# ithakis/Option-Replicating-Portfolio-with-Neural-Networks

Measured on AMD Instinct MI355X. Metric: MC paths/sec training 30-step hedge-MLP + terminal P&L std-dev, 1/2/4/8 MI355X, higher is better.
Workload: dtype fp32

## Files before the change

csrc/hedge_lm.hip:

```cpp
#include <utility>

#include "hedge_core.h"
#include "hedge_narrow.h"

namespace rph {

typedef float lm_f32x16 __attribute__((ext_vector_type(16)));

template <int P>
struct LmShape {
  static constexpr int NP = ((P + 31) / 32) * 32;
  static constexpr int NB = NP / 32;
  static constexpr int NBLK = NB * (NB + 1) / 2;
  static constexpr int JP = NP + 33;
  static_assert(NP <= LM_NPMAX && NBLK * 1024 <= LM_GBLK_MAX, "network too large for the LM solver");
};

template <class F, int... J>
RPH_INLINE void lm_static_for(F&& f, std::integer_sequence<int, J...>) {
  (f(std::integral_constant<int, J>{}), ...);
}
template <int N, class F>
RPH_INLINE void lm_static_for(F&& f) {
  lm_static_for(f, std::make_integer_sequence<int, N>{});
}

}
#include "lm_chol.h"
namespace rph {

template <int P>
struct LmTPack {
  using TG = TileGrid<P>;
  static constexpr int OFF = LmShape<P>::NBLK * 1024;
  static constexpr int LEN = TG::NTILE * 256;
  static constexpr bool ON = TG::NX > 0 && OFF + LEN <= LM_GBLK_MAX;
  static constexpr int COPY = ON ? LEN : 0;
};

RPH_INLINE void lm_blk(int b, int NB, int& mb, int& nb) {
  int m = 0;
  while (b >= NB - m) {
    b -= NB - m;
    ++m;
  }
  mb = m;
  nb = m + b;
}

RPH_INLINE constexpr int lm_row(int q, int h) { return (q & 3) + 8 * (q >> 2) + 4 * h; }

template <class B>
__global__ __launch_bounds__(256, B::WAVES_PER_SIMD) void k_lm_pass(const TrainDesc d, const LmDesc lm, const int pass,
                                                                   const double* __restrict__ red_new) {
  constexpr int P = B::P;
  constexpr int R = B::R;
  constexpr int NR = B::NR;
  using S = typename B::S;
  using LS = LmShape<P>;
  constexpr int NP = LS::NP, NB = LS::NB, NBLK = LS::NBLK, JP = LS::JP;
  constexpr int NIN = B::NIN_, H = B::H_, NO = B::NO_, HEAD = B::HEAD_, NHOLD = B::NHOLD;
  const uint32_t kat = prefetch_kernarg_begin<(sizeof(TrainDesc) + sizeof(LmDesc) + 16 < 640 ? sizeof(TrainDesc) + sizeof(LmDesc) + 16 : 640)>();
  __shared__ __attribute__((aligned(16))) float scratch[B::SCRATCH_FLOATS];
  __shared__ __attribute__((aligned(16))) float wl[P + 4];
  __shared__ __attribute__((aligned(16))) float jt[B::FINAL ? 4 : LM_TILE * JP];
  __shared__ __attribute__((aligned(16))) unsigned char og_img[B::OGM ? B::OG_LDS : 16];
  const int tid = threadIdx.x, lane = tid & 63, wid = tid >> 6;
  prefetch_kernarg_end(kat);
  const bool stamp_wg = blockIdx.x >= 2 && blockIdx.y == 0;
#define RPH_STAMPP(k)                 \
  do {                                \
    if (stamp_wg) RPH_STAMP(k);       \
  } while (0)
  RPH_STAMPP(0);
  const int inst = blockIdx.y;
  double* st = lm.state + (size_t)inst * LMS_FLOATS;
  red_new += (size_t)inst * LM_RED;
  float* const slab_b = lm.slab_b + (size_t)inst * lm.num_wgs * R;
  float* const slab_g = lm.slab_g + (size_t)inst * lm.gram_wgs * NBLK * 1024;
  double* sl = st + LMS_SLOTS + LM_SLOT * (pass & 1);
  const int trial = pass == 0 ? 0 : 1 - (int)sl[LSS_BEST];
  const Perm perm = make_perm(1u, 0u, 0u, false);
  const bool path_wg = (int)blockIdx.x < lm.num_wgs;
  typename B::Pre pre;
  const int gram_base = B::OGM ? 0 : lm.gram_base;
  const bool fin = B::FINAL || pass == lm.passes;
  const typename B::Sched sc =
      B::sched(d, lm.num_wgs, (gram_base > 0 || fin) ? 0 : lm.gram_wgs, lm.gram_skip, lm.leaf_blocks);
  if (path_wg) B::load(d, 0, perm, sc.b0 * 128, lane, pre);
  for (int i = tid; i < P; i += 256) {
    float w;
    if (pass == 0) {
      const float* w0p = lm.w0 != nullptr ? lm.w0 + inst * LM_NPMAX : d.wts->w[0];
      w = w0p[i];
      if (lm.renorm) {
        if (i >= S::OW1 && i < S::OW1 + NIN * H) {
          const int f = (i - S::OW1) / H;
          w = (float)((double)w * ((double)lm.ren_isd[f] / (double)d.fisd[f]));
        } else if (i >= S::OB1 && i < S::OB1 + H) {
          double acc = (double)w;
#pragma unroll
          for (int f = 0; f < NIN; ++f)
            acc += (double)w0p[S::OW1 + f * H + (i - S::OB1)] * (double)lm.ren_isd[f] *
                   ((double)d.fmu[f] - (double)lm.ren_mu[f]);
          w = (float)acc;
        }
      }
    } else {
      w = (float)st[LMS_W + trial * LM_NPMAX + i];
    }
    wl[i] = w;
    if (pass == 0 && blockIdx.x == 0) st[LMS_W + i] = (double)w;
  }
  if (pass > 0 && sl[LSS_COPY] != 0.0) {
    constexpr int NG = LmShape<P>::NBLK * 1024 + LmTPack<P>::COPY;
    constexpr int NGR = LM_RED_OUTG - LM_GBLK_MAX + (B::NU <= LM_OG_MAX ? B::NU * (B::NU + 1) / 2 : 1);
    double* best_red = st + LMS_RED;
    for (int e = blockIdx.x * 256 + tid; e < NG + NGR; e += (int)gridDim.x * 256) {
      const int o = e < NG ? e : LM_GBLK_MAX + e - NG;
      best_red[o] = red_new[o];
    }
  }
  if (pass > 0 && sl[LSS_STOP] != 0.0) return;
  if (lm.dp_fused && blockIdx.x == 0 && tid == 0)
    __hip_atomic_fetch_add(lm.dp.counter, 1u, __ATOMIC_RELAXED, __HIP_MEMORY_SCOPE_AGENT);
  if (pass == 0 && blockIdx.x == 0 && tid == 0) {
    sl[LSS_BEST] = 1.0;
    sl[LSS_LAM] = lm.lam_carry > 0.f ? fmax(st[LMS_LAM] * (double)lm.lam_carry, (double)lm.lam_min) : (double)lm.lam0;
    sl[LSS_NU] = 2.0;
    sl[LSS_PRED] = 0.0;
    sl[LSS_COPY] = 0.0;
    sl[LSS_SPEC_IDX] = (double)LM_SPEC;
    sl[LSS_LBEST] = INFINITY;
    sl[LSS_STOP] = 0.0;
    st[LMS_NACC] = 0.0;
    st[LMS_FAIL] = 0.0;
  }
  if (pass == 0 && blockIdx.x == 0 && inst == 0 && !lm.weights_only && !lm.explore) {
    for (int k = tid; k < MAXHIST; k += 256) d.fit->hist[k] = __builtin_nanf("");
  }
  __syncthreads();
  RPH_STAMPP(1);
  if (path_wg) {
    typename B::Frags fr;
    B::make_frags(wl + S::OW2, fr);
    float val[NR];
    B::partial(d, 0, perm, wl, fr, scratch, pre, val, sc, og_img,
               lm.slab_o + ((size_t)inst * lm.num_wgs + blockIdx.x) * 3 * 1024);
#pragma unroll
    for (int j = 0; j < NR; ++j)
      if (tid + 256 * j < R) slab_b[(size_t)blockIdx.x * R + tid + 256 * j] = val[j];
  }
  RPH_STAMPP(2);
  const int gtile = (int)blockIdx.x - gram_base;
  if (fin || gtile < 0 || gtile >= lm.gram_wgs) return;
  if constexpr (!B::FINAL) {
  if (wid == 0) {
    const long long slot = (long long)gtile * LM_TILE + lane;
    float x[NIN], pr[NHOLD];
    bool ok;
    if (lm.gram_side) {
      ok = true;
#pragma unroll
      for (int f = 0; f < NIN; ++f) x[f] = (lm.gfeat[f][slot] - d.fmu[f]) * d.fisd[f];
#pragma unroll
      for (int k = 0; k < NHOLD - 1; ++k) pr[k] = lm.gprice[k][slot];
    } else {
      const long long p = (slot / lm.gram_blk) * lm.gram_blk_stride + slot % lm.gram_blk;
      ok = p < d.n_local;
      const long long q = ok ? p : 0;
#pragma unroll
      for (int f = 0; f < NIN; ++f) x[f] = (d.feat[f][q] - d.fmu[f]) * d.fisd[f];
#pragma unroll
      for (int k = 0; k < NHOLD - 1; ++k) pr[k] = d.price[k][q];
    }
    pr[NHOLD - 1] = d.bond;
    float z1[H], a1[H], z2[H], a2[H], hold[NHOLD];
    net_forward<NIN, H, NO, HEAD>(wl, x, d.alpha, z1, a1, z2, a2, hold);
    float wq = 1.f;
    if (d.loss == LOSS_PINBALL) {
      const long long p = (slot / lm.gram_blk) * lm.gram_blk_stride + slot % lm.gram_blk;
      float V = 0.f;
#pragma unroll
      for (int k = 0; k < NHOLD; ++k) V = fmaf(hold[k], pr[k], V);
      const float y = lm.gram_side ? lm.gtarget[slot] : d.target[ok ? p : 0];
      const float ra = ok ? fabsf(V - y) : 0.f;
      float sa = ra, sc = ok ? 1.f : 0.f;
#pragma unroll
      for (int o = 32; o >= 1; o >>= 1) {
        sa += __shfl_xor(sa, o, 64);
        sc += __shfl_xor(sc, o, 64);
      }
      const float dl = fmaxf(lm.q_delta, lm.q_kappa * sa / fmaxf(sc, 1.f));
      wq = 0.5f * __builtin_amdgcn_rsqf(fmaxf(ra, dl));
    }
    float dout[NO];
    if (HEAD == HEAD_COMPLEMENT) {
      dout[0] = pr[0] - pr[1];
    } else {
#pragma unroll
      for (int k = 0; k < NO; ++k) dout[k] = pr[k];
// ... 509 lines not shown
          const int i = k + 1 + e / MK, j = k + 1 + e % MK;
          if (j <= i) A[i * LDA + j] = aij[t] - (aik[t] * ajk[t]) * inv;
        }
      }
      lmc_wave_sync();
    });
    const int li = lane < N ? lane : 0;
    double rw[N], cl[N];
#pragma unroll
    for (int k = 0; k < N; ++k) {
      rw[k] = A[li * LDA + k];
      cl[k] = A[k * LDA + li];
    }
    const double di = lane < N ? A[lane * LDA + lane] : 1.0;
    const double ri = lm_rcp(di);
    const double gi = lane < N ? pre.gi : 0.0;
    double b = -gi;
#pragma unroll
    for (int k = 0; k < N; ++k) {
      const double zk = lmc_readlane(b, k) * lmc_readlane(ri, k);
      if (lane > k && lane < N) b -= rw[k] * zk;
    }
    b *= ri;
#pragma unroll
    for (int k = N - 1; k >= 0; --k) {
      const double dk = lmc_readlane(b, k);
      if (lane < k) b -= (cl[k] * ri) * dk;
    }
    if (lane >= N) b = 0.0;
    if (lane < N) out[lane] = b;
    double gd = 0.0;
#pragma unroll
    for (int j = 0; j < N; ++j) {
      const double gj = lane < N ? (lane == j ? G2d[li] : (lane < j ? rw[j] : cl[j])) : 0.0;
      gd += (0.5 * gj) * lmc_readlane(b, j);
    }
    double t = b * (gi + gd), tl = b * gi;
#pragma unroll
    for (int o = 32; o >= 1; o >>= 1) {
      t += __shfl_xor(t, o, 64);
      tl += __shfl_xor(tl, o, 64);
    }
    if (lane == 0) {
      *dl = t;
      dl[1] = tl;
      s_ok = ok ? 1 : 0;
    }
  }
  __syncthreads();
  return s_ok != 0;
}

template <int P, int R, int NU>
__global__ __launch_bounds__(256) void k_lm_solve(const TrainDesc d, const LmDesc lm, const double* __restrict__ red_new,
                                                  const int pass) {
#pragma clang fp contract(off)
  using LS = LmShape<P>;
  constexpr int NB = LS::NB, NBLK = LS::NBLK;
  extern __shared__ __attribute__((aligned(16))) double lds[];
  __shared__ int s_fail;
  __shared__ double s_diag;
  const int tid = threadIdx.x, lane = tid & 63, wid = tid >> 6;
  const int m = blockIdx.x;
  unsigned long long ts[8] = {};
  const bool stamp_on = d.stamps != nullptr && m == 0 && blockIdx.y == 0 && tid == 0;
#define RPH_STAMPS(k)                                        \
  do {                                                       \
    if (stamp_on) ts[(k)] = rph_stamp_clock();                \
  } while (0)
  RPH_STAMPS(0);
#ifdef RPH_LDS_POISON
  for (int i = tid; i < TileGrid<P>::LDS_BYTES / 8; i += 256) lds[i] = __builtin_nan("");
  __syncthreads();
#endif
  const int inst = blockIdx.y;
  double* st = lm.state + (size_t)inst * LMS_FLOATS;
  red_new += (size_t)inst * LM_RED;
  double* best_red = st + LMS_RED;
  const double* sin = st + LMS_SLOTS + LM_SLOT * (pass & 1);
  double* sout = st + LMS_SLOTS + LM_SLOT * ((pass + 1) & 1);
  const double sv_best = sin[LSS_BEST], sv_lbest = sin[LSS_LBEST], sv_stop = sin[LSS_STOP];
  const double sv_lam = sin[LSS_LAM], sv_nu = sin[LSS_NU], sv_pred = sin[LSS_PRED], sv_sidx = sin[LSS_SPEC_IDX];
  const double t_loss = red_new[LM_GBLK_MAX + LM_NPMAX], cnt = red_new[LM_GBLK_MAX + LM_NPMAX + 3];
  double sp_lam[LM_SPEC], sp_ok[LM_SPEC], sp_pred[LM_SPEC];
#pragma unroll
  for (int k = 0; k < LM_SPEC; ++k) {
    sp_lam[k] = st[LMS_SPEC_LAM + k];
    sp_ok[k] = st[LMS_SPEC_OK + k];
    sp_pred[k] = st[LMS_SPEC_PRED + k];
  }
  constexpr int NDS = (P + 63) / 64;
  const int tc = tid < P ? tid : P - 1;
  const double w_slot0 = st[LMS_W + tc], w_slot1 = st[LMS_W + LM_NPMAX + tc];
  const double g_new = red_new[LM_GBLK_MAX + tc], g_old = best_red[LM_GBLK_MAX + tc];
  const double d_new = lmc_gram<TileGrid<P>::NBG>(red_new, tc, tc), d_old = lmc_gram<TileGrid<P>::NBG>(best_red, tc, tc);
  double ds_new[NDS], ds_old[NDS];
#pragma unroll
  for (int k = 0; k < NDS; ++k) {
    const int i = lane + 64 * k < P ? lane + 64 * k : P - 1;
    ds_new[k] = lmc_gram<TileGrid<P>::NBG>(red_new, i, i);
    ds_old[k] = lmc_gram<TileGrid<P>::NBG>(best_red, i, i);
  }
  const bool final_pass = pass == lm.passes;
  constexpr bool OG_PRE = NU * NU <= 512;
  LmOgPre og_pre[2];
  double ogm_new = -1.0, ogm_old = -1.0;
  if constexpr (OG_PRE) {
    if (final_pass && m == 0 && lm.out_gram && lm.out_n == NU) {
      ogm_new = red_new[LM_RED_OUTG];
      ogm_old = best_red[LM_RED_OUTG];
#pragma unroll
      for (int u = 0; u < 2; ++u) {
// ... 254 lines not shown
      break;
    default:
      LmcOwner<P, 2>::template run<STAGED>(src, lds + TG::OFF_DIAG, g, T, pub, fac, &s_fail, lds + TG::OFF_RDG,
                                             lds + TG::OFF_X, xdone);
      break;
  }
  __syncthreads();
  RPH_STAMPS(3);
#ifdef RPH_DUMP_T
  if (m == 0 && d.stamps != nullptr)
    for (int i = tid; i < TG::NTILE * 256 + 2 * TG::PT; i += 256) reinterpret_cast<double*>(d.stamps)[i] = lds[i];
#endif
  const bool failed = s_fail != 0;
  __shared__ double s_pred[4];
  if (!failed) {
    double pv = 0.0;
    if (tid < P) {
      const double dv = vec[tid];
      pv = 0.5 * (dmp * dv * dv - gi * dv);
    }
#pragma unroll
    for (int o = 32; o >= 1; o >>= 1) pv += __shfl_xor(pv, o, 64);
    if (lane == 0) s_pred[wid] = pv;
    __syncthreads();
  }
  const double pred = (s_pred[0] + s_pred[1]) + (s_pred[2] + s_pred[3]);
  if (m > 0) {
    if (tid < P) st[LMS_SPEC_W + m * LM_NPMAX + tid] = failed ? wbest : wbest + vec[tid];
    if (tid == 0) {
      st[LMS_SPEC_LAM + m] = lam_m;
      st[LMS_SPEC_PRED + m] = failed ? 0.0 : pred;
      st[LMS_SPEC_OK + m] = failed ? 0.0 : 1.0;
    }
    return;
  }
  RPH_STAMPS(4);
  if (failed) {
    if (tid < P) st[LMS_W + (1 - best) * LM_NPMAX + tid] = wbest;
    publish(fmin(lam * lm.lam_up * lm.lam_up, (double)lm.lam_max), pred_prev, (double)LM_SPEC);
    if (tid == 0) {
      st[LMS_FAIL] += 1.0;
      st[LMS_FAILTOT] += 1.0;
    }
    return;
  }
  RPH_STAMPS(5);
  if (tid < P) st[LMS_W + (1 - best) * LM_NPMAX + tid] = wbest + vec[tid];
  publish(lam, pred, 1.0);
  if (stamp_on)
    for (int k = 0; k < 8; ++k) d.stamps[k] = ts[k];
#undef RPH_STAMPS
}

template <int NIN, int H, int NO, int HEAD>
struct LmKernels {
  using Body = NarrowPairBody<NIN, H, NO, HEAD>;
  using BodyOG = NarrowPairBody<NIN, H, NO, HEAD, true>;
  using S = NetShape<NIN, H, NO, HEAD>;
  static constexpr int smem() { return TileGrid<S::P>::LDS_BYTES; }
  static_assert(smem() + 128 <= 160 * 1024, "LM solve exceeds the LDS of one workgroup");
};

static int lm_validate(const TrainDesc* d, const LmDesc* lm, int P, int R, int nblk, int nu) {
  if (int rc = validate_train(d, 3 , "rph_lm")) return rc;
  if (!lm->state || !lm->slab_b || !lm->slab_g) return rph_report("rph_lm", "null LM buffer");
  if (d->batch != d->n_local || d->steps_per_epoch != 1) return rph_report("rph_lm", "LM fits are full batch");
  if (lm->num_wgs < 1 || lm->num_wgs > LM_PASS_WGS_MAX || lm->passes < 0 || lm->passes >= MAXHIST)
    return rph_report("rph_lm", "bad num_wgs (1..512) / passes");
  if (lm->leaf_blocks < 0 || (lm->leaf_blocks > 0 && (long long)lm->leaf_blocks * 128 * 4 * lm->num_wgs < d->batch))
    return rph_report("rph_lm", "leaf_blocks: the waves' leaves must cover the shard");
  if (lm->gram_wgs < 1 || lm->gram_wgs > 65535) return rph_report("rph_lm", "bad Gram workgroup count");
  if (lm->gram_base != 0 && (lm->gram_base != lm->num_wgs || lm->inst != 1))
    return rph_report("rph_lm", "gram_base: 0 or the path grid (one instance)");
  if (lm->gram_side) {
    const int nhold = d->head == HEAD_COMPLEMENT ? 2 : d->nout;
    for (int f = 0; f < d->nin; ++f)
      if (!lm->gfeat[f]) return rph_report("rph_lm", "null Gram subsample feature");
    for (int k = 0; k < nhold - 1; ++k)
      if (!lm->gprice[k]) return rph_report("rph_lm", "null Gram subsample price");
  } else {
    if (lm->gram_blk < 1 || lm->gram_blk > lm->gram_blk_stride)
      return rph_report("rph_lm", "bad Gram subsample geometry");
    const long long ns = (long long)lm->gram_wgs * LM_TILE;
    const long long last = ((ns - 1) / lm->gram_blk) * lm->gram_blk_stride + (ns - 1) % lm->gram_blk;
    if (last >= d->n_local) return rph_report("rph_lm", "Gram subsample leaves the shard");
  }
  if (lm->red_wgs != nblk * 1024 / 64 + R / 4 + lm_og_wgs(nu)) return rph_report("rph_lm", "bad red_wgs");
  if (lm->out_gram && (!lm->slab_o || nu > LM_OG_MAX)) return rph_report("rph_lm", "output Gram needs slab_o (<= 64 output parameters)");
  if (d->loss != LOSS_MSE && d->loss != LOSS_PINBALL) return rph_report("rph_lm", "LM fits: MSE or pinball loss");
  if (d->loss == LOSS_PINBALL && ((lm->gram_side && !lm->gtarget) || lm->out_gram || lm->out_n > 0 ||
                                  lm->bias_index >= 0 || !(lm->q_delta > 0.f)))
    return rph_report("rph_lm", "pinball LM fits: subsample targets with a simulated subsample, no output / "
                                "bias step, q_delta > 0");
  if (R != 128 && R != 256) return rph_report("rph_lm", "packet width must be 128 or 256");
  if (lm->inst < 1 || lm->inst > LM_SEL_MAX) return rph_report("rph_lm", "bad instance count");
  if (lm->inst > 1 && !lm->explore) return rph_report("rph_lm", "several instances are exploration fits only");
  if (lm->dp_fused) {
    const int nflags = R / 4 + lm_og_wgs(nu);
    if (!lm->gram_side || lm->inst != 1 || lm->explore || lm->weights_only)
      return rph_report("rph_lm", "fused DP exchange: one main fit on the shared Gram subsample only");
    if (lm->dp.world < 2 || lm->dp.world > 8 || lm->dp.rank < 0 || lm->dp.rank >= lm->dp.world ||
        lm->dp.pitch < LM_DP_PITCH || !lm->dp.counter || !lm->dp.error || nflags > LM_DP_FLAGS)
      return rph_report("rph_lm", "fused DP exchange: bad mailbox descriptor");
    for (int q = 0; q < lm->dp.world; ++q)
      if (!lm->dp.mbox[q]) return rph_report("rph_lm", "fused DP exchange: null peer mailbox");
  }
  if (lm->explore && lm->weights_only) return rph_report("rph_lm", "exploration fits publish nothing");
  if (lm->out_gram && lm->bias_index != -1 && (lm->bias_index < P - nu || lm->bias_index >= P))
    return rph_report("rph_lm", "output Gram: bias_index must be -1 or an output-layer parameter");
  return 0;
}

template <int A, int B, int C, int E>
static int lm_pass_launch(const TrainDesc* d, const LmDesc* lm, int pass, const double* red_new, hipStream_t s) {
  using K = LmKernels<A, B, C, E>;
  const bool og = lm->out_gram && pass > lm->passes - LM_OUTG_TAIL;
  const int gend = pass == lm->passes ? 0 : (og && K::BodyOG::OGM ? 0 : lm->gram_base) + lm->gram_wgs;
  const unsigned grid = (unsigned)(gend > lm->num_wgs ? gend : lm->num_wgs);
  if constexpr (K::BodyOG::OGM) {
    if (og) {
      hipLaunchKernelGGL((k_lm_pass<typename K::BodyOG>), dim3(grid, lm->inst), dim3(256), 0, s, *d, *lm, pass,
                         red_new);
      return (int)hipGetLastError();
    }
  }
  hipLaunchKernelGGL((k_lm_pass<typename K::Body>), dim3(grid, lm->inst), dim3(256), 0, s, *d, *lm, pass, red_new);
  return (int)hipGetLastError();
}

__global__ __launch_bounds__(256) void k_lm_dp_exchange(const LmDpDesc x, double* __restrict__ red, const int ng,
                                                         const int p) {
  __shared__ unsigned s_seq;
  const int tid = threadIdx.x, wg = blockIdx.x, W = x.world, me = x.rank;
  if (tid == 0) s_seq = __hip_atomic_load(x.counter, __ATOMIC_RELAXED, __HIP_MEMORY_SCOPE_AGENT) + 1u;
  __syncthreads();
  const unsigned seq = s_seq;
  const int slot = (int)(seq % DP_SLOTS);
  (void)p;
  const int len = ng + (LM_RED - LM_GBLK_MAX), chunk = (len + LM_DP_WGS - 1) / LM_DP_WGS;
  const int e0 = wg * chunk, e1 = min(len, e0 + chunk);
  auto off = [&](int e) {
    return e < ng ? e : LM_GBLK_MAX + e - ng;
  };
  for (int e = e0 + tid; e < e1; e += 256) {
    const double v = red[off(e)];
    for (int q = 0; q < W; ++q)
      if (q != me)
        __hip_atomic_store(x.mbox[q] + ((size_t)slot * W + me) * x.pitch + e, v, __ATOMIC_RELAXED,
                           __HIP_MEMORY_SCOPE_SYSTEM);
  }
  asm volatile("s_waitcnt vmcnt(0)" ::: "memory");
  __syncthreads();
  if (tid < W && tid != me) {
    unsigned* fo = reinterpret_cast<unsigned*>(x.mbox[tid] + ((size_t)slot * W + me) * x.pitch + LM_RED + wg);
    __hip_atomic_store(fo, seq, __ATOMIC_RELEASE, __HIP_MEMORY_SCOPE_SYSTEM);
    const unsigned* fi =
        reinterpret_cast<const unsigned*>(x.mbox[me] + ((size_t)slot * W + tid) * x.pitch + LM_RED + wg);
    unsigned it = 0;
    const unsigned long long t0 = __builtin_amdgcn_s_memrealtime();
    while (__hip_atomic_load(fi, __ATOMIC_ACQUIRE, __HIP_MEMORY_SCOPE_SYSTEM) != seq) {
      __builtin_amdgcn_s_sleep(2);
      if ((++it & 255u) == 0u && (__builtin_amdgcn_s_memrealtime() - t0 > DP_SPIN_TICKS ||
                                  __hip_atomic_load(x.error, __ATOMIC_RELAXED, __HIP_MEMORY_SCOPE_SYSTEM) != 0u)) {
        __hip_atomic_store(x.error, 1u, __ATOMIC_RELAXED, __HIP_MEMORY_SCOPE_SYSTEM);
        break;
      }
    }
  }
  __syncthreads();
  for (int e = e0 + tid; e < e1; e += 256) {
    const int o = off(e);
    double s = 0.0;
    for (int q = 0; q < W; ++q)
      s += q == me ? red[o]
                   : __hip_atomic_load(x.mbox[me] + ((size_t)slot * W + q) * x.pitch + e, __ATOMIC_RELAXED,
                                       __HIP_MEMORY_SCOPE_SYSTEM);
    red[o] = s;
  }
  __syncthreads();
// ... 128 lines not shown
  hipLaunchKernelGGL(k_lm_select, dim3(1), dim3(256), 0, (hipStream_t)stream, *d, *lm, sel, main_state, world, rank,
                     P, phase);
  return (int)hipGetLastError();
}

extern "C" int rph_lm_dp_exchange(const LmDpDesc* x, double* red, int ng, int p, void* stream) {
  if (!x || !red || x->world < 2 || x->world > 8 || x->rank < 0 || x->rank >= x->world)
    return rph_report("rph_lm_dp_exchange", "bad world / rank");
  if (x->pitch < LM_RED + LM_DP_WGS || ng < 0 || ng > LM_GBLK_MAX || p < 1 || (ng > 0 && p > LM_NPMAX))
    return rph_report("rph_lm_dp_exchange", "bad mailbox pitch / block geometry");
  if ((x->pitch % 2) != 0) return rph_report("rph_lm_dp_exchange", "mailbox rows must be 16-byte aligned");
  for (int q = 0; q < x->world; ++q)
    if (!x->mbox[q]) return rph_report("rph_lm_dp_exchange", "null peer mailbox");
  if (ng == 0) {
    if (p > LM_GREG || (p & 1)) return rph_report("rph_lm_dp_exchange", "bad gradient-region length");
    hipLaunchKernelGGL(k_lm_dp_exchange_g, dim3(1), dim3(256), 0, (hipStream_t)stream, *x, red, p);
    return (int)hipGetLastError();
  }
  hipLaunchKernelGGL(k_lm_dp_exchange, dim3(LM_DP_WGS), dim3(256), 0, (hipStream_t)stream, *x, red, ng, p);
  return (int)hipGetLastError();
}

extern "C" int rph_lm_shape(int nin, int h, int nout, int head, int* p, int* r, int* nblk) {
  int rc = -1;
  match_shape(NarrowShapes{}, nin, h, nout, head, &rc, [&](auto t) {
    using S = typename decltype(t)::S;
    *p = S::P;
    *r = S::R;
    *nblk = LmShape<S::P>::NBLK;
    return 0;
  });
  return rc;
}

extern "C" int rph_lm_pass_wps(int nin, int h, int nout, int head) {
  int wps = 1;
  match_shape(NarrowShapes{}, nin, h, nout, head, &wps, [](auto t) {
    using T = decltype(t);
    return (int)LmKernels<T::NIN, T::H, T::NO, T::HEAD>::Body::WAVES_PER_SIMD;
  });
  return wps;
}

template <class K>
static LmDesc lm_pass_desc(const LmDesc& lm, const int pass) {
  LmDesc lp = lm;
  const bool og = lm.out_gram && pass > lm.passes - LM_OUTG_TAIL;
  if (og && K::BodyOG::WAVES_PER_SIMD == 1 && lm.leaf_blocks == 0 && lm.gram_base == 0 && lm.num_wgs > 256 &&
      pass == lm.passes)
    lp.num_wgs = 256;
  return lp;
}

extern "C" int rph_lm_eval(const TrainDesc* d, const LmDesc* lm, double* red_new, int pass, void* stream) {
  hipStream_t s = (hipStream_t)stream;
  int rc = 0;
  if (match_shape(NarrowShapes{}, d->nin, d->h, d->nout, d->head, &rc, [&](auto t) {
        using T = decltype(t);
        using K = LmKernels<T::NIN, T::H, T::NO, T::HEAD>;
        constexpr int P = K::S::P, R = K::S::R, NU = K::Body::NU, NBLK = LmShape<P>::NBLK;
        if (int rc = lm_validate(d, lm, P, R, NBLK, NU)) return rc;
        const LmDesc lp = lm_pass_desc<K>(*lm, pass);
        if (int rc = lm_pass_launch<T::NIN, T::H, T::NO, T::HEAD>(d, &lp, pass, red_new, s)) return rc;
        const int ngw = lm_gram_red_wgs(NBLK * 1024, lp.gram_wgs);
        const int wg0 = pass == lp.passes ? ngw : 0;
        const int rg = ngw + lm_pk_red_wgs(R, lp.num_wgs, lp.dp_fused) + lm_og_wgs(NU) - wg0;
        hipLaunchKernelGGL((k_lm_reduce<P, R, NU>), dim3(rg, lp.inst), dim3(1024), 0, s, lp, red_new, pass, wg0);
        return (int)hipGetLastError();
      }))
    return rc;
  return rph_report("rph_lm_eval", "no LM solver for this network shape (8-unit nets only)");
}

extern "C" int rph_lm_solve(const TrainDesc* d, const LmDesc* lm, const double* red_new, int pass, void* stream) {
  hipStream_t s = (hipStream_t)stream;
  int rc = 0;
  if (match_shape(NarrowShapes{}, d->nin, d->h, d->nout, d->head, &rc, [&](auto t) {
        using T = decltype(t);
        using K = LmKernels<T::NIN, T::H, T::NO, T::HEAD>;
        constexpr auto kernel = k_lm_solve<K::S::P, K::S::R, K::Body::NU>;
        const int bytes = K::smem();
        static bool attr = false;
        if (!attr) {
          hipError_t e = hipFuncSetAttribute((const void*)kernel, hipFuncAttributeMaxDynamicSharedMemorySize, bytes);
          if (e != hipSuccess) {
            (void)hipGetLastError();
            return rph_report("rph_lm_solve", "dynamic LDS request refused");
          }
          attr = true;
        }
        hipLaunchKernelGGL(kernel, dim3(LM_SPEC, lm->inst), dim3(256), bytes, s, *d, *lm, red_new, pass);
        return (int)hipGetLastError();
      }))
    return rc;
  return rph_report("rph_lm_solve", "no LM solver for this network shape");
}

extern "C" int rph_lm_fit(const TrainDesc* d, const LmDesc* lm, double* red_new, void* stream) {
  for (int k = 0; k <= lm->passes; ++k) {
    if (int rc = rph_lm_eval(d, lm, red_new, k, stream)) return rc;
    if (int rc = rph_lm_solve(d, lm, red_new, k, stream)) return rc;
  }
  return 0;
}
```

csrc/hedge_mlp.hip:

```cpp
#include "hedge_core.h"
#include "hedge_fit.h"
#include "hedge_lag.h"
#include "hedge_narrow.h"

#include <type_traits>

namespace rph {

template <int NIN, int H, int NO, int HEAD>
__global__ __launch_bounds__(256) void k_hedge_train_step(const TrainDesc d, const int step, const int epoch,
                                                          const Perm perm) {
  using B = NarrowBody<NIN, H, NO, HEAD>;
  constexpr int R = B::R;
  constexpr int P = B::P;
  prefetch_kernarg<sizeof(TrainDesc) + 2 * sizeof(int) + sizeof(Perm)>();
  __shared__ __attribute__((aligned(16))) float lds[B::SCRATCH_FLOATS];
  __shared__ __attribute__((aligned(16))) float wl[P + 4];
  __shared__ int s_last;

  RPH_DASSERT(d.batch > 0 && d.n_local >= d.batch && d.num_wgs == (int)gridDim.x);
  RPH_STAMP(0);
  const float stopped = d.fit->stopped;
  const float wv = threadIdx.x < P ? d.wts->w[0][threadIdx.x] : 0.f;
  UpdPre<P> up;
  if (d.fused_update) prefetch_update<P>(up, d.wts, d.opt, d.fit, d.lr_sched, epoch, step);
  const int lane = threadIdx.x & 63, wid = threadIdx.x >> 6;
  typename B::Pre pre;
  pre.valid = false;
  if (B::first(wid) < d.batch) B::load(d, step, perm, B::first(wid), lane, pre);

  if (stopped != 0.f) return;
  if (threadIdx.x < P) wl[threadIdx.x] = wv;
  if (d.fused_update) {
    asm volatile("" ::"v"(up.m[0]), "v"(up.v[0]), "v"(up.w[0]), "v"(up.wbest[0]), "s"(up.t), "s"(up.lr), "s"(up.loss_sum),
                 "s"(up.wait), "s"(up.best_loss), "s"(up.lr_sched_e));
  }
  __syncthreads();
  RPH_STAMP(1);
  float vv[1];
  B::partial(d, step, perm, wl, typename B::Frags{}, lds, pre, vv);
  float val = vv[0];
  float* red = lds;
  RPH_STAMP(3);

  if (gridDim.x > 1) {
    const int G = gridDim.x;
    if (threadIdx.x < R) {
      if (d.deterministic) st_agent(d.slab + (size_t)blockIdx.x * R + threadIdx.x, val);
      else __hip_atomic_fetch_add(d.acc + (blockIdx.x % ACC_REPLICAS) * R + threadIdx.x, val, __ATOMIC_RELAXED,
                                  __HIP_MEMORY_SCOPE_AGENT);
    }
    asm volatile("s_waitcnt vmcnt(0)" ::: "memory");
    __syncthreads();
// ... 29 lines not shown
              "global_load_dword %0, %8, off sc1\n\t"
              "global_load_dword %1, %8, off offset:512 sc1\n\t"
              "global_load_dword %2, %8, off offset:1024 sc1\n\t"
              "global_load_dword %3, %8, off offset:1536 sc1\n\t"
              "global_load_dword %4, %8, off offset:2048 sc1\n\t"
              "global_load_dword %5, %8, off offset:2560 sc1\n\t"
              "global_load_dword %6, %8, off offset:3072 sc1\n\t"
              "global_load_dword %7, %8, off offset:3584 sc1\n\t"
              "s_waitcnt vmcnt(0)"
              : "=&v"(r0), "=&v"(r1), "=&v"(r2), "=&v"(r3), "=&v"(r4), "=&v"(r5), "=&v"(r6), "=&v"(r7)
              : "v"(a)
              : "memory");
        } else {
          float* b = a + 4 * R;
          asm volatile(
              "global_load_dword %0, %8, off sc1\n\t"
              "global_load_dword %1, %8, off offset:1024 sc1\n\t"
              "global_load_dword %2, %8, off offset:2048 sc1\n\t"
              "global_load_dword %3, %8, off offset:3072 sc1\n\t"
              "global_load_dword %4, %9, off sc1\n\t"
              "global_load_dword %5, %9, off offset:1024 sc1\n\t"
              "global_load_dword %6, %9, off offset:2048 sc1\n\t"
              "global_load_dword %7, %9, off offset:3072 sc1\n\t"
              "s_waitcnt vmcnt(0)"
              : "=&v"(r0), "=&v"(r1), "=&v"(r2), "=&v"(r3), "=&v"(r4), "=&v"(r5), "=&v"(r6), "=&v"(r7)
              : "v"(a), "v"(b)
              : "memory");
        }
        val = ((r0 + r1) + (r2 + r3)) + ((r4 + r5) + (r6 + r7));
#pragma unroll
        for (int rp = 0; rp < ACC_REPLICAS; ++rp) st_agent(a + rp * R, 0.f);
      }
    }
    if (threadIdx.x == 0) __hip_atomic_store(d.counter, 0u, __ATOMIC_RELAXED, __HIP_MEMORY_SCOPE_AGENT);
  }
  if (threadIdx.x < R) red[threadIdx.x] = val;
  __syncthreads();
  RPH_STAMP(6);

  if (d.dp_world > 1) {
    dp_allreduce<R>(d, red);
    RPH_STAMP(7);
  }
  if (d.fused_update) {
    apply_update<P>(red, up, d.wts, d.opt, d.fit, epoch, step, d.steps_per_epoch);
  } else if (threadIdx.x < R) {
    d.grad_out[threadIdx.x] = red[threadIdx.x];
  }
  if (d.dp_world <= 1) RPH_STAMP(7);
}

template <int NIN, int H, int NO, int HEAD, bool PA, bool EX = false>
__global__ __launch_bounds__(256) void k_hedge_eval(const EvalDesc d) {
  using S = NetShape<NIN, H, NO, HEAD>;
  constexpr int NHOLD = S::NHOLD;
  static_assert(!PA || NIN >= NHOLD - 1, "price alias needs a feature per traded asset");
  prefetch_kernarg<sizeof(EvalDesc)>();
  RPH_DASSERT(d.n_local > 0 && d.num_wgs == (int)gridDim.x && d.wa != nullptr && d.stats != nullptr);
  __shared__ double sst[4][EVAL_NSTAT];
  constexpr int WBOFF = (S::P + 3) / 4 * 4;
  __shared__ __attribute__((aligned(16))) float wl[WBOFF + S::P + 4];
  const bool has_b = d.wb != nullptr;
  for (int i = threadIdx.x; i < S::P; i += 256) {
    wl[i] = d.wa->w[0][i];
    if (has_b) wl[WBOFF + i] = d.wb->w[0][i];
  }
  __syncthreads();
  if (blockIdx.x == 0) {
    for (int i = threadIdx.x; i < S::P; i += 256) {
      if (d.snap_a) d.snap_a->w[0][i] = wl[i];
      if (d.snap_b) d.snap_b->w[0][i] = has_b ? wl[WBOFF + i] : wl[i];
    }
  }
  const float* __restrict__ WA = wl;
  const float* __restrict__ WB = has_b ? wl + WBOFF : wl;
  const int lane = threadIdx.x & 63, wid = threadIdx.x >> 6;

  constexpr int NS = 64;
  float st[NS];
#pragma unroll
  for (int i = 0; i < NS; ++i) st[i] = 0.f;
  float rmin = INFINITY, rmax = -INFINITY;

  struct In {
    float x[NIN], pt[NHOLD], pt1[NHOLD], tgt, gb;
    int p;
    bool valid;
  };
  constexpr int EPF = 4;
  const int stride = (int)gridDim.x * 256;
  const bool has1 = d.price_t1[0] != nullptr;
  const bool pnl_on = !EX && d.pnl_acc != nullptr;
  const bool pnl_read = pnl_on && !d.pnl_first;
  auto load_in = [&](int p, In& in) {
    in.p = p;
    in.valid = p < d.n_local;
    const int pp = in.valid ? p : 0;
#pragma unroll
    for (int f = 0; f < NIN; ++f) in.x[f] = d.feat[f][pp];
#pragma unroll
    for (int k = 0; k < NHOLD - 1; ++k) {
      if constexpr (PA) in.pt[k] = in.x[PA ? k : 0];
      else in.pt[k] = d.price_t[k][pp];
      in.pt1[k] = has1 ? d.price_t1[k][pp] : 0.f;
    }
    in.tgt = (has1 && d.target) ? d.target[pp] : 0.f;
    in.gb = d.g_base ? d.g_base[pp] : 0.f;
  };
  In q[EPF];
  const int p_first = blockIdx.x * 256 + threadIdx.x;
#pragma unroll
  for (int i = 0; i < EPF; ++i) load_in(p_first + i * stride, q[i]);

  for (int p0 = blockIdx.x * 256; p0 < d.n_local; p0 += stride) {
    const In cur = q[0];
#pragma unroll
    for (int i = 0; i + 1 < EPF; ++i) q[i] = q[i + 1];
    if (p0 + EPF * stride < d.n_local) load_in(cur.p + EPF * stride, q[EPF - 1]);
    const int p = cur.p;
    const bool valid = cur.valid;
    const float racc = pnl_read ? d.pnl_acc[valid ? p : 0] : 0.f;
    uint32_t zo = 0;
    asm volatile("" : "+v"(zo));
    const float* __restrict__ WAi = (const float*)__builtin_assume_aligned(WA + (zo & ~3u), 16);
    const float* __restrict__ WBi = (const float*)__builtin_assume_aligned(WB + (zo & ~3u), 16);
    float z1[H], a1[H], z2[H], a2[H], hold[NHOLD], holdv[NHOLD], xn[NIN];
#pragma unroll
    for (int f = 0; f < NIN; ++f) xn[f] = (cur.x[f] - d.fmu[f]) * d.fisd[f];
    net_forward<NIN, H, NO, HEAD>(WAi, xn, d.alpha, z1, a1, z2, a2, hold);
#pragma unroll
    for (int k = 0; k < NHOLD; ++k) holdv[k] = hold[k];
    if (has_b) {
      net_forward<NIN, H, NO, HEAD>(WBi, xn, d.alpha, z1, a1, z2, a2, holdv);
#pragma unroll
      for (int k = 0; k < NHOLD; ++k) hold[k] = hold[k] + d.hold_c * (holdv[k] - hold[k]);
    }
    float V = 0.f;
#pragma unroll
    for (int k = 0; k < NHOLD - 1; ++k) V = fmaf(holdv[k], cur.pt[k], V);
    V = fmaf(holdv[NHOLD - 1], d.bond_t, V);
    if (d.g_base) V = cur.gb + d.blend_c * (V - cur.gb);
    [[maybe_unused]] float cont = V, xval = 0.f;
    [[maybe_unused]] bool exer = false;
    if constexpr (EX) {
      xval = d.ex_kind == EX_PUT ? fmaxf(d.ex_strike - cur.pt[0], 0.f) : fmaxf(cur.pt[0] - d.ex_strike, 0.f);
      exer = xval > 0.f && xval >= cont;
      V = exer ? xval : cont;
    }
    float res = 0.f, pred1 = 0.f;
    const float tgt = cur.tgt;
    if (has1) {
#pragma unroll
      for (int k = 0; k < NHOLD - 1; ++k) pred1 = fmaf(hold[k], cur.pt1[k], pred1);
      pred1 = fmaf(hold[NHOLD - 1], d.bond_t1, pred1);
      if (d.target) res = tgt - pred1;
    }
    if (valid) {
      if (d.v_out) d.v_out[p] = V;
#pragma unroll
      for (int k = 0; k < NHOLD; ++k)
        if (d.hold_out[k]) d.hold_out[k][p] = hold[k];
      if (d.resid_out) d.resid_out[p] = res;
      if (d.pred1_out) d.pred1_out[p] = pred1;
      if constexpr (!EX) {
        if (pnl_on) {
          float gain = 0.f;
#pragma unroll
          for (int k = 0; k < NHOLD - 1; ++k) gain = fmaf(hold[k], cur.pt1[k] - cur.pt[k] * d.pnl_grow, gain);
          d.pnl_acc[p] = fmaf(d.pnl_carry, gain, racc);
        }
      }
      st[ES_V] += V;
      st[ES_V2] += V * V;
      st[ES_RES] += res;
      st[ES_RES2] += res * res;
      st[ES_ABSRES] += fabsf(res);
      st[ES_APE] += d.target ? fabsf(res) * __frcp_rn(fmaxf(fabsf(tgt), 1e-7f)) : 0.f;
      st[ES_PRED1] += pred1;
      st[ES_COUNT] += 1.f;
      if constexpr (EX) {
        st[ES_EXER] += exer ? 1.f : 0.f;
        st[ES_EXVAL] += exer ? xval : 0.f;
        st[ES_CONT] += cont;
      }
#pragma unroll
      for (int k = 0; k < NHOLD; ++k) {
        st[ES_HOLD + k] += hold[k];
        st[ES_HOLD2 + k] += hold[k] * hold[k];
      }
      rmin = fminf(rmin, res);
      rmax = fmaxf(rmax, res);
    }
  }
  wave_reduce_scatter<NS>(st, lane);
#pragma unroll
  for (int o = 1; o < 64; o <<= 1) {
    rmin = fminf(rmin, __shfl_xor(rmin, o, 64));
    rmax = fmaxf(rmax, __shfl_xor(rmax, o, 64));
  }
  if (lane < EVAL_NSTAT) sst[wid][lane] = (double)st[0];
  if (lane == 0) {
    sst[wid][ES_RESMIN] = rmin;
    sst[wid][ES_RESMAX] = rmax;
  }
  __syncthreads();
  if (threadIdx.x < EVAL_NSTAT) {
    const int i = threadIdx.x;
    double v;
    if (i == ES_RESMIN) v = fmin(fmin(sst[0][i], sst[1][i]), fmin(sst[2][i], sst[3][i]));
    else if (i == ES_RESMAX) v = fmax(fmax(sst[0][i], sst[1][i]), fmax(sst[2][i], sst[3][i]));
    else v = sst[0][i] + sst[1][i] + sst[2][i] + sst[3][i];
    d.stats[(size_t)blockIdx.x * EVAL_NSTAT + i] = v;
  }
}


template <int NIN, int H, int NO, int HEAD, bool EX = false>
__global__ __launch_bounds__(256) void k_hedge_pnl(const PnlDesc d) {
  using S = NetShape<NIN, H, NO, HEAD>;
  constexpr int NHOLD = S::NHOLD;
  constexpr int NA = NHOLD - 1;
  constexpr int WBOFF = (S::P + 3) / 4 * 4;
  prefetch_kernarg<sizeof(PnlDesc)>();
  RPH_DASSERT(d.n_local > 0 && d.num_wgs == (int)gridDim.x && d.snap != nullptr && d.stats != nullptr);
  __shared__ __attribute__((aligned(16))) float wl[WBOFF + S::P + 4];
  __shared__ double sred[4][EX ? 12 : 8];
  const int tid = threadIdx.x, lane = tid & 63, wid = tid >> 6;
  const long long base = (long long)blockIdx.x * 256 * PNL_PPT + tid;
  const bool has_b = d.has_b != 0;
  float wealth[PNL_PPT], s_cur[PNL_PPT][NA > 0 ? NA : 1];
  long long pidx[PNL_PPT];
#pragma unroll
  for (int j = 0; j < PNL_PPT; ++j) {
    const long long p = base + (long long)j * 256;
    const bool ok = p < d.n_local;
    pidx[j] = ok ? p : 0;
    wealth[j] = ok ? (d.w0 ? d.w0[p] : d.wealth0) : 0.f;
#pragma unroll
    for (int a = 0; a < NA; ++a) s_cur[j][a] = d.price[a][pidx[j]];
  }
  float xr[PNL_PPT][NIN], s_nxt[PNL_PPT][NA > 0 ? NA : 1];
  auto load_date = [&](int t) {
#pragma unroll
    for (int j = 0; j < PNL_PPT; ++j) {
#pragma unroll
      for (int f = 0; f < NIN; ++f) xr[j][f] = d.feat[f][(long long)t * d.feat_ts[f] + pidx[j]];
#pragma unroll
      for (int a = 0; a < NA; ++a) s_nxt[j][a] = d.price[a][(long long)(t + 1) * d.price_ts[a] + pidx[j]];
    }
  };
  [[maybe_unused]] int tau[PNL_PPT];
  [[maybe_unused]] float pnl_ex[PNL_PPT];
  [[maybe_unused]] double paid[PNL_PPT];
  if constexpr (EX) {
#pragma unroll
    for (int j = 0; j < PNL_PPT; ++j) {
      tau[j] = d.n_dates;
      pnl_ex[j] = 0.f;
      paid[j] = 0.0;
    }
  }
  if (d.n_dates > 0) load_date(0);
  for (int t = 0; t < d.n_dates; ++t) {
    float xc[PNL_PPT][NIN], sc_nxt[PNL_PPT][NA > 0 ? NA : 1];
#pragma unroll
    for (int j = 0; j < PNL_PPT; ++j) {
// ... 393 lines not shown
```

csrc/hedge_narrow.h:

```cpp
#pragma once
#include "hedge_core.h"

namespace rph {

template <int NIN, int H, int NO, int HEAD, int WPE = 1, int PFD = 1, bool LDSW = (WPE > 1), bool HYB = false>
struct NarrowBody {
  static constexpr int WAVES_PER_SIMD = WPE;
  static constexpr int NIN_ = NIN, H_ = H, NO_ = NO, HEAD_ = HEAD;
  static constexpr bool LDS_WEIGHTS = LDSW;
  static constexpr int PF = PFD;
  using S = NetShape<NIN, H, NO, HEAD>;
  static constexpr int P = S::P;
  static constexpr int R = S::R;
  static constexpr int NR = (R + 255) / 256;
  static constexpr int NREP = NARROW_NREP;
  static constexpr bool ACC_PLAIN = true;
  static constexpr int NHOLD = S::NHOLD;
  static constexpr int SCRATCH_FLOATS = (4 * R > 1024 ? 4 * R : 1024) + 8;
  struct Frags {};
  struct Pre {
    float x[NIN], pr[NHOLD], y;
    bool valid;
  };

  RPH_INLINE static void make_frags(const float*, Frags&) {}

  RPH_INLINE static long long first(int wid) { return (long long)(blockIdx.x * 4 + wid) * 64; }

  RPH_INLINE static void load(const TrainDesc& d, int step, const Perm& perm, long long j0, int lane, Pre& p) {
    const long long jl = j0 + lane;
    const long long j = (long long)step * d.batch + jl;
    p.valid = (jl < d.batch) && (j < d.n_local);
    const uint32_t q = p.valid ? perm_path(perm, (uint32_t)j, d.chunk_log2, d.n_local) : 0u;
#pragma unroll
    for (int f = 0; f < NIN; ++f) p.x[f] = d.feat[f][q];
#pragma unroll
    for (int k = 0; k < NHOLD - 1; ++k) p.pr[k] = d.price[k][q];
    p.pr[NHOLD - 1] = d.bond;
    p.y = d.target[q];
  }

  RPH_INLINE static void partial(const TrainDesc& d, int step, const Perm& perm, const float* __restrict__ W,
                                 const Frags&, float* lds, Pre& pre, float (&val)[NR]) {
    const int lane = threadIdx.x & 63, wid = threadIdx.x >> 6;
    const long long stride = (long long)gridDim.x * 4 * 64;
    float g[R];
#pragma unroll
    for (int i = 0; i < R; ++i) g[i] = 0.f;
    const float alpha = d.alpha;
    Pre q[PF];
    q[0] = pre;
#pragma unroll
    for (int i = 1; i < PF; ++i) {
// ... 67 lines not shown
#pragma unroll
        for (int f = 0; f < NIN; ++f) g[S::OW1 + f * H + i] = fmaf(x[f], dz1, g[S::OW1 + f * H + i]);
      }
    }
    RPH_STAMP(5);
    wave_reduce_scatter<R>(g, lane);
    constexpr int PER = R / 64;
#pragma unroll
    for (int i = 0; i < PER; ++i) lds[wid * R + lane * PER + i] = g[i];
    __syncthreads();
    const int t = threadIdx.x;
    val[0] = (t < R) ? (lds[t] + lds[R + t]) + (lds[2 * R + t] + lds[3 * R + t]) : 0.f;
    __syncthreads();
  }
};

typedef float nb_f2 __attribute__((ext_vector_type(2)));

RPH_INLINE nb_f2 nb_s(float w) { return nb_f2{w, w}; }
RPH_INLINE nb_f2 nb_fma(nb_f2 a, nb_f2 b, nb_f2 c) { return __builtin_elementwise_fma(a, b, c); }
RPH_INLINE nb_f2 nb_lrelu(nb_f2 z, float alpha) { return __builtin_elementwise_max(z, z * alpha); }
RPH_INLINE nb_f2 nb_lrelu_bwd(nb_f2 a, nb_f2 da, float alpha) {
  const nb_f2 t = da * alpha;
  return nb_f2{a.x > 0.f ? da.x : t.x, a.y > 0.f ? da.y : t.y};
}
RPH_INLINE float nb_acc(float g, nb_f2 a, nb_f2 b) { return fmaf(a.x, b.x, fmaf(a.y, b.y, g)); }

typedef __bf16 nb_bf16x8 __attribute__((ext_vector_type(8)));
typedef __bf16 nb_bf16x4 __attribute__((ext_vector_type(4)));
typedef float nb_f32x16 __attribute__((ext_vector_type(16)));
typedef short nb_s16x4 __attribute__((ext_vector_type(4)));
typedef short nb_s16x8 __attribute__((ext_vector_type(8)));
typedef __attribute__((address_space(3))) nb_s16x4 nb_lds_s16x4;

template <int PITCH, int NU>
RPH_INLINE void nb_img_put(unsigned char* img, int row, int c0, float u0, float u1, float u2, float u3) {
  const __bf16 h0 = (__bf16)u0, h1 = (__bf16)u1, h2 = (__bf16)u2, h3 = (__bf16)u3;
  const nb_bf16x4 h = {h0, h1, h2, h3};
  const nb_bf16x4 l = {(__bf16)(u0 - (float)h0), (__bf16)(u1 - (float)h1), (__bf16)(u2 - (float)h2),
                       (__bf16)(u3 - (float)h3)};
  *(nb_bf16x4*)(img + row * PITCH + 2 * c0) = h;
  *(nb_bf16x4*)(img + row * PITCH + 2 * (NU + c0)) = l;
}
template <int PITCH>
RPH_INLINE nb_bf16x8 nb_img_frag(const unsigned char* img, int s, int ub, int lane) {
  const int grp = lane >> 4, i = lane & 15, q = i >> 2, p = i & 3;
  const int c0 = 32 * ub + 16 * (grp & 1), hh = grp >> 1;
  const int off = (16 * s + 8 * hh + q) * PITCH + (c0 + 4 * p) * 2;
  const nb_s16x4 r0 = __builtin_amdgcn_ds_read_tr16_b64_v4i16((nb_lds_s16x4*)(img + off));
  const nb_s16x4 r1 = __builtin_amdgcn_ds_read_tr16_b64_v4i16((nb_lds_s16x4*)(img + off + 4 * PITCH));
  return __builtin_bit_cast(nb_bf16x8, __builtin_shufflevector(r0, r1, 0, 1, 2, 3, 4, 5, 6, 7));
}

template <int NIN, int H, int NO, int HEAD, bool OG = false>
struct NarrowPairBody {
  static constexpr int WAVES_PER_SIMD = (!OG && NIN <= 2 && HEAD == HEAD_FREE && NO <= 2) ? 2 : 1;
  static constexpr int NIN_ = NIN, H_ = H, NO_ = NO, HEAD_ = HEAD;
  using S = NetShape<NIN, H, NO, HEAD>;
  static constexpr int P = S::P;
  static constexpr int R = S::R;
  static constexpr int NR = (R + 255) / 256;
  static constexpr int NHOLD = S::NHOLD;
  static constexpr int SCRATCH_FLOATS = (4 * R > 1024 ? 4 * R : 1024) + 8;
  static_assert(R <= 256, "one packet entry per thread");
  static constexpr int NU = HEAD == HEAD_FREE ? H * NO + NO : H + 1;
  static constexpr int NUP = NU <= 32 ? 32 : 64;
  static constexpr int NBO = NUP == 32 ? 1 : 3;
  static constexpr int OG_PITCH = 4 * NUP + 8;
  static constexpr int OG_ROWS = 64;
  static constexpr int OG_LDS = 4 * OG_ROWS * OG_PITCH;
  static constexpr bool OGM = OG && NU <= 64;
  static_assert(!OG || NU <= 64, "output-layer Gram: at most 64 output parameters");
  static constexpr bool FINAL = OG;
  static_assert(!OG || LM_OUTG_TAIL == 1, "the output-Gram body is the final-evaluation body (gradient of the output block only)");
  static_assert(P - NU == S::OW3, "the output block is [OW3, P)");
  static_assert(4 * NBO * 1024 * 4 <= OG_LDS, "the waves' output-Gram tiles reuse the image LDS");
  struct Frags {};
  struct Pre {
    nb_f2 x[NIN], pr[NHOLD], y;
    nb_f2 m;
  };

  RPH_INLINE static void make_frags(const float*, Frags&) {}
  RPH_INLINE static long long first(int wid) { return (long long)(blockIdx.x * 4 + wid) * 128; }

  struct Sched {
    long long b0, bstep, bend;
  };
  RPH_INLINE static Sched sched(const TrainDesc& d, int num_wgs, int gram_wgs, int gram_skip, int leaf_blocks = 0) {
    const long long nblk = (d.batch + 127) / 128;
    const int TW = num_wgs * 4, w = (int)blockIdx.x * 4 + (int)(threadIdx.x >> 6);
    if (leaf_blocks > 0) {
      const long long b0 = (long long)w * leaf_blocks, b1 = b0 + leaf_blocks;
      return {b0, 1, b1 < nblk ? b1 : nblk};
    }
    const int GW = (gram_wgs < num_wgs ? gram_wgs : num_wgs) * 4;
    const long long per = nblk / TW;
    if (gram_skip <= 0 || GW >= TW || per <= 0) return {w, TW, nblk};
    const long long gb = per > gram_skip ? per - gram_skip : 0;
    if (w < GW) return {w, GW, GW * gb};
    return {GW * gb + (w - GW), TW - GW, nblk};
  }

  RPH_INLINE static void load(const TrainDesc& d, int, const Perm&, long long j0, int lane, Pre& p) {
    const long long ja = j0 + lane, jb = ja + 64;
    const bool va = ja < d.batch, vb = jb < d.batch;
    const long long qa = va ? ja : 0, qb = vb ? jb : 0;
#pragma unroll
    for (int f = 0; f < NIN; ++f) p.x[f] = nb_f2{d.feat[f][qa], d.feat[f][qb]};
#pragma unroll
    for (int k = 0; k < NHOLD - 1; ++k) p.pr[k] = nb_f2{d.price[k][qa], d.price[k][qb]};
    p.pr[NHOLD - 1] = nb_s(d.bond);
    p.y = nb_f2{d.target[qa], d.target[qb]};
    p.m = nb_f2{va ? 1.f : 0.f, vb ? 1.f : 0.f};
  }

  RPH_INLINE static void og_wave_sync() {
    __builtin_amdgcn_fence(__ATOMIC_RELEASE, "wavefront");
    __builtin_amdgcn_wave_barrier();
    __builtin_amdgcn_fence(__ATOMIC_ACQUIRE, "wavefront");
  }
  RPH_INLINE static void og_put(unsigned char* img, int row, int c0, float u0, float u1, float u2, float u3) {
    nb_img_put<OG_PITCH, NUP>(img, row, c0, u0, u1, u2, u3);
  }
  RPH_INLINE static nb_bf16x8 og_frag(const unsigned char* img, int s, int ub, int lane) {
    return nb_img_frag<OG_PITCH>(img, s, ub, lane);
  }

  RPH_INLINE static void og_accum(unsigned char* img, nb_f32x16 (&oacc)[NBO], const nb_f2 (&a2)[H],
                                  const nb_f2 (&pr)[NHOLD], const nb_f2 m, const int lane) {
    nb_f2 c[NO];
    if (HEAD == HEAD_COMPLEMENT) {
      c[0] = (pr[0] - pr[1]) * m;
    } else {
#pragma unroll
      for (int k = 0; k < NO; ++k) c[k] = pr[k] * m;
    }
    float ua[(NU + 3) / 4 * 4], ub[(NU + 3) / 4 * 4];
#pragma unroll
    for (int j = 0; j < H; ++j)
#pragma unroll
      for (int k = 0; k < NO; ++k) {
        const nb_f2 v = a2[j] * c[k];
        ua[j * NO + k] = v.x;
        ub[j * NO + k] = v.y;
      }
#pragma unroll
    for (int k = 0; k < NO; ++k) {
      ua[H * NO + k] = c[k].x;
      ub[H * NO + k] = c[k].y;
    }
#pragma unroll
    for (int e = NU; e < (NU + 3) / 4 * 4; ++e) ua[e] = ub[e] = 0.f;
    constexpr int LO = NUP / 32;
#pragma unroll
    for (int h2 = 0; h2 < 2; ++h2) {
      og_wave_sync();
#pragma unroll
      for (int c0 = 0; c0 < NU; c0 += 4) {
        if (h2) og_put(img, lane, c0, ub[c0], ub[c0 + 1], ub[c0 + 2], ub[c0 + 3]);
        else og_put(img, lane, c0, ua[c0], ua[c0 + 1], ua[c0 + 2], ua[c0 + 3]);
      }
      og_wave_sync();
#pragma unroll
      for (int s2 = 0; s2 < OG_ROWS / 16; ++s2) {
        const nb_bf16x8 h0 = og_frag(img, s2, 0, lane), l0 = og_frag(img, s2, LO, lane);
        oacc[0] = __builtin_amdgcn_mfma_f32_32x32x16_bf16(h0, h0, oacc[0], 0, 0, 0);
        oacc[0] = __builtin_amdgcn_mfma_f32_32x32x16_bf16(h0, l0, oacc[0], 0, 0, 0);
        oacc[0] = __builtin_amdgcn_mfma_f32_32x32x16_bf16(l0, h0, oacc[0], 0, 0, 0);
        if constexpr (NBO == 3) {
          const nb_bf16x8 h1 = og_frag(img, s2, 1, lane), l1 = og_frag(img, s2, LO + 1, lane);
          oacc[1] = __builtin_amdgcn_mfma_f32_32x32x16_bf16(h0, h1, oacc[1], 0, 0, 0);
          oacc[1] = __builtin_amdgcn_mfma_f32_32x32x16_bf16(h0, l1, oacc[1], 0, 0, 0);
          oacc[1] = __builtin_amdgcn_mfma_f32_32x32x16_bf16(l0, h1, oacc[1], 0, 0, 0);
          oacc[2] = __builtin_amdgcn_mfma_f32_32x32x16_bf16(h1, h1, oacc[2], 0, 0, 0);
          oacc[2] = __builtin_amdgcn_mfma_f32_32x32x16_bf16(h1, l1, oacc[2], 0, 0, 0);
          oacc[2] = __builtin_amdgcn_mfma_f32_32x32x16_bf16(l1, h1, oacc[2], 0, 0, 0);
        }
      }
    }
  }

  RPH_INLINE static void partial(const TrainDesc& d, int step, const Perm& perm, const float* __restrict__ W,
                                 const Frags&, float* lds, Pre& pre, float (&val)[NR], const Sched& sc,
                                 unsigned char* og_lds = nullptr, float* __restrict__ og_out = nullptr) {
    const int lane = threadIdx.x & 63, wid = threadIdx.x >> 6;
    const long long stride = sc.bstep * 128;
    const long long jend = sc.bend * 128 < d.batch ? sc.bend * 128 : d.batch;
    constexpr bool PKG = HEAD == HEAD_FREE && NO % 2 == 0 && P % 2 == 0;
    float g[R];
    nb_f2 gv[PKG ? R / 2 : 1];
#pragma unroll
    for (int i = 0; i < R; ++i) g[i] = 0.f;
#pragma unroll
    for (int i = 0; i < (PKG ? R / 2 : 1); ++i) gv[i] = nb_s(0.f);
    const float alpha = d.alpha;
    const float two_inv = 2.f * d.inv_batch;
    const bool pinball = d.loss == LOSS_PINBALL;
    const float q = d.quantile;
    Pre cur = pre;
    if constexpr (FINAL) asm volatile("" ::: "v255", "a3");
    nb_f32x16 oacc[NBO];
    unsigned char* const img = og_lds + wid * OG_ROWS * OG_PITCH;
    if constexpr (OGM) {
#pragma unroll
      for (int b = 0; b < NBO; ++b) oacc[b] = nb_f32x16{};
      constexpr int NU4 = (NU + 3) / 4 * 4;
#pragma unroll
      for (int c0 = NU4; c0 < NUP; c0 += 4) og_put(img, lane, c0, 0.f, 0.f, 0.f, 0.f);
    }
    for (long long j0 = sc.b0 * 128; j0 < jend; j0 += stride) {
      uint32_t z = 0;
      asm volatile("" : "+v"(z));
      const float* __restrict__ Wi = (const float*)__builtin_assume_aligned(W + (z & ~3u), 16);
      nb_f2 x[NIN], pr[NHOLD];
#pragma unroll
      for (int f = 0; f < NIN; ++f) x[f] = (cur.x[f] - d.fmu[f]) * d.fisd[f];
#pragma unroll
      for (int k = 0; k < NHOLD; ++k) pr[k] = cur.pr[k];
      const nb_f2 y = cur.y, m = cur.m;
      if (j0 + stride < jend) load(d, step, perm, j0 + stride, lane, cur);

      nb_f2 a1[H], a2[H], o[NO];
#pragma unroll
      for (int j = 0; j < H; ++j) {
        nb_f2 acc = nb_s(Wi[S::OB1 + j]);
#pragma unroll
        for (int f = 0; f < NIN; ++f) acc = nb_fma(x[f], nb_s(Wi[S::OW1 + f * H + j]), acc);
        a1[j] = nb_lrelu(acc, alpha);
      }
#pragma unroll
      for (int j = 0; j < H; ++j) a2[j] = nb_s(Wi[S::OB2 + j]);
#pragma unroll
      for (int i = 0; i < H; ++i)
#pragma unroll
        for (int j = 0; j < H; ++j) a2[j] = nb_fma(a1[i], nb_s(Wi[S::OW2 + i * H + j]), a2[j]);
#pragma unroll
      for (int j = 0; j < H; ++j) a2[j] = nb_lrelu(a2[j], alpha);
#pragma unroll
      for (int k = 0; k < NO; ++k) {
        nb_f2 acc0 = nb_s(Wi[S::OB3 + k]), acc1 = nb_s(0.f);
#pragma unroll
        for (int j = 0; j < H; j += 2) {
          acc0 = nb_fma(a2[j], nb_s(Wi[S::OW3 + j * NO + k]), acc0);
          acc1 = nb_fma(a2[j + 1], nb_s(Wi[S::OW3 + (j + 1) * NO + k]), acc1);
        }
        o[k] = acc0 + acc1;
      }
      nb_f2 V;
      if (HEAD == HEAD_COMPLEMENT) {
        V = nb_fma(o[0], pr[0] - pr[1], pr[1]);
      } else {
        V = o[0] * pr[0];
#pragma unroll
        for (int k = 1; k < NO; ++k) V = nb_fma(o[k], pr[k], V);
      }
      const nb_f2 e = V - y;
      nb_f2 le, dV;
      if (pinball) {
        float lx, ly, gx, gy;
        path_loss(LOSS_PINBALL, q, V.x, y.x, lx, gx);
        path_loss(LOSS_PINBALL, q, V.y, y.y, ly, gy);
        le = nb_f2{lx, ly} * m;
        dV = nb_f2{gx, gy} * m * d.inv_batch;
      } else {
        le = e * e * m;
        dV = e * m * two_inv;
      }
      const nb_f2 ae = nb_f2{fabsf(e.x), fabsf(e.y)} * m;
      const nb_f2 ape = ae * nb_f2{__builtin_amdgcn_rcpf(fmaxf(fabsf(y.x), 1e-7f)),
                                   __builtin_amdgcn_rcpf(fmaxf(fabsf(y.y), 1e-7f))};
      if constexpr (PKG) {
        gv[P / 2].x += le.x + le.y;
        gv[P / 2].y += ae.x + ae.y;
// ... 139 lines not shown
```

csrc/rph_layout.h:

```cpp
#pragma once
#include <stddef.h>

#include "rph_types.h"

namespace rph {

#define RPH_FIELDS_TrainDesc(X, T)                                                                                  \
  X(T, feat) X(T, price) X(T, target) X(T, wts) X(T, opt) X(T, fit) X(T, lr_sched) X(T, slab) X(T, counter)          \
  X(T, grad_out) X(T, bond) X(T, alpha) X(T, quantile) X(T, inv_batch) X(T, loss) X(T, n_local) X(T, batch)         \
  X(T, steps_per_epoch) X(T, chunk_log2) X(T, shuffle) X(T, seed) X(T, fused_update) X(T, num_wgs) X(T, nin)        \
  X(T, h) X(T, nout) X(T, head) X(T, pad_acc) X(T, acc) X(T, deterministic) X(T, pad_stamps) X(T, stamps)           \
  X(T, dp_world) X(T, dp_rank) X(T, dp_mbox) X(T, dp_flags) X(T, dp_counter) X(T, dp_error) X(T, mfma_fp32)         \
  X(T, pad_lag) X(T, lag) X(T, variant) X(T, pad_fit_init) X(T, fit_init) X(T, fmu) X(T, fisd)
#define RPH_FIELDS_EvalDesc(X, T)                                                                                   \
  X(T, feat) X(T, price_t) X(T, price_t1) X(T, target) X(T, wa) X(T, wb) X(T, g_base) X(T, v_out) X(T, hold_out)    \
  X(T, resid_out) X(T, pred1_out) X(T, stats) X(T, bond_t) X(T, bond_t1) X(T, alpha) X(T, blend_c) X(T, hold_c)     \
  X(T, n_local) X(T, num_wgs) X(T, nin) X(T, h) X(T, nout) X(T, head) X(T, fmu) X(T, fisd) X(T, pad_snap)           \
  X(T, snap_a) X(T, snap_b) X(T, ex_kind) X(T, ex_strike) X(T, pnl_acc) X(T, pnl_grow) X(T, pnl_carry)              \
  X(T, pnl_first) X(T, pad_pnl)
#define RPH_FIELDS_PnlFinishDesc(X, T)                                                                              \
  X(T, acc) X(T, w0) X(T, payoff) X(T, pnl_out) X(T, stats) X(T, carry) X(T, n_local) X(T, num_wgs) X(T, nin)       \
  X(T, h) X(T, nout) X(T, head) X(T, pad0)
#define RPH_FIELDS_PnlDesc(X, T)                                                                                    \
  X(T, feat) X(T, feat_ts) X(T, price) X(T, price_ts) X(T, snap) X(T, fmu) X(T, fisd) X(T, bond) X(T, w0)           \
  X(T, payoff) X(T, pnl_out) X(T, stats) X(T, alpha) X(T, hold_c) X(T, wealth0) X(T, has_b) X(T, n_local)           \
  X(T, n_dates) X(T, num_wgs) X(T, nin) X(T, h) X(T, nout) X(T, head) X(T, ex_kind) X(T, ex_every) X(T, ex_strike)  \
  X(T, tau_out)
#define RPH_FIELDS_LmDpDesc(X, T) \
  X(T, mbox) X(T, counter) X(T, error) X(T, world) X(T, rank) X(T, pitch) X(T, fault)
#define RPH_FIELDS_LmDesc(X, T)                                                                                     \
  X(T, state) X(T, slab_b) X(T, slab_g) X(T, num_wgs) X(T, gram_wgs) X(T, red_wgs) X(T, passes) X(T, gram_blk)      \
  X(T, gram_blk_stride) X(T, inv_ns) X(T, inv_n) X(T, lam0) X(T, lam_up) X(T, lam_down) X(T, lam_min) X(T, lam_max) \
  X(T, ridge) X(T, bias_index) X(T, weights_only) X(T, damping) X(T, stop_min) X(T, stop_tol) X(T, gram_skip)       \
  X(T, inst) X(T, explore) X(T, lam_carry) X(T, diag_floor) X(T, w0) X(T, renorm) X(T, pad1) X(T, ren_mu)           \
  X(T, ren_isd) X(T, out_n) X(T, out_mu) X(T, out_gram) X(T, out_tr) X(T, slab_o) X(T, gfeat) X(T, gprice)          \
  X(T, gram_side) X(T, q_delta) X(T, q_kappa) X(T, pad_dp) X(T, dp) X(T, dp_fused) X(T, leaf_blocks) X(T, gtarget)  \
  X(T, gram_base) X(T, pad4)
#define RPH_FIELDS_SimDesc(X, T)                                                                                    \
  X(T, model) X(T, n_local) X(T, path_offset) X(T, n_fine) X(T, reduction) X(T, n_coarse) X(T, na) X(T, fp64)       \
  X(T, parity) X(T, sv1) X(T, shift1) X(T, dims1) X(T, pad_sv2) X(T, sv2) X(T, shift2) X(T, dims2) X(T, pad_s0)     \
  X(T, s0) X(T, mu) X(T, sigma) X(T, chol) X(T, dt) X(T, inv_norm) X(T, v0) X(T, a) X(T, b) X(T, c) X(T, kappa)     \
  X(T, theta) X(T, xi) X(T, rho) X(T, l0) X(T, lc) X(T, eta) X(T, n0) X(T, seed) X(T, out) X(T, out2) X(T, out3)    \
  X(T, final_out) X(T, final2_out) X(T, sv_tscale) X(T, scheme) X(T, path_stat) X(T, map_blk) X(T, map_stride)

#define RPH_FIELDS_OosDesc(X, T)                                                                                    \
  X(T, sim) X(T, snap) X(T, fmu) X(T, fisd) X(T, bond) X(T, pnl_out) X(T, payoff_out) X(T, stats) X(T, alpha)       \
  X(T, hold_c) X(T, wealth0) X(T, strike) X(T, has_b) X(T, payoff_kind) X(T, n_dates) X(T, num_wgs) X(T, nin)       \
  X(T, h) X(T, nout) X(T, head)

#define RPH_DESCRIPTORS(X) \
  X(TrainDesc) X(EvalDesc) X(PnlFinishDesc) X(PnlDesc) X(LmDpDesc) X(LmDesc) X(SimDesc)
#define RPH_DESCRIPTORS_EXT(X) X(OosDesc)

struct FieldRow {
  const char* strct;
  const char* field;
  unsigned offset, size;
};

#define RPH_FIELD_ROW(T, f) {#T, #f, (unsigned)offsetof(T, f), (unsigned)sizeof(T::f)},
#define RPH_STRUCT_ROWS(T) RPH_FIELDS_##T(RPH_FIELD_ROW, T)
constexpr FieldRow kFieldRows[] = {RPH_DESCRIPTORS(RPH_STRUCT_ROWS)};
constexpr FieldRow kFieldRowsExt[] = {RPH_DESCRIPTORS_EXT(RPH_STRUCT_ROWS)};

constexpr bool layout_same(const char* a, const char* b) {
  for (; *a && *a == *b; ++a, ++b) {}
  return *a == *b;
}
template <size_t N>
constexpr bool layout_covers(const FieldRow (&rows)[N], const char* strct, size_t size) {
  size_t end = 0;
  for (const FieldRow& r : rows)
    if (layout_same(r.strct, strct)) {
      if (r.offset != end) return false;
      end += r.size;
    }
  return end == size;
}
#define RPH_STRUCT_COVERED_IN(rows, T)                                                         \
  static_assert(layout_covers(rows, #T, sizeof(T)), "RPH_FIELDS_" #T " does not cover " #T     \
                                                    ": a field is missing or out of order, or " \
                                                    "the struct has implicit padding");
#define RPH_STRUCT_COVERED(T) RPH_STRUCT_COVERED_IN(kFieldRows, T)
#define RPH_STRUCT_COVERED_EXT(T) RPH_STRUCT_COVERED_IN(kFieldRowsExt, T)
RPH_DESCRIPTORS(RPH_STRUCT_COVERED)
RPH_DESCRIPTORS_EXT(RPH_STRUCT_COVERED_EXT)

struct ConstRow {
  const char* name;
  long long value;
};

#define RPH_CONST(n) {#n, (long long)(n)},
#define RPH_FLOAT_INDEX(n, T, f) {#n, (long long)(offsetof(T, f) / 4)},
constexpr ConstRow kConstRows[] = {
    RPH_CONST(PMAX) RPH_CONST(MAXIN) RPH_CONST(MAXHOLD) RPH_CONST(MAXHIST) RPH_CONST(EVAL_NSTAT) RPH_CONST(LAG_SLOTS)
    RPH_CONST(LAG_FLOATS) RPH_CONST(PNL_PPT) RPH_CONST(OOS_WGS_PER_CU) RPH_CONST(NETW_FLOATS) RPH_CONST(OPT_FLOATS) RPH_CONST(FIT_FLOATS)
    RPH_CONST(DP_SLOTS) RPH_CONST(LM_NPMAX) RPH_CONST(LM_TILE) RPH_CONST(LM_GBLK_MAX) RPH_CONST(LM_OUTG)
    RPH_CONST(LM_OUTG_TAIL) RPH_CONST(LM_RED_OUTG) RPH_CONST(LM_RED) RPH_CONST(LM_PASS_WGS_MAX) RPH_CONST(LM_OG_MAX)
    RPH_CONST(LM_SPEC) RPH_CONST(LM_SLOT) RPH_CONST(LM_DP_WGS) RPH_CONST(LM_DP_FLAGS) RPH_CONST(LM_DP_PITCH)
    RPH_CONST(LM_SEL_W) RPH_CONST(LM_SEL_MAX)
    RPH_CONST(HEAD_FREE) RPH_CONST(HEAD_COMPLEMENT) RPH_CONST(LOSS_MSE) RPH_CONST(LOSS_PINBALL)
    RPH_CONST(EX_NONE) RPH_CONST(EX_PUT) RPH_CONST(EX_CALL) RPH_CONST(HESTON_EULER) RPH_CONST(HESTON_QE)
    RPH_CONST(STAT_NONE) RPH_CONST(STAT_MEAN) RPH_CONST(STAT_GEOMEAN) RPH_CONST(STAT_MAX) RPH_CONST(STAT_MIN)
    RPH_CONST(SIM_GBM_ARITH) RPH_CONST(SIM_GBM_LOG) RPH_CONST(SIM_SV_REF) RPH_CONST(SIM_HESTON) RPH_CONST(SIM_BASKET)
    RPH_CONST(SIM_MORTALITY)
    RPH_CONST(ES_V) RPH_CONST(ES_V2) RPH_CONST(ES_RES) RPH_CONST(ES_RES2) RPH_CONST(ES_ABSRES) RPH_CONST(ES_APE)
    RPH_CONST(ES_PRED1) RPH_CONST(ES_COUNT) RPH_CONST(ES_HOLD) RPH_CONST(ES_HOLD2) RPH_CONST(ES_RESMIN)
    RPH_CONST(ES_RESMAX) RPH_CONST(ES_EXER) RPH_CONST(ES_EXVAL) RPH_CONST(ES_CONT) RPH_CONST(ES_TAU)
    RPH_CONST(LMS_W) RPH_CONST(LMS_RED) RPH_CONST(LMS_BEST) RPH_CONST(LMS_LAM) RPH_CONST(LMS_NACC) RPH_CONST(LMS_FAIL)
    RPH_CONST(LMS_LFIN) RPH_CONST(LMS_FAILTOT) RPH_CONST(LMS_SPEC_LAM) RPH_CONST(LMS_SPEC_PRED) RPH_CONST(LMS_SPEC_OK)
    RPH_CONST(LMS_SPEC_W) RPH_CONST(LMS_SLOTS) RPH_CONST(LMS_FLOATS)
    RPH_CONST(LSS_BEST) RPH_CONST(LSS_LAM) RPH_CONST(LSS_NU) RPH_CONST(LSS_PRED) RPH_CONST(LSS_COPY)
    RPH_CONST(LSS_SPEC_IDX) RPH_CONST(LSS_LBEST) RPH_CONST(LSS_STOP)
    RPH_FLOAT_INDEX(W_CUR, NetWeights, cur)
    RPH_FLOAT_INDEX(O_M, OptState, m) RPH_FLOAT_INDEX(O_V, OptState, v) RPH_FLOAT_INDEX(O_T, OptState, t)
    RPH_FLOAT_INDEX(O_LR, OptState, lr) RPH_FLOAT_INDEX(O_B1, OptState, beta1) RPH_FLOAT_INDEX(O_B2, OptState, beta2)
    RPH_FLOAT_INDEX(O_EPS, OptState, eps) RPH_FLOAT_INDEX(O_NAN, OptState, nan_steps)
    RPH_FLOAT_INDEX(F_WBEST, FitState, w_best) RPH_FLOAT_INDEX(F_BEST, FitState, best_loss)
    RPH_FLOAT_INDEX(F_WAIT, FitState, wait) RPH_FLOAT_INDEX(F_STOPPED, FitState, stopped)
    RPH_FLOAT_INDEX(F_EPOCH, FitState, epoch) RPH_FLOAT_INDEX(F_PATIENCE, FitState, patience)
    RPH_FLOAT_INDEX(F_MAXEP, FitState, max_epochs) RPH_FLOAT_INDEX(F_RESTORE, FitState, restore_best)
    RPH_FLOAT_INDEX(F_HASBEST, FitState, has_best) RPH_FLOAT_INDEX(F_LOSS_SUM, FitState, loss_sum)
    RPH_FLOAT_INDEX(F_LOSS_CNT, FitState, loss_cnt) RPH_FLOAT_INDEX(F_ABS_SUM, FitState, abs_sum)
    RPH_FLOAT_INDEX(F_APE_SUM, FitState, ape_sum) RPH_FLOAT_INDEX(F_LAST_LOSS, FitState, last_loss)
    RPH_FLOAT_INDEX(F_LAST_MAE, FitState, last_mae) RPH_FLOAT_INDEX(F_LAST_MAPE, FitState, last_mape)
    RPH_FLOAT_INDEX(F_RESTORE_END, FitState, restore_at_end) RPH_FLOAT_INDEX(F_HIST, FitState, hist)
};

}
```

csrc/rph_types.h:

```cpp
#pragma once
#include <stdint.h>

namespace rph {

constexpr int PMAX = 2048;
constexpr int MAXIN = 8;
constexpr int MAXHOLD = 8;
constexpr int MAXHIST = 1024;
constexpr int EVAL_NSTAT = 32;
constexpr int LAG_SLOTS = 16;
constexpr int LAG_FLOATS = 3 * PMAX + 16;
constexpr int PNL_PPT = 4;
constexpr int OOS_WGS_PER_CU = 8;

enum Head : int { HEAD_FREE = 0, HEAD_COMPLEMENT = 1 };
enum Loss : int { LOSS_MSE = 0, LOSS_PINBALL = 1 };

struct NetWeights {
  float w[2][PMAX];
  float cur;
  float pad[3];
};

struct OptState {
// ... 190 lines not shown
  unsigned* error;
  int world, rank;
  int pitch;
  int fault;
};

struct LmDesc {
  double* state;
  float* slab_b;
  float* slab_g;
  int num_wgs;
  int gram_wgs;
  int red_wgs;
  int passes;
  int gram_blk;
  int gram_blk_stride;
  float inv_ns;
  float inv_n;
  float lam0, lam_up, lam_down, lam_min, lam_max, ridge;
  int bias_index;
  int weights_only;
  int damping;
  int stop_min;
  float stop_tol;
  int gram_skip;
  int inst;
  int explore;
  float lam_carry;
  float diag_floor;
  const float* w0;
  int renorm;
  int pad1;
  float ren_mu[MAXIN];
  float ren_isd[MAXIN];
  int out_n;
  float out_mu;
  int out_gram;
  float out_tr;
  float* slab_o;
  const float* gfeat[MAXIN];
  const float* gprice[MAXIN];
  int gram_side;
  float q_delta;
  float q_kappa;
  int pad_dp;
  LmDpDesc dp;
  int dp_fused;
  int leaf_blocks;
  const float* gtarget;
  int gram_base;
  int pad4;
};

constexpr int LM_SEL_W = LM_NPMAX + 2;
constexpr int LM_SEL_MAX = 64;


enum EvalStat : int {
  ES_V = 0, ES_V2 = 1, ES_RES = 2, ES_RES2 = 3, ES_ABSRES = 4, ES_APE = 5, ES_PRED1 = 6,
  ES_COUNT = 7, ES_HOLD = 8 , ES_HOLD2 = 16 , ES_RESMIN = 24,
  ES_RESMAX = 25,
  ES_EXER = 26, ES_EXVAL = 27, ES_CONT = 28, ES_TAU = 29
};

enum ExKind : int { EX_NONE = 0, EX_PUT = 1, EX_CALL = 2 };

struct SimDesc {
  int model;
  int n_local;
  long long path_offset;
  int n_fine;
  int reduction;
  int n_coarse;
  int na;
  int fp64;
  int parity;
  const uint32_t* sv1; const uint32_t* shift1; int dims1;
  int pad_sv2;
  const uint32_t* sv2; const uint32_t* shift2; int dims2;
  int pad_s0;
  double s0[MAXIN], mu[MAXIN], sigma[MAXIN];
  double chol[MAXIN * MAXIN];
  double dt;
  double inv_norm[MAXIN];
  double v0, a, b, c, kappa, theta, xi, rho;
  double l0, lc, eta; int n0; uint32_t seed;
  float* out;
  float* out2;
  float* out3;
  float* final_out;
  float* final2_out;
  double sv_tscale;
  int scheme;
  int path_stat;
  long long map_blk;
  long long map_stride;
};

struct OosDesc {
  SimDesc sim;
  const NetWeights* snap;
  const float* fmu;
  const float* fisd;
  const double* bond;
  float* pnl_out;
  float* payoff_out;
// ... 27 lines not shown
```

csrc/runtime.cpp:

```cpp
#include <hip/hip_runtime.h>
#include <rccl/rccl.h>
#include <stddef.h>
#include <stdio.h>
#include <string.h>

#include "rph_layout.h"

using namespace rph;

static thread_local char g_err[512];

static int set_err(const char* what, int code, const char* msg) {
  snprintf(g_err, sizeof(g_err), "%s failed (%d): %s", what, code, msg ? msg : "");
  return code == 0 ? -1 : code;
}

#define HIP_TRY(expr)                                                              \
  do {                                                                             \
    hipError_t _e = (expr);                                                        \
    if (_e != hipSuccess) return set_err(#expr, (int)_e, hipGetErrorString(_e));   \
  } while (0)

#define NCCL_TRY(expr)                                                             \
  do {                                                                             \
    ncclResult_t _r = (expr);                                                      \
    if (_r != ncclSuccess) return set_err(#expr, (int)_r, ncclGetErrorString(_r)); \
  } while (0)

extern "C" const char* rph_last_error() { return g_err; }

namespace rph {
int rph_report(const char* what, const char* msg) { return set_err(what, -22, msg); }
int rph_report_shape(const char* what, int nin, int h, int nout, int head) {
  char msg[128];
  snprintf(msg, sizeof(msg), "unsupported network shape (nin %d, h %d, nout %d, head %d)", nin, h, nout, head);
  return rph_report(what, msg);
}
}

extern "C" int rph_layout_fields(const FieldRow** rows) {
  *rows = kFieldRows;
  return (int)(sizeof(kFieldRows) / sizeof(kFieldRows[0]));
}

extern "C" int rph_layout_fields_ext(const FieldRow** rows) {
  *rows = kFieldRowsExt;
  return (int)(sizeof(kFieldRowsExt) / sizeof(kFieldRowsExt[0]));
}

extern "C" int rph_layout_consts(const ConstRow** rows) {
  *rows = kConstRows;
  return (int)(sizeof(kConstRows) / sizeof(kConstRows[0]));
}

extern "C" int rph_device_info(int dev, int* cus, int* lds_per_cu, long long* hbm_bytes, char* name, int name_cap) {
  hipDeviceProp_t p;
  HIP_TRY(hipGetDeviceProperties(&p, dev));
  *cus = p.multiProcessorCount;
  *lds_per_cu = (int)p.maxSharedMemoryPerMultiProcessor;
  *hbm_bytes = (long long)p.totalGlobalMem;
  snprintf(name, name_cap, "%s", p.gcnArchName);
  return 0;
}

extern "C" int rph_memset_async(void* ptr, int value, long long bytes, void* stream) {
  HIP_TRY(hipMemsetAsync(ptr, value, (size_t)bytes, (hipStream_t)stream));
  return 0;
}

extern "C" int rph_stream_sync(void* stream) {
  HIP_TRY(hipStreamSynchronize((hipStream_t)stream));
  return 0;
}

extern "C" int rph_graph_begin(void* stream) {
  HIP_TRY(hipStreamBeginCapture((hipStream_t)stream, hipStreamCaptureModeThreadLocal));
  return 0;
}

extern "C" int rph_graph_end(void* stream, void** exec_out, long long* num_nodes) {
  hipGraph_t g = nullptr;
  HIP_TRY(hipStreamEndCapture((hipStream_t)stream, &g));
  size_t nn = 0;
  HIP_TRY(hipGraphGetNodes(g, nullptr, &nn));
  *num_nodes = (long long)nn;
  hipGraphExec_t ex = nullptr;
  HIP_TRY(hipGraphInstantiate(&ex, g, nullptr, nullptr, 0));
  HIP_TRY(hipGraphDestroy(g));
  *exec_out = (void*)ex;
  return 0;
}

extern "C" int rph_graph_launch(void* exec, void* stream) {
  HIP_TRY(hipGraphLaunch((hipGraphExec_t)exec, (hipStream_t)stream));
  return 0;
}

extern "C" int rph_graph_destroy(void* exec) {
  HIP_TRY(hipGraphExecDestroy((hipGraphExec_t)exec));
  return 0;
// ... 91 lines not shown
```

rphedge/api.py:

```python
from __future__ import annotations

import math
import time
from dataclasses import dataclass, field

import numpy as np
import torch

from . import risk
from .config import RunConfig, parse_params
from .driver import BackwardInduction, InductionConfig, InductionResult, error_history, expected_value_trajectory
from .engine import Exercise, TrainConfig, gram_subsample, make_backend, set_weights
from .models import hedge_mlp as hm
from .ops import layout as L
from .ops import paths as P
from .parallel import dist as D
from .utils.logging import get_logger
from .utils.profiling import PhaseTimer


@dataclass
class RunResult:
    phi: float
    psi: float
# ... 272 lines not shown
        if p.nfrac_final is not None:
            en = float(p.nfrac_final.double().sum())
            out["E_N_T"] = (D.all_reduce_scalar(en, device=self.device) if w > 1 else en) / n * c.N
        out["mean_Y_T"] = (D.all_reduce_scalar(float(yT.double().sum()), device=self.device) if w > 1
                           else float(yT.double().sum())) / n * (c.Y if self.kind != "pension" else 1.0)
        return out

    def init_align(self) -> tuple | None:
        c = self.cfg
        if str(getattr(c.train, "init", "reference")) != "aligned" or self.kind != "basket":
            return None
        return tuple(c.basket_weights or [1.0 / c.n_assets] * c.n_assets)

    def feature_centers(self) -> tuple | None:
        c = self.cfg
        if self.kind == "pension" or c.payoff not in ("call", "put", "basket_call"):
            return None
        k = float(c.K) / float(c.Y)
        nin = self.spec.nin
        return tuple([k] * nin) if self.kind == "basket" else (k,) + (None,) * (nin - 1)

    def init_weights(self, stats: dict) -> np.ndarray:
        c, spec = self.cfg, self.spec
        if self.kind == "pension":
            bias = [1.0 - stats["p_oom"], stats["p_oom"]]
        elif spec.head == L.HEAD_COMPLEMENT:
            bias = [stats["E_payoff"]]
        else:
            p_itm = 1.0 - stats["p_oom"]
            bias = [p_itm, stats["E_payoff"] - p_itm] + [0.0] * (spec.nout - 2)
            if self.kind == "basket":
                bias = [p_itm / c.n_assets] * c.n_assets + [stats["E_payoff"] - p_itm]
        return hm.init_weights(spec, bias[: spec.nout], seed=c.train.seed,
                               spread=str(getattr(c.train, "init", "reference")) in ("spread", "aligned"),
                               align=self.init_align(),
                               shared_stream=bool(c.parity.shared_initializer))

    def build(self, w0: np.ndarray | None = None):
        c = self.cfg
        if self.paths is None:
            self.simulate()
        self.stats0 = self.summary_stats()
        self.w0 = self.init_weights(self.stats0) if w0 is None else w0
        tr = c.train
        tcfg = TrainConfig(batch_size=tr.batch_size, shuffle=tr.shuffle, chunk_log2=tr.chunk_log2, seed=tr.seed,
                           lr=tr.lr, deterministic=tr.deterministic, max_wgs=tr.max_wgs,
                           mfma_fp32=str(tr.mfma_precision).lower() == "fp32", step_mode=tr.step_mode,
                           lm_gram_paths=int(tr.lm_gram_paths), lm_damping=str(tr.lm_damping),
                           lm_leaf_paths=int(getattr(tr, "lm_leaf_paths", -1)),
                           lm_lam0=float(tr.lm_lam0), lm_lam_up=float(tr.lm_lam_up),
                           lm_lam_down=float(tr.lm_lam_down), lm_out_fix=bool(tr.lm_out_fix),
                           lm_out_mu=float(tr.lm_out_mu), lm_out_tr=float(getattr(tr, "lm_out_tr", 0.0)),
                           lm_ridge=float(getattr(tr, "lm_ridge", 1e-10)),
                           lm_diag_floor=float(tr.lm_diag_floor))
        if int(tr.variant) >= 0:
            tcfg.variant = int(tr.variant)
        kw = {}
        if self.backend_kind == "hip" and self.di.world > 1:
            if self.di.probe is None and self.di.dp_mode == "xgmi":
                D.select_transport(self.di)
            self.mailbox = D.make_mailbox(self.di, self.spec.red_width)
            kw["mailbox"] = self.mailbox
            self.lm_mailbox = D.make_mailbox(self.di, L.LM_DP_PITCH, tag="rph_lmbox",
                                             mode=self.di.lm_dp_mode)
            kw["lm_mailbox"] = self.lm_mailbox
            kw["lm_comm"] = self.di.lm_comm
        self.backend = make_backend(self.backend_kind, self.spec, self.n_local, tcfg, device=self.device,
                                    comm=self.di.comm, world=self.di.world, rank=self.di.rank, stream=self.stream,
                                    **kw)
        pf = c.parity
        icfg = InductionConfig(epochs_first=tr.epochs_first, epochs_rest=tr.epochs_rest,
                               patience_first=tr.patience_first, patience_rest=tr.patience_rest,
                               early_stopping=tr.early_stopping,
                               lr_schedule_first=tr.lr_schedule_first and pf.lr_schedule_first_only,
                               lr=tr.lr, lr_rest=tr.lr_rest, lr_decay=tr.lr_decay,
                               q99=tr.q99, quantile=tr.quantile, cost_of_capital=tr.cost_of_capital,
                               shared_q99_model=pf.shared_q99_model,
                               holdings_blend_sign_rp=pf.holdings_blend_sign_rp, warm_start=pf.warm_start, carry_optimizer=pf.carry_optimizer,
                               restore_best_at_end=pf.restore_best_at_end, keep_paths=c.keep_paths,
                               poll_every=tr.poll_every, seed=tr.seed,
                               feature_norm="none" if pf.raw_features else tr.feature_norm,
                               feature_centers=self.feature_centers(),
                               feature_norm_floor=float(getattr(tr, "feature_norm_floor", 0.0)),
                               optimizer=str(tr.optimizer).lower(), lm_passes_first=int(tr.lm_passes_first),
                               q99_optimizer=str(getattr(tr, "q99_optimizer", "adam")).lower(),
                               lm_q_passes_first=int(getattr(tr, "lm_q_passes_first", 40)),
                               lm_q_passes_rest=int(getattr(tr, "lm_q_passes_rest", 4)),
                               lm_q_delta=float(getattr(tr, "lm_q_delta", 1e-4)),
                               lm_q_kappa=float(getattr(tr, "lm_q_kappa", 3.0)),
                               lm_q_start=str(getattr(tr, "lm_q_start", "mse")),
                               lm_passes_rest=int(tr.lm_passes_rest), lm_stop_tol=float(tr.lm_stop_tol),
                               lm_stop_min=int(tr.lm_stop_min), lm_lam0_rest=float(tr.lm_lam0_rest),
                               lm_lam0_first=float(tr.lm_lam0_first),
                               lm_lam_carry=float(tr.lm_lam_carry), lm_starts=int(tr.lm_starts),
                               lm_renorm=bool(tr.lm_renorm),
                               lm_explore_passes=int(tr.lm_explore_passes), lm_explore_log2=int(tr.lm_explore_log2),
                               lm_explore_one=bool(getattr(tr, "lm_explore_one", False)),
                               init_spread=str(getattr(tr, "init", "reference")) in ("spread", "aligned"),
                               init_align=self.init_align(),
                               init_shared_stream=bool(pf.shared_initializer),
                               mean_refit=bool(tr.mean_refit) and not pf.keras_fit_only,
                               exercise=self.exercise)
        backend_q = None
        if (self.backend_kind == "hip" and self.di.world == 1 and icfg.q99 and not icfg.shared_q99_model
                and not icfg.poll_every and tr.concurrent_q99):
            backend_q = make_backend(self.backend_kind, self.spec, self.n_local, tcfg, device=self.device,
                                     world=1, rank=0, stream=None)
# ... 311 lines not shown
```

rphedge/config.py:

```python
from __future__ import annotations

import math
from dataclasses import asdict, dataclass, field, fields

GBM_KEYS = ("Y", "K", "T", "mu", "r", "sigma", "rebalancing", "N", "P", "x", "l0", "c", "ita", "dt", "n_paths")
SV_KEYS = ("Y", "K", "T", "mu", "r", "s0", "a", "b", "c", "rebalancing", "N", "P", "x", "l0", "ita", "dt",
           "n_paths")


@dataclass
class ParityFlags:

    shared_q99_model: bool = False
    holdings_blend_sign_rp: bool = False
    lambda_fine_index: bool = False
    sv_c_overwrite: bool = False
    sv_reference_dynamics: bool = False
    sv_sqrt_nan: bool = False
    fine_terminal_payoff: bool = True
    lr_schedule_first_only: bool = True
    warm_start: bool = True
    carry_optimizer: bool = True
    restore_best_at_end: bool = False
    numpy_binomial: bool = False
# ... 24 lines not shown
    patience_first: int = 50
    patience_rest: int = 7
    lr: float = 1e-3
    lr_schedule_first: bool = True
    lr_rest: float = 0.0
    lr_decay: float = 1.0
    early_stopping: bool = True
    cost_of_capital: float = 0.1
    quantile: float = 0.99
    q99: bool = True
    shuffle: bool = True
    chunk_log2: int = 0
    seed: int = 1234
    leaky_alpha: float = 0.3
    poll_every: int = 0
    deterministic: bool = False
    max_wgs: int = 0
    hidden: int = 8
    mfma_precision: str = "bf16"
    step_mode: str = "auto"
    variant: int = -1
    concurrent_q99: bool = True
    optimizer: str = "adam"
    q99_optimizer: str = "adam"
    lm_q_passes_first: int = 40
    lm_q_passes_rest: int = 4
    lm_q_delta: float = 1e-4
    lm_q_kappa: float = 3.0
    lm_q_start: str = "mse"
    lm_passes_first: int = 80
    lm_passes_rest: int = 3
    lm_stop_tol: float = 0.0
    lm_stop_min: int = 2
    init: str = "reference"
    lm_lam0_rest: float = 0.0
    lm_lam_carry: float = 0.0
    lm_out_fix: bool = False
    lm_out_mu: float = 1e-5
    lm_out_tr: float = 0.0
    lm_ridge: float = 1e-10
    lm_renorm: bool = False
    lm_starts: int = 1
    lm_explore_passes: int = 45
    lm_explore_log2: int = 16
    lm_explore_one: bool = False
    lm_gram_paths: int = 4096
    lm_leaf_paths: int = -1
    lm_damping: str = "simple"
    lm_lam0: float = 1e-3
    lm_lam_up: float = 4.0
    lm_lam_down: float = 1.0 / 3.0
    lm_lam0_first: float = 0.0
    lm_diag_floor: float = 0.0
    mean_refit: bool = True
    feature_norm: str = "date"
    feature_norm_floor: float = 0.0


@dataclass
class RunConfig:

    Y: float = 1.0
    K: float = 1.0
    T: float = 10.0
    mu: float = 0.08
    r: float = 0.03
    sigma: float = 0.15
    rebalancing: float = 0.25
    N: int = 10_000
    P: float = 100.0
    x: float = 55.0
    l0: float = 0.01
    c: float = 0.075
    ita: float = 0.000597
    dt: float = 1 / 100
    n_paths: int = 12
    s0: float = 0.15965
    a: float = 0.0033566
    b: float = 0.15431
    sv_c: float = 0.015833
    kappa: float = 2.0
    theta: float = 0.0256
    xi: float = 0.3
    rho: float = -0.7
    v0: float = 0.0256
    heston_scheme: str = "qe"
    sv_days_per_year: float = 252.0
    model: str = "gbm"
    payoff: str = "guarantee"
    path_feature: bool = True
    option_type: str = "CALL"
    exercise: str = "european"
    exercise_every: int = 1
    oos_paths_log2: int = 0
    oos_seed: int | None = None
    oos_stress: object = None
    mortality: bool = True
    n_assets: int = 1
    basket_weights: tuple = ()
    basket_corr: float = 0.5
    device: str | None = None
    backend: str | None = None
    world_size: int | None = None
    dtype: str = "fp32"
    verbose: bool = True
    save_dir: str | None = None
# ... 71 lines not shown
```

rphedge/driver.py:

```python
from __future__ import annotations

import math
from dataclasses import dataclass, field

import numpy as np
import torch

from .engine import (MAXIN, DateData, Exercise, FitConfig, PnlData, TrainConfig, fit_seed, fit_summary,
                     geometric_lr_schedule, keras_lr_schedule, pnl_fold_factors, reduce_stats)
from .models.hedge_mlp import NetSpec
from .ops import layout as L
from .ops.paths import Paths


@dataclass
class InductionConfig:
    epochs_first: int = 500
    epochs_rest: int = 100
    patience_first: int = 50
    patience_rest: int = 7
    early_stopping: bool = True
    lr_schedule_first: bool = True
    lr: float = 1e-3
    lr_rest: float = 0.0
# ... 239 lines not shown
    def explore_data(self, t: int) -> DateData | None:
        if self.explore_paths is None:
            return None
        if t != self.paths.n_coarse - 2:
            raise ValueError(f"explore_data(t={t}): the exploration prefix holds the terminal payoff, the target of "
                             f"the first fitted date t = {self.paths.n_coarse - 2} only")
        xp, xv = self.explore_paths
        mu, isd = self.norms[t] if self.norms else ((), ())
        return DateData(feats=xp.features(t), prices_next=xp.prices(t + 1), bond_next=float(xp.bond[t + 1]),
                        target=xv, prices_now=xp.prices(t), bond_now=float(xp.bond[t]), fmu=mu, fisd=isd)

    def date_data(self, t: int) -> DateData:
        p = self.paths
        mu, isd = self.norms[t] if self.norms else ((), ())
        gp = self.gram_paths
        return DateData(feats=p.features(t), prices_next=p.prices(t + 1), bond_next=float(p.bond[t + 1]),
                        target=self.values[t + 1], prices_now=p.prices(t), bond_now=float(p.bond[t]),
                        fmu=mu, fisd=isd, gram_feats=gp.features(t) if gp is not None else None,
                        gram_prices_next=gp.prices(t + 1) if gp is not None else None,
                        gram_target=self.gvalues[t + 1] if self.gvalues is not None else None)

    def gram_date_data(self, t: int) -> DateData:
        gp = self.gram_paths
        mu, isd = self.norms[t] if self.norms else ((), ())
        return DateData(feats=gp.features(t), prices_next=gp.prices(t + 1), bond_next=float(gp.bond[t + 1]),
                        target=self.gvalues[t + 1], prices_now=gp.prices(t), bond_now=float(gp.bond[t]),
                        fmu=mu, fisd=isd)

    def eval_gram_values(self, t: int, with_target: bool = True):
        c, be = self.cfg, self.backend
        gd = self.gram_date_data(t)
        if not with_target:
            gd.target = None
        ns = self.ggbuf.numel()
        be.eval(self.w_mse, gd, self.gstats[0], v_out=self.ggbuf, n_local=ns)
        be.eval(self.w_mse, gd, self.gstats[1], wts_b=self.w_q, g_base=self.ggbuf,
                blend_c=c.cost_of_capital, hold_c=self.hold_c, v_out=self.gvalues[t], n_local=ns)

    def restore_gram_values(self, date: int):
        if self.gvalues is None:
            return
        if date >= self.paths.n_coarse - 1:
            self.gvalues[date].copy_(self.g_terminal)
        else:
            self.eval_gram_values(date, with_target=False)

    def enqueue(self, start: int | None = None):
        c, be = self.cfg, self.backend
        nc = self.paths.n_coarse
        start = nc - 2 if start is None else int(start)
        self.ran = list(range(start, -1, -1))
        self.pnl_done = start == nc - 2
        fold = self.pnl_fold and self.pnl_done
        for t in self.ran:
            first = t == nc - 2
            pnl_kw = dict(pnl_acc=self.pnl_acc, pnl_grow=float(self.pnl_grow[t]), pnl_carry=float(self.pnl_carry[t]),
                          pnl_first=first) if fold else {}
            data = self.date_data(t)
            if not c.carry_optimizer and c.warm_start and not first:
                self.opt_mse.copy_(self.opt_init)
                if c.q99:
                    self.opt_q.copy_(self.opt_init)
            if not c.warm_start and not first:
                self.w_mse.copy_(self.w_init)
                self.opt_mse.copy_(self.opt_init)
                if c.q99:
                    if not c.shared_q99_model:
                        self.w_q.copy_(self.w_init)
                    self.opt_q.copy_(self.opt_init)
            f_m, f_q = self.fits[t]
            s_m, s_q = self.stats[t]
            join = None
            q_from_mse = self.q_lm and str(c.lm_q_start).lower() == "mse"
            if self.backend_q is not None and not q_from_mse:
                main = torch.cuda.current_stream(self.values.device)
                if self._side is None:
                    self._side = torch.cuda.Stream(self.values.device)
                fork = torch.cuda.Event()
                fork.record(main)
                self._side.wait_event(fork)
                with torch.cuda.stream(self._side):
                    self.backend_q.fit(self.w_q, self.opt_q, f_q, data, self._fcfg(first, L.LOSS_PINBALL),
                                       seed=fit_seed(c.seed, t, 1), poll_every=0)
                    join = torch.cuda.Event()
                    join.record(self._side)
            be.fit(self.w_mse, self.opt_mse, f_m, data, self._fcfg(first, L.LOSS_MSE, t),
                   seed=fit_seed(c.seed, t, 0), poll_every=c.poll_every)
            if c.mean_refit and c.optimizer != "lm":
                be.bias_refit(self.w_mse, self.opt_mse, f_m, data, self._fcfg(first, L.LOSS_MSE))
            hold_out = [self.holdings[t, k] for k in range(self.spec.nhold)] if self.holdings is not None else None
            resid_out = self.residuals[t] if self.residuals is not None else None
            if c.q99:
                be.eval(self.w_mse, data, s_m, v_out=self.gbuf)
                if join is not None:
                    torch.cuda.current_stream(self.values.device).wait_event(join)
                else:
                    if q_from_mse:
                        self.w_q.copy_(self.w_mse)
                    be.fit(self.w_q, self.opt_q, f_q, data, self._fcfg(first, L.LOSS_PINBALL),
                           seed=fit_seed(c.seed, t, 1), poll_every=c.poll_every)
                be.eval(self.w_mse, data, s_q, wts_b=self.w_q, g_base=self.gbuf, blend_c=c.cost_of_capital,
                        hold_c=self.hold_c, v_out=self.values[t], hold_out=hold_out, resid_out=resid_out,
                        snap_a=self.snap[t, 0], snap_b=self.snap[t, 1], **pnl_kw)
                if self.gvalues is not None:
                    self.eval_gram_values(t)
            else:
                be.eval(self.w_mse, data, s_q, v_out=self.values[t], hold_out=hold_out, resid_out=resid_out,
                        snap_a=self.snap[t, 0], exercise=self.exercise_at(t), **pnl_kw)
        if fold:
            be.pnl_finish(self.pnl_acc, self.values[0], self.values[nc - 1], float(self.pnl_carry_all),
                          self.pnl_stats, pnl_out=self.pnl_paths)
        elif self.pnl_done:
            be.pnl(self.snap, self.pnl_data, self.pnl_stats, has_b=c.q99, hold_c=self.hold_c,
                   pnl_out=self.pnl_paths, exercise=c.exercise, tau_out=self.tau)

    def collect(self) -> InductionResult:
        c = self.cfg
        nc = self.paths.n_coarse
        dtc = self.paths.grid.dt_coarse
        res = InductionResult(values=self.values, holdings=self.holdings, residuals=self.residuals,
                              weights_snapshots=self.snap)
        for t in getattr(self, "ran", range(nc - 2, -1, -1)):
            f_m, f_q = self.fits[t]
            s_m, s_q = self.stats[t]
            d = DateResult(index=t, time=t * dtc, fit_mse=fit_summary(f_m),
                           fit_q99=fit_summary(f_q) if c.q99 else None,
                           stats=reduce_stats(s_q, self.world),
                           stats_mse=reduce_stats(s_m, self.world) if c.q99 else None)
            res.dates.append(d)
        d0 = res.dates[-1]
        res.terminal = res.dates[0]
        res.v0 = d0.mean_value
        res.holdings0 = d0.mean_holdings(self.spec.nhold)
        if self.pnl_done:
            res.pnl = DateResult(index=-1, time=float(self.paths.grid.times()[-1]),
                                 stats=reduce_stats(self.pnl_stats, self.world))
            res.pnl_paths = self.pnl_paths
            res.tau = self.tau
        return res


def price_features(paths: Paths) -> list:
    nin = len(paths.features(0))
    return list(range(nin)) if paths.kind not in ("pension", "heston", "sv", "gbm_stat") else [0]


def feature_norms(paths: Paths, mode: str, world: int = 1, centers=None, floor: float = 0.0) -> list:
    mode = (mode or "none").lower()
    if mode == "none":
        return []
    if mode not in ("global", "date", "horizon"):
        raise ValueError(f"feature_norm must be none | global | date | horizon, got {mode!r}")
    nd = paths.n_coarse - 1
    nin = len(paths.features(0))
    s1, s2 = [], []
    for t in range(nd):
        for x in paths.features(t):
            s1.append(x.sum(dtype=torch.float64))
# ... 71 lines not shown
```

rphedge/engine/config.py:

```python
from __future__ import annotations

from dataclasses import dataclass, field

import numpy as np
import torch

from ..ops import layout as L


def keras_lr_schedule(epochs: int) -> list:
    return [1e-2 if e < 100 else 1e-3 if e < 200 else 5e-4 if e < 400 else float("nan") for e in range(epochs)]


def geometric_lr_schedule(lr0: float, epochs: int, decay: float = 1.0) -> tuple:
    n = max(int(epochs), 1)
    if n == 1 or decay == 1.0:
        return tuple([float(lr0)] * n)
    return tuple(float(lr0) * decay ** (e / (n - 1)) for e in range(n))


@dataclass
class FitConfig:
    epochs: int = 100
    patience: int = 7
# ... 4 lines not shown
    restore_at_end: bool = False
    early_stopping: bool = True
    optimizer: str = "adam"
    lm_stop_tol: float = 0.0
    lm_stop_min: int = 2
    lm_lam0: float | None = None
    lm_lam_carry: float = 0.0
    lm_renorm: tuple | None = None
    lm_starts: int = 1
    lm_explore_passes: int = 0
    lm_explore_paths: int = 0
    lm_w0s: object = None
    lm_explore_data: object = None
    lm_q_delta: float = 0.0
    lm_q_kappa: float = 3.0

    def key(self):
        return (self.epochs, self.patience if self.early_stopping else 1 << 30, self.restore_best,
                self.restore_at_end, tuple(self.lr_schedule) if self.lr_schedule is not None else None)


@dataclass
class TrainConfig:
    batch_size: int = 512
    shuffle: bool = True
    chunk_log2: int = 0
    seed: int = 1234
    lr: float = 1e-3
    beta1: float = 0.9
    beta2: float = 0.999
    eps: float = 1e-7
    max_wgs: int = 0
    paths_per_thread: int = 1
    deterministic: bool = False
    split_update: bool = False
    mfma_fp32: bool = False
    lm_gram_paths: int = 4096
    lm_lam0: float = 1e-3
    lm_lam_up: float = 4.0
    lm_lam_down: float = 1.0 / 3.0
    lm_lam_min: float = 1e-9
    lm_lam_max: float = 1e10
    lm_ridge: float = 1e-10
    lm_diag_floor: float = 0.0
    lm_damping: str = "simple"
    lm_bias_fix: bool = True
    lm_gram_skip: int = 3
    lm_leaf_paths: int = -1
    lm_gram_overlap: bool | None = None
    lm_out_fix: bool = False
    lm_out_mu: float = 1e-5
    lm_out_tr: float = 0.0
    lm_split: bool = False
    expose_packet: bool = False
    step_mode: str = "auto"
    variant: int = -1


@dataclass
class DateData:

    feats: list
    prices_next: list
    bond_next: float
    target: torch.Tensor
    prices_now: list = field(default_factory=list)
    bond_now: float = 1.0
    fmu: tuple = ()
    fisd: tuple = ()
    gram_feats: list | None = None
    gram_prices_next: list | None = None
    gram_target: torch.Tensor | None = None


@dataclass
class PnlData:

    n_dates: int
    features: object
    prices: object
    bond: torch.Tensor
    fmu: torch.Tensor
    fisd: torch.Tensor
    w0: torch.Tensor | None
    payoff: torch.Tensor
    wealth0: float = 0.0


def pnl_fold_factors(bond) -> tuple:
    b = np.asarray(bond, np.float64)
    g = (b[1:] / b[:-1]).astype(np.float32)
    tail = np.concatenate([np.cumprod(g[::-1].astype(np.float64))[::-1], [1.0]])
    return g, tail[1:].astype(np.float32), np.float32(tail[0])


@dataclass(frozen=True)
class Exercise:

    kind: str
    strike: float
    every: int = 1

    def __post_init__(self):
        if self.kind not in ("put", "call"):
            raise ValueError(f"exercise kind must be 'put' or 'call', got {self.kind!r}")
        if int(self.every) < 1:
# ... 10 lines not shown
```

rphedge/engine/hip.py:

```python
from __future__ import annotations

import os
from dataclasses import replace

import numpy as np
import torch

from ..models.hedge_mlp import NetSpec
from ..ops import layout as L
from .config import DateData, Exercise, FitConfig, PnlData, TrainConfig
from .lm_geometry import (_lm_bias_index, _lm_out_n, gram_subsample, lm_explore_nsub, lm_gram_geometry, lm_og_wgs,
                          lm_out_nu, lm_pass_schedule, lm_shard_gram_wgs, lm_tpack_len)
from .state import StateBlocks, _Cache, _check_eval_data, _set_norm, _steps, fit_template

PNL_PPT = L.PNL_PPT
PERSISTENT_MAX_WGS = 64


def _env(name: str, default) -> int:
    return int(os.environ.get("RPH_" + name, default))


_clone = lambda desc: type(desc).from_buffer_copy(desc)


class HipBackend(StateBlocks):
    name = "hip"

    def __init__(self, spec: NetSpec, n_local: int, tcfg: TrainConfig, device=None, comm=None,
                 world: int = 1, rank: int = 0, stream=None, mailbox=None, lm_mailbox=None, lm_comm=None):
        from ..ops import native

        self.mailbox = mailbox
        self.lm_mailbox = lm_mailbox
        self._lm_nccl = lm_comm
        self.native = native
        native.load(required=True)
        self.spec, self.n_local, self.tcfg = spec, int(n_local), tcfg
        self.device = torch.device(device) if device is not None else torch.device("cuda", torch.cuda.current_device())
        self.comm, self.world, self.rank, self.stream = comm, world, rank, stream
        self.shape = (spec.nin, spec.hidden, spec.nout, spec.head)
        self.P, self.R = native.net_nparams(*self.shape)
        self._lm_shape, self._lm_wps = native.lm_shape(*self.shape), native.lm_pass_wps(*self.shape)
        assert self.P == spec.nparams
        self.batch_local, self.steps_per_epoch = _steps(self.n_local, tcfg, world)
        hyb512 = spec.hidden == 8 and spec.nin <= 3 and self.R <= 128 and world == 1
        auto_v = 5 if (hyb512 or (spec.hidden == 8 and self.R > 128)) else 0
        self.variant = int(tcfg.variant) if int(tcfg.variant) >= 0 else auto_v
        work = max(1, self.batch_local // (256 * max(1, tcfg.paths_per_thread)))
        mw = int(tcfg.max_wgs)
        if mw <= 0:
            mw = 512 if (spec.hidden == 32 and not tcfg.mfma_fp32 and spec.nin == 1) else 256
            if (self.variant == 5 and hyb512 and tcfg.step_mode in ("auto", "lag") and not tcfg.deterministic
                    and not tcfg.split_update):
                mw = 512
        self.num_wgs = int(max(1, min(mw, work)))
        dev = self.device
        self.slab = torch.zeros(self.num_wgs, self.R, dtype=torch.float32, device=dev)
        self.counter = torch.zeros(4, dtype=torch.int32, device=dev)
        self.grad = torch.zeros(self.R, dtype=torch.float32, device=dev)
        self.acc = torch.zeros(8, self.R, dtype=torch.float32, device=dev)
        self.acc_fit = torch.zeros(3, L.LAG_SLOTS, self.R, dtype=torch.float32, device=dev)
        self.fit_ctl = torch.zeros(4, dtype=torch.int32, device=dev)
        self.lag = torch.zeros(2, L.LAG_FLOATS, dtype=torch.float32, device=dev)
        self._acc_clean = False
        self.stamps = None
        self.eval_wgs = int(max(1, min(_env("EVAL_WGS", 2048), (self.n_local + 255) // 256)))
        self._cache = _Cache()
        self.lm_last_fused = False
        self._lm_same_gram = True

    def _template(self, fcfg: FitConfig):
        return self._cache.get(("fit", fcfg.key()), lambda: fit_template(fcfg, self.device))

    def _lr(self, fcfg: FitConfig):
        if fcfg.lr_schedule is None:
            return None
        return self._cache.get(("lr", tuple(fcfg.lr_schedule)),
                               lambda: torch.tensor(list(fcfg.lr_schedule), dtype=torch.float32, device=self.device))

    def _train_desc(self, wts, opt, fit, data: DateData, fcfg: FitConfig, seed: int, lr_t):
        n = self.native
        d = n.TrainDesc()
        n.fill_ptrs(d.feat, data.feats)
        n.fill_ptrs(d.price, data.prices_next)
        d.target = data.target.data_ptr()
        d.wts, d.opt, d.fit = wts.data_ptr(), opt.data_ptr(), fit.data_ptr()
        d.lr_sched = n.ptr(lr_t)
        d.slab, d.counter, d.grad_out = self.slab.data_ptr(), self.counter.data_ptr(), self.grad.data_ptr()
        d.bond, d.alpha, d.quantile = float(data.bond_next), float(self.spec.alpha), float(fcfg.quantile)
        d.inv_batch, d.loss = 1.0 / float(self.batch_local * self.world), int(fcfg.loss)
        d.n_local, d.batch, d.steps_per_epoch = self.n_local, self.batch_local, self.steps_per_epoch
        d.chunk_log2, d.shuffle = int(self.tcfg.chunk_log2), 1 if self.tcfg.shuffle else 0
        d.seed = int(seed) & 0xFFFFFFFF
        fused_dp = self.mailbox is not None and self.world > 1
        d.fused_update = 1 if ((self.world == 1 or fused_dp) and not self.tcfg.split_update) else 0
        if self.world > 1 and self.comm is None and not fused_dp:
            raise RuntimeError("HipBackend with world_size > 1 needs an RCCL communicator or an IPC mailbox")
        if fused_dp:
            self.mailbox.fill(d)
        else:
            d.dp_world, d.dp_rank = 1, 0
        d.acc, d.stamps = self.acc.data_ptr(), n.ptr(self.stamps)
        d.deterministic, d.mfma_fp32 = 1 if self.tcfg.deterministic else 0, 1 if self.tcfg.mfma_fp32 else 0
        d.variant, d.num_wgs = self.variant, self.num_wgs
        d.nin, d.h, d.nout, d.head = self.shape
        _set_norm(d, data)
        return d

    def _full_batch_desc(self, wts, opt, fit, data: DateData, fcfg: FitConfig, loss: int):
        d = self._train_desc(wts, opt, fit, data, fcfg, 0, None)
        d.batch, d.steps_per_epoch, d.shuffle = self.n_local, 1, 0
        d.inv_batch = 1.0 / float(self.n_local * max(self.world, 1))
        d.loss = int(loss)
        return d

    def fit(self, wts, opt, fit, data: DateData, fcfg: FitConfig, seed: int, poll_every: int = 0):
        assert len(data.feats) == self.spec.nin and len(data.prices_next) == self.spec.nhold - 1
        if fcfg.optimizer == "lm":
            return self._lm_fit(wts, opt, fit, data, fcfg)
        d = self._train_desc(wts, opt, fit, data, fcfg, seed, self._lr(fcfg))
        n, S = self.native, self.steps_per_epoch
        mode = self.step_mode(poll_every)
        if mode == "lag" and not self.tcfg.expose_packet:
            d.grad_out = None
        if mode == "lag" and fcfg.epochs > 0:
            d.fit_init = self._template(fcfg).data_ptr()
            if not self._acc_clean:
                n.memset_async(self.acc_fit, 0, self.stream)
        else:
            fit.copy_(self._template(fcfg), non_blocking=True)
        self._acc_clean = False
        if mode == "persistent":
            n.memset_async(self.acc_fit, 0, self.stream)
            n.memset_async(self.fit_ctl, 0, self.stream)
            d.acc, d.counter = self.acc_fit.data_ptr(), self.fit_ctl.data_ptr()
            n.train_fit(d, fcfg.epochs, self.stream)
            return
        if mode == "lag":
            d.acc, d.lag = self.acc_fit.data_ptr(), self.lag.data_ptr()
            if not poll_every:
                n.train_lag_fit(d, fcfg.epochs, self.stream)
                self._acc_clean = fcfg.epochs > 0
                return
            k = 0
            for e in range(fcfg.epochs):
                for s in range(S):
                    n.train_lag_step(d, k, e, self.stream)
                    k += 1
                if poll_every and (e + 1) % poll_every == 0 and e + 1 < fcfg.epochs:
                    if float(fit[L.F_STOPPED].item()) != 0.0:
                        break
            n.train_lag_finalize(d, k, self.stream)
            self._acc_clean = True
            return
        per_step_host = (self.world > 1 and d.fused_update == 0) or self.tcfg.split_update
        if not poll_every and not per_step_host:
            n.train_ticket_fit(d, fcfg.epochs, self.stream)
            return
        for e in range(fcfg.epochs):
            for s in range(S):
                n.train_step(d, s, e, self.stream)
                if (self.world > 1 and d.fused_update == 0) or self.tcfg.split_update:
                    if self.comm is not None:
                        self.comm.allreduce_(self.grad, self.stream)
                    n.train_update(d, s, e, self.stream)
            if poll_every and (e + 1) % poll_every == 0 and e + 1 < fcfg.epochs:
                if float(fit[L.F_STOPPED].item()) != 0.0:
                    break

    def lm_supported(self) -> bool:
        return self._lm_shape is not None

# ... 41 lines not shown
        gw, blk, stride, inv = g["side" if (side or self.world <= 1) else "local"]
        if side:
            if data.gram_feats[0].numel() != gw * L.LM_TILE:
                raise ValueError(f"Gram subsample data has {data.gram_feats[0].numel()} paths, expected {gw * L.LM_TILE}")
            self.native.fill_ptrs(lm.gfeat, data.gram_feats)
            self.native.fill_ptrs(lm.gprice, data.gram_prices_next)
        lm.gram_side = 1 if side else 0
        lm.gram_wgs, lm.gram_blk, lm.gram_blk_stride, lm.inv_ns = gw, blk, stride, inv
        auto = int(lm.leaf_blocks) > 0 if self.tcfg.lm_gram_overlap is None else bool(self.tcfg.lm_gram_overlap)
        lm.gram_base = lm.num_wgs if (_env("LM_GRAM_OVERLAP", auto) and int(lm.inst) == 1) else 0
        return side or self.world <= 1

    def lm_exchange_bytes(self) -> int:
        if self.world <= 1:
            return 0
        P, _, nblk = self._lm_shape
        return 8 * self._lm_greg(False) if self._lm_same_gram else 8 * (nblk * 1024 + lm_tpack_len(P, nblk) + L.LM_RED - L.LM_GBLK_MAX)

    def _lm_greg(self, og: bool) -> int:
        n = L.LM_RED_OUTG - L.LM_GBLK_MAX
        if og:
            nu = lm_out_nu(self.spec)
            n += nu * (nu + 1) // 2
        return n + (n & 1)

    def lm_exchange_bytes_run(self, passes_first: int, passes_rest: int, dates: int) -> int:
        if self.world <= 1:
            return 0
        if not self._lm_same_gram:
            return self.lm_exchange_bytes() * (passes_first + 1 + (dates - 1) * (passes_rest + 1))
        og = bool(_lm_out_n(self.spec, self.tcfg))
        tot = 0
        for n in [passes_first] + [passes_rest] * (dates - 1):
            k_og = min(L.LM_OUTG_TAIL, n + 1) if og else 0
            tot += 8 * ((n + 1 - k_og) * self._lm_greg(False) + k_og * self._lm_greg(True))
        return tot

    def _lm_set_fit(self, lm, fcfg: FitConfig, data: DateData, fused: bool):
        lm.passes = int(fcfg.epochs)
        lm.stop_tol, lm.stop_min = float(fcfg.lm_stop_tol), max(1, int(fcfg.lm_stop_min))
        lm.lam0 = float(self.tcfg.lm_lam0 if fcfg.lm_lam0 is None else fcfg.lm_lam0)
        lm.lam_carry, lm.q_kappa = float(fcfg.lm_lam_carry), float(fcfg.lm_q_kappa)
        lm.q_delta = float(fcfg.lm_q_delta) if float(fcfg.lm_q_delta) > 0.0 else 1e-6
        lm.renorm = 0
        if fcfg.lm_renorm is not None and data.fmu:
            mu, isd = fcfg.lm_renorm
            for i in range(len(mu)):
                lm.ren_mu[i], lm.ren_isd[i] = float(mu[i]), float(isd[i])
            lm.renorm = 1
        lm.dp_fused = 1 if fused else 0
        if fused:
            lm.dp = self._cache.get(("lm_dp",), self.lm_mailbox.lm_desc)

    def _lm_prepare(self, wts, opt, fit, data: DateData, fcfg: FitConfig):
        pin = int(fcfg.loss) == L.LOSS_PINBALL
        if int(fcfg.loss) not in (L.LOSS_MSE, L.LOSS_PINBALL):
            raise ValueError(f"no Levenberg-Marquardt fit for loss {fcfg.loss}")
        explore = int(fcfg.lm_starts) >= 1 and int(fcfg.lm_explore_passes) > 0
        if pin and explore:
            raise ValueError("pinball LM fits have no multi-start exploration")
        lm = self._lm_buffers(fcfg.loss)["desc"]
        self._lm_same_gram = self._lm_gram_mode(lm, data, allow_side=(not pin or data.gram_target is not None))
        fused = self.world > 1 and self.lm_mailbox is not None and self._lm_same_gram and not self.tcfg.lm_split
        self._lm_set_fit(lm, fcfg, data, fused)
        if explore:
            lm.lam_carry = 1.0
        self.lm_last_fused = fused
        return self._full_batch_desc(wts, opt, fit, data, fcfg, fcfg.loss), lm

    def _lm_fit(self, wts, opt, fit, data: DateData, fcfg: FitConfig):
        d, lm = self._lm_prepare(wts, opt, fit, data, fcfg)
        if int(fcfg.lm_starts) >= 1 and int(fcfg.lm_explore_passes) > 0:
            self._lm_explore(d, fcfg)
        self._lm_launch(d, lm, self._lm_buffers(fcfg.loss)["red"],
                        (self.world <= 1 or lm.dp_fused) and not self.tcfg.lm_split, not self._lm_same_gram)

    def _lm_launch(self, d, lm, red, one_launch: bool, gram: bool):
        n = self.native
        if one_launch:
            n.lm_fit(d, lm, red, self.stream)
            return
        for k in range(lm.passes + 1):
            n.lm_eval(d, lm, red, k, self.stream)
            og = bool(lm.out_gram) and k > lm.passes - L.LM_OUTG_TAIL
            self._lm_allreduce(red, gram=gram, og=og)
            n.lm_solve(d, lm, red, k, self.stream)

    def lm_explore_paths(self, fcfg: FitConfig) -> int:
        return lm_explore_nsub(fcfg, self.n_local)

    def _lm_explore_buffers(self, K: int, nsub: int) -> dict:
        _, R, nblk = self._lm_shape
        t, dev = self.tcfg, self.device
        wps = _env("LM_EXPLORE_WPS", self._lm_wps)
        nw, leaf = lm_pass_schedule(nsub, 0 if int(t.lm_leaf_paths) >= 0 else -1, wps)
        nw1 = lm_pass_schedule(nsub, 0 if int(t.lm_leaf_paths) >= 0 else -1)[0]
        if K > 1:
            nw = max(1, min(nw, 256 * wps // K))
            nw1 = max(1, min(nw1, 256 // K))
            if leaf > 0:
                leaf = -(-((nsub + 127) // 128) // (4 * nw))
        gw = lm_shard_gram_wgs(nsub, t.lm_gram_paths, 1, nw1)
        bufs = dict(state=torch.zeros(K, L.LMS_FLOATS, dtype=torch.float64, device=dev),
                    red=torch.zeros(K, L.LM_RED, dtype=torch.float64, device=dev),
                    slab_b=torch.zeros(K, nw, R, dtype=torch.float32, device=dev),
                    slab_g=torch.zeros(K, gw, nblk * 1024, dtype=torch.float32, device=dev),
                    w0=torch.zeros(K, L.LM_NPMAX, dtype=torch.float32, device=dev), w0_rows=None,
                    sel=torch.zeros(L.LM_RED, dtype=torch.float64, device=dev))
        lm = _clone(self._lm_buffers()["base"])
        lm.state, lm.slab_b, lm.slab_g, lm.w0 = (bufs[k].data_ptr() for k in ("state", "slab_b", "slab_g", "w0"))
        lm.inst, lm.explore, lm.out_n, lm.out_gram = K, 1, 0, 0
        lm.num_wgs, lm.gram_wgs, lm.leaf_blocks = nw, gw, leaf
        lm.gram_blk, lm.gram_blk_stride = lm_gram_geometry(nsub, gw * L.LM_TILE, 1)
        lm.inv_ns, lm.inv_n = 1.0 / float(gw * L.LM_TILE), 1.0 / float(nsub)
        bufs["desc"] = lm
        return bufs

    def _lm_explore_prepare(self, d_main, fcfg: FitConfig):
        K, xd = int(fcfg.lm_starts), fcfg.lm_explore_data
        if self.world > 1 and xd is None:
            raise ValueError("data-parallel multi-start exploration needs lm_explore_data (the global prefix)")
        nsub = self.lm_explore_paths(fcfg)
        if K > L.LM_SEL_MAX:
            raise ValueError(f"{K} starts exceed the {L.LM_SEL_MAX} selection candidates")
        if fcfg.lm_w0s is None or len(fcfg.lm_w0s) < K:
            raise ValueError("multi-start exploration needs lm_w0s (one start point per instance)")
        x = self._cache.get(("lm_explore", K, nsub), lambda: self._lm_explore_buffers(K, nsub))
        self._lm_set_fit(x["desc"], replace(fcfg, epochs=int(fcfg.lm_explore_passes), lm_stop_tol=0.0, lm_lam_carry=0.0,
                                            lm_renorm=None), None, False)
        d = _clone(d_main)
        if xd is not None:
            self.native.fill_ptrs(d.feat, xd.feats)
            self.native.fill_ptrs(d.price, xd.prices_next)
            d.target = xd.target.data_ptr()
# ... 160 lines not shown
            d.ex_kind, d.ex_every, d.ex_strike = L.EX_KINDS[exercise.kind], int(exercise.every), float(exercise.strike)
        if tau_out is not None:
            assert tau_out.dtype == torch.int32 and tau_out.numel() == nl
            d.tau_out = tau_out.data_ptr()
        assert stats.shape[0] == d.num_wgs and snap.shape[0] >= data.n_dates
        n.pnl(d, self.stream)

    def oos_wgs(self, n_local: int) -> int:
        return int(max(1, min(self.native.oos_max_wgs(), (int(n_local) + 255) // 256)))

    def oos(self, sim, snap, data: PnlData, stats, payoff_kind: int, strike: float, has_b: bool = False,
            hold_c: float = 0.0, pnl_out=None, payoff_out=None):
        n = self.native
        d = n.OosDesc()
        d.sim = sim
        nl = int(sim.n_local)
        d.snap = snap.data_ptr()
        d.fmu, d.fisd, d.bond = data.fmu.data_ptr(), data.fisd.data_ptr(), data.bond.data_ptr()
        for name, t in (("pnl_out", pnl_out), ("payoff_out", payoff_out)):
            if t is not None and (t.dtype != torch.float32 or t.numel() != nl):
                raise ValueError(f"oos: {name} must be float32 [{nl}]")
        d.pnl_out, d.payoff_out = n.ptr(pnl_out), n.ptr(payoff_out)
        if stats.dtype != torch.float64 or stats.dim() != 2 or stats.shape[1] != L.EVAL_NSTAT:
            raise ValueError(f"oos: stats must be float64 [num_wgs, {L.EVAL_NSTAT}]")
        d.stats = stats.data_ptr()
        d.alpha, d.hold_c, d.wealth0, d.strike = float(self.spec.alpha), float(hold_c), float(data.wealth0), float(strike)
        d.has_b, d.payoff_kind, d.n_dates, d.num_wgs = 1 if has_b else 0, int(payoff_kind), int(data.n_dates), int(stats.shape[0])
        d.nin, d.h, d.nout, d.head = self.shape
        if snap.shape[0] < data.n_dates or data.fmu.shape[0] < data.n_dates or data.bond.numel() < data.n_dates + 1:
            raise ValueError("oos: snapshot / standardisation / bond tables shorter than n_dates")
        n.oos(d, self.stream)
        return d

    def pnl_finish(self, acc, w0, payoff, carry: float, stats, pnl_out=None):
        n = self.native
        d = n.PnlFinishDesc()
        for t in (acc, w0, payoff):
            assert t.dtype == torch.float32 and t.numel() == self.n_local
        d.acc, d.w0, d.payoff = acc.data_ptr(), w0.data_ptr(), payoff.data_ptr()
        if pnl_out is not None:
            assert pnl_out.dtype == torch.float32 and pnl_out.numel() == self.n_local
        d.pnl_out = n.ptr(pnl_out)
        d.stats = stats.data_ptr()
        d.carry = float(carry)
        d.n_local, d.num_wgs = self.n_local, self.pnl_wgs()
        d.nin, d.h, d.nout, d.head = self.shape
        assert stats.shape[0] == d.num_wgs
        n.pnl_finish(d, self.stream)

    def eval(self, wts, data: DateData, stats, wts_b=None, g_base=None, blend_c=0.0, hold_c=0.0,
             v_out=None, hold_out=None, resid_out=None, pred1_out=None, snap_a=None, snap_b=None,
             n_local: int | None = None, exercise: Exercise | None = None, pnl_acc=None, pnl_grow: float = 1.0,
             pnl_carry: float = 1.0, pnl_first: bool = False):
        _check_eval_data(self.spec, data)
        n = self.native
        d = n.EvalDesc()
        d.snap_a, d.snap_b = n.ptr(snap_a), n.ptr(snap_b)
        n.fill_ptrs(d.feat, data.feats)
        n.fill_ptrs(d.price_t, data.prices_now)
        n.fill_ptrs(d.price_t1, data.prices_next)
        d.target = n.ptr(data.target)
        d.wa, d.wb, d.g_base, d.v_out = wts.data_ptr(), n.ptr(wts_b), n.ptr(g_base), n.ptr(v_out)
        if hold_out is not None:
            n.fill_ptrs(d.hold_out, hold_out)
        d.resid_out, d.pred1_out = n.ptr(resid_out), n.ptr(pred1_out)
        d.stats = stats.data_ptr()
        d.bond_t, d.bond_t1 = float(data.bond_now), float(data.bond_next)
        d.alpha = float(self.spec.alpha)
        d.blend_c, d.hold_c = float(blend_c), float(hold_c)
        d.n_local = self.n_local if n_local is None else int(n_local)
        if d.n_local != int(data.feats[0].numel()):
            raise ValueError(f"eval over {data.feats[0].numel()} paths with n_local {d.n_local}")
        d.num_wgs = self.eval_wgs
        d.nin, d.h, d.nout, d.head = self.shape
        _set_norm(d, data)
        if exercise is not None:
            d.ex_kind, d.ex_strike = L.EX_KINDS[exercise.kind], float(exercise.strike)
        if pnl_acc is not None:
            if pnl_acc.dtype != torch.float32 or pnl_acc.numel() != d.n_local:
                raise ValueError(f"eval: pnl_acc must be float32 [{d.n_local}]")
            d.pnl_acc = pnl_acc.data_ptr()
            d.pnl_grow, d.pnl_carry, d.pnl_first = float(pnl_grow), float(pnl_carry), 1 if pnl_first else 0
        n.eval_(d, self.stream)
```

rphedge/ops/native.py:

```python
from __future__ import annotations

import ctypes as C
import os
from pathlib import Path

import torch

from . import layout as L
from .layout import DP_SLOTS, MAXHOLD, MAXIN

_LIB_ENV = os.environ.get("RPH_NATIVE_LIB", "")
_LIB_PATH = Path(_LIB_ENV).resolve() if _LIB_ENV.endswith(".so") else Path(__file__).resolve().parent.parent / "_lib" / (
    {"debug": "librphedge_debug.so", "asan": "librphedge_asan.so"}.get(_LIB_ENV, "librphedge.so"))
_lib = None
_load_error: str | None = None

VP = C.c_void_p



class TrainDesc(C.Structure):
    _fields_ = [
        ("feat", VP * MAXIN), ("price", VP * MAXHOLD), ("target", VP),
        ("wts", VP), ("opt", VP), ("fit", VP), ("lr_sched", VP),
# ... 34 lines not shown
        for f in range(MAXIN):
            self.fisd[f] = 1.0


class PnlFinishDesc(C.Structure):
    _fields_ = [
        ("acc", VP), ("w0", VP), ("payoff", VP), ("pnl_out", VP), ("stats", VP),
        ("carry", C.c_float), ("n_local", C.c_int), ("num_wgs", C.c_int),
        ("nin", C.c_int), ("h", C.c_int), ("nout", C.c_int), ("head", C.c_int), ("pad0", C.c_int),
    ]


class PnlDesc(C.Structure):
    _fields_ = [
        ("feat", VP * MAXIN), ("feat_ts", C.c_longlong * MAXIN), ("price", VP * MAXHOLD),
        ("price_ts", C.c_longlong * MAXHOLD), ("snap", VP), ("fmu", VP), ("fisd", VP), ("bond", VP),
        ("w0", VP), ("payoff", VP), ("pnl_out", VP), ("stats", VP),
        ("alpha", C.c_float), ("hold_c", C.c_float), ("wealth0", C.c_float), ("has_b", C.c_int),
        ("n_local", C.c_int), ("n_dates", C.c_int), ("num_wgs", C.c_int),
        ("nin", C.c_int), ("h", C.c_int), ("nout", C.c_int), ("head", C.c_int),
        ("ex_kind", C.c_int), ("ex_every", C.c_int), ("ex_strike", C.c_float), ("tau_out", VP),
    ]


class LmDpDesc(C.Structure):
    _fields_ = [
        ("mbox", VP * 8), ("counter", VP), ("error", VP),
        ("world", C.c_int), ("rank", C.c_int), ("pitch", C.c_int), ("fault", C.c_int),
    ]


class LmDesc(C.Structure):
    _fields_ = [
        ("state", VP), ("slab_b", VP), ("slab_g", VP),
        ("num_wgs", C.c_int), ("gram_wgs", C.c_int), ("red_wgs", C.c_int), ("passes", C.c_int),
        ("gram_blk", C.c_int), ("gram_blk_stride", C.c_int), ("inv_ns", C.c_float), ("inv_n", C.c_float),
        ("lam0", C.c_float), ("lam_up", C.c_float), ("lam_down", C.c_float), ("lam_min", C.c_float),
        ("lam_max", C.c_float), ("ridge", C.c_float), ("bias_index", C.c_int), ("weights_only", C.c_int),
        ("damping", C.c_int), ("stop_min", C.c_int), ("stop_tol", C.c_float), ("gram_skip", C.c_int),
        ("inst", C.c_int), ("explore", C.c_int), ("lam_carry", C.c_float), ("diag_floor", C.c_float), ("w0", VP),
        ("renorm", C.c_int), ("pad1", C.c_int), ("ren_mu", C.c_float * MAXIN), ("ren_isd", C.c_float * MAXIN),
        ("out_n", C.c_int), ("out_mu", C.c_float), ("out_gram", C.c_int), ("out_tr", C.c_float),
        ("slab_o", VP),
        ("gfeat", VP * MAXIN), ("gprice", VP * MAXIN), ("gram_side", C.c_int), ("q_delta", C.c_float), ("q_kappa", C.c_float),
        ("pad_dp", C.c_int), ("dp", LmDpDesc), ("dp_fused", C.c_int), ("leaf_blocks", C.c_int), ("gtarget", VP),
        ("gram_base", C.c_int), ("pad4", C.c_int),
    ]

    def __init__(self, *a, **kw):
        super().__init__(*a, **kw)
        self.inst = 1


class SimDesc(C.Structure):
    _fields_ = [
        ("model", C.c_int), ("n_local", C.c_int), ("path_offset", C.c_longlong),
        ("n_fine", C.c_int), ("reduction", C.c_int), ("n_coarse", C.c_int), ("na", C.c_int),
        ("fp64", C.c_int), ("parity", C.c_int),
        ("sv1", VP), ("shift1", VP), ("dims1", C.c_int), ("pad_sv2", C.c_int),
        ("sv2", VP), ("shift2", VP), ("dims2", C.c_int), ("pad_s0", C.c_int),
        ("s0", C.c_double * MAXIN), ("mu", C.c_double * MAXIN), ("sigma", C.c_double * MAXIN),
        ("chol", C.c_double * (MAXIN * MAXIN)), ("dt", C.c_double), ("inv_norm", C.c_double * MAXIN),
        ("v0", C.c_double), ("a", C.c_double), ("b", C.c_double), ("c", C.c_double),
        ("kappa", C.c_double), ("theta", C.c_double), ("xi", C.c_double), ("rho", C.c_double),
        ("l0", C.c_double), ("lc", C.c_double), ("eta", C.c_double), ("n0", C.c_int), ("seed", C.c_uint32),
        ("out", VP), ("out2", VP), ("out3", VP), ("final_out", VP), ("final2_out", VP),
        ("sv_tscale", C.c_double), ("scheme", C.c_int), ("path_stat", C.c_int),
        ("map_blk", C.c_longlong), ("map_stride", C.c_longlong),
    ]


class OosDesc(C.Structure):

    _fields_ = [
        ("sim", SimDesc), ("snap", VP), ("fmu", VP), ("fisd", VP), ("bond", VP), ("pnl_out", VP),
        ("payoff_out", VP), ("stats", VP),
        ("alpha", C.c_float), ("hold_c", C.c_float), ("wealth0", C.c_float), ("strike", C.c_float),
        ("has_b", C.c_int), ("payoff_kind", C.c_int), ("n_dates", C.c_int), ("num_wgs", C.c_int),
        ("nin", C.c_int), ("h", C.c_int), ("nout", C.c_int), ("head", C.c_int),
    ]


DESCRIPTORS = (TrainDesc, EvalDesc, PnlFinishDesc, PnlDesc, LmDpDesc, LmDesc, SimDesc)
DESCRIPTORS_EXT = (OosDesc,)

PYTHON_ONLY: tuple[str, ...] = ()


class _FieldRow(C.Structure):
    _fields_ = [("strct", C.c_char_p), ("field", C.c_char_p), ("offset", C.c_uint), ("size", C.c_uint)]


class _ConstRow(C.Structure):
    _fields_ = [("name", C.c_char_p), ("value", C.c_longlong)]


def native_layout(lib) -> tuple[list[tuple[str, str, int, int]], list[tuple[str, int]]]:
    fr, cr = C.POINTER(_FieldRow)(), C.POINTER(_ConstRow)()
    nf, nc = lib.rph_layout_fields(C.byref(fr)), lib.rph_layout_consts(C.byref(cr))
    return ([(r.strct.decode(), r.field.decode(), r.offset, r.size) for r in fr[:nf]],
            [(r.name.decode(), r.value) for r in cr[:nc]])


def native_layout_ext(lib) -> list[tuple[str, str, int, int]]:
    fr = C.POINTER(_FieldRow)()
    nf = lib.rph_layout_fields_ext(C.byref(fr))
    return [(r.strct.decode(), r.field.decode(), r.offset, r.size) for r in fr[:nf]]


def layout_mismatches(fields, consts, classes=DESCRIPTORS, layout=L) -> list[str]:
    bad = []
    for cls in classes:
        s = cls.__name__
        nat = {f: (o, z) for t, f, o, z in fields if t == s}
        py = {f[0]: (getattr(cls, f[0]).offset, getattr(cls, f[0]).size) for f in cls._fields_}
        say = lambda v, side: f"{side} offset {v[0]} size {v[1]}" if v else f"not in {side}"
        bad += [f"{s}.{f}: {say(nat.get(f), 'native')}, {say(py.get(f), 'ctypes')}"
                for f in dict(nat, **py) if nat.get(f) != py.get(f)]
        size = max((o + z for o, z in nat.values()), default=0)
        if size != C.sizeof(cls):
            bad.append(f"{s}: native size {size}, ctypes size {C.sizeof(cls)}")
    nat = dict(consts)
    py = {k: v for k, v in vars(layout).items() if k.isupper() and type(v) is int}
    bad += [f"layout.{k}: native {v}, python {py.get(k, 'has none')}" for k, v in nat.items() if py.get(k) != v]
    bad += [f"layout.{k}: python {v}, not in the native table" for k, v in py.items()
            if k not in nat and k not in PYTHON_ONLY]
    return bad


def _bind(lib):
    sig = {
        "rph_last_error": (C.c_char_p, []),
        "rph_layout_fields": (C.c_int, [C.POINTER(C.POINTER(_FieldRow))]),
        "rph_layout_consts": (C.c_int, [C.POINTER(C.POINTER(_ConstRow))]),
        "rph_layout_fields_ext": (C.c_int, [C.POINTER(C.POINTER(_FieldRow))]),
        "rph_oos": (C.c_int, [C.POINTER(OosDesc), VP]),
        "rph_oos_check": (C.c_int, [C.POINTER(OosDesc)]),
        "rph_oos_max_wgs": (C.c_int, [C.POINTER(C.c_int)]),
        "rph_device_info": (C.c_int, [C.c_int, C.POINTER(C.c_int), C.POINTER(C.c_int), C.POINTER(C.c_longlong),
                                      C.c_char_p, C.c_int]),
        "rph_memset_async": (C.c_int, [VP, C.c_int, C.c_longlong, VP]),
        "rph_stream_sync": (C.c_int, [VP]),
        "rph_graph_begin": (C.c_int, [VP]),
        "rph_graph_end": (C.c_int, [VP, C.POINTER(VP), C.POINTER(C.c_longlong)]),
        "rph_graph_launch": (C.c_int, [VP, VP]),
        "rph_graph_destroy": (C.c_int, [VP]),
        "rph_nccl_unique_id": (C.c_int, [C.c_char_p]),
        "rph_nccl_init": (C.c_int, [C.c_char_p, C.c_int, C.c_int, C.POINTER(VP)]),
        "rph_nccl_allreduce_f32": (C.c_int, [VP, VP, C.c_longlong, VP]),
        "rph_nccl_allreduce_f64": (C.c_int, [VP, VP, C.c_longlong, VP]),
        "rph_nccl_allreduce_u32": (C.c_int, [VP, VP, C.c_longlong, VP]),
        "rph_nccl_destroy": (C.c_int, [VP]),
        "rph_net_nparams": (C.c_int, [C.c_int] * 4 + [C.POINTER(C.c_int), C.POINTER(C.c_int)]),
        "rph_train_step": (C.c_int, [C.POINTER(TrainDesc), C.c_int, C.c_int, VP]),
        "rph_train_update": (C.c_int, [C.POINTER(TrainDesc), C.c_int, C.c_int, VP]),
        "rph_train_fit": (C.c_int, [C.POINTER(TrainDesc), C.c_int, VP]),
        "rph_train_lag_step": (C.c_int, [C.POINTER(TrainDesc), C.c_int, C.c_int, VP]),
        "rph_train_lag_finalize": (C.c_int, [C.POINTER(TrainDesc), C.c_int, VP]),
        "rph_train_lag_fit": (C.c_int, [C.POINTER(TrainDesc), C.c_int, VP]),
        "rph_train_ticket_fit": (C.c_int, [C.POINTER(TrainDesc), C.c_int, VP]),
        "rph_eval": (C.c_int, [C.POINTER(EvalDesc), VP]),
        "rph_pnl": (C.c_int, [C.POINTER(PnlDesc), VP]),
        "rph_pnl_finish": (C.c_int, [C.POINTER(PnlFinishDesc), VP]),
        "rph_lm_shape": (C.c_int, [C.c_int] * 4 + [C.POINTER(C.c_int)] * 3),
        "rph_lm_pass_wps": (C.c_int, [C.c_int] * 4),
        "rph_lm_eval": (C.c_int, [C.POINTER(TrainDesc), C.POINTER(LmDesc), VP, C.c_int, VP]),
        "rph_lm_solve": (C.c_int, [C.POINTER(TrainDesc), C.POINTER(LmDesc), VP, C.c_int, VP]),
        "rph_lm_fit": (C.c_int, [C.POINTER(TrainDesc), C.POINTER(LmDesc), VP, VP]),
        "rph_lm_dp_exchange": (C.c_int, [C.POINTER(LmDpDesc), VP, C.c_int, C.c_int, VP]),
        "rph_lm_select": (C.c_int, [C.POINTER(TrainDesc), C.POINTER(LmDesc), VP, VP, C.c_int, C.c_int, C.c_int,
                                    C.c_int, VP]),
        "rph_sobol_normal": (C.c_int, [VP, C.c_int, C.c_int, VP, VP, C.c_longlong, C.c_int, C.c_int, VP]),
        "rph_sobol_normal_check": (C.c_int, [C.c_int, C.c_longlong]),
        "rph_simulate": (C.c_int, [C.POINTER(SimDesc), VP]),
        "rph_simulate_check": (C.c_int, [C.POINTER(SimDesc)]),
        "rph_simulate_pair": (C.c_int, [C.POINTER(SimDesc), C.POINTER(SimDesc), C.POINTER(C.c_int), VP]),
        "rph_payoff": (C.c_int, [C.c_int, C.c_int, C.c_int, VP, VP, C.c_float, VP, VP, VP, VP]),
        "rph_radix_hist": (C.c_int, [VP, C.c_longlong, C.c_uint32, C.c_uint32, C.c_int, C.c_int, VP, VP]),
        "rph_ipc_alloc": (C.c_int, [C.c_longlong, C.POINTER(VP), C.c_char_p]),
        "rph_ipc_open": (C.c_int, [C.c_char_p, C.POINTER(VP)]),
        "rph_ipc_close": (C.c_int, [VP]),
        "rph_free": (C.c_int, [VP]),
        "rph_ipc_handle_size": (C.c_int, []),
        "rph_ipc_is_finegrained": (C.c_int, []),
    }
    for name, (res, args) in sig.items():
        fn = getattr(lib, name)
        fn.restype = res
        fn.argtypes = args


def load(required: bool | None = None):
    global _lib, _load_error
    if _lib is not None:
        return _lib
    if required is None:
        required = torch.cuda.is_available()
    try:
        if _LIB_ENV.endswith(".so") and not _LIB_PATH.exists():
            raise FileNotFoundError(f"RPH_NATIVE_LIB={_LIB_ENV} does not exist (it is never built implicitly)")
        if not _LIB_PATH.exists() or os.environ.get("RPH_REBUILD"):
            from .. import build as _build

            v = os.environ.get("RPH_NATIVE_LIB", "")
            _build.build(debug=v == "debug", asan=v == "asan")
        lib = C.CDLL(str(_LIB_PATH), mode=C.RTLD_GLOBAL)
        _bind(lib)
        fields, consts = native_layout(lib)
        bad = layout_mismatches(fields + native_layout_ext(lib), consts, classes=DESCRIPTORS + DESCRIPTORS_EXT)
        if bad:
            raise RuntimeError("native/Python layout mismatch:\n  " + "\n  ".join(bad))
        _lib = lib
        return lib
    except Exception as e:
        _load_error = f"{type(e).__name__}: {e}"
        if required:
            raise RuntimeError(f"rphedge native library unavailable on a GPU machine: {_load_error}") from e
        return None


def available() -> bool:
    return load(required=False) is not None


def _check(rc: int, what: str):
    if rc != 0:
        msg = _lib.rph_last_error().decode() if _lib is not None else ""
        raise RuntimeError(f"{what} failed with code {rc}: {msg}")


def ptr(t) -> int | None:
    if t is None:
        return None
    return t.data_ptr()


def fill_ptrs(arr, tensors):
    for i, t in enumerate(tensors):
        arr[i] = ptr(t)


def stream_handle(stream=None) -> int:
    if isinstance(stream, int):
        return stream
    s = stream if stream is not None else torch.cuda.current_stream()
    return s.cuda_stream


def net_nparams(nin: int, h: int, nout: int, head: int) -> tuple[int, int]:
    lib = load(required=True)
    p, r = C.c_int(), C.c_int()
    if lib.rph_net_nparams(nin, h, nout, head, C.byref(p), C.byref(r)) != 0:
        raise ValueError(f"unsupported hedge network shape nin={nin} h={h} nout={nout} head={head}")
    return p.value, r.value


def sobol_normal(out: torch.Tensor, table, offset: int = 0, raw: bool = False, stream=None):
    lib = load(required=True)
    sv, sh, dims = table
    n, d = out.shape
    assert d <= dims
    fp64 = 1 if out.dtype == torch.float64 else 0
# ... 19 lines not shown
def simulate_pair(a: SimDesc, b: SimDesc, stream=None) -> bool:
    lib = load(required=True)
    merged = C.c_int(0)
    _check(lib.rph_simulate_pair(C.byref(a), C.byref(b), C.byref(merged), stream_handle(stream)), "rph_simulate_pair")
    return bool(merged.value)


def train_step(desc: TrainDesc, step: int, epoch: int, stream=None):
    _check(_lib.rph_train_step(C.byref(desc), int(step), int(epoch), stream_handle(stream)), "rph_train_step")


def train_fit(desc: TrainDesc, epochs: int, stream=None):
    _check(_lib.rph_train_fit(C.byref(desc), int(epochs), stream_handle(stream)), "rph_train_fit")


def train_lag_step(desc: TrainDesc, k: int, epoch: int, stream=None):
    _check(_lib.rph_train_lag_step(C.byref(desc), int(k), int(epoch), stream_handle(stream)), "rph_train_lag_step")


def train_lag_fit(desc: TrainDesc, epochs: int, stream=None):
    load(required=True)
    _check(_lib.rph_train_lag_fit(C.byref(desc), int(epochs), stream_handle(stream)), "rph_train_lag_fit")


def train_ticket_fit(desc: TrainDesc, epochs: int, stream=None):
    load(required=True)
    _check(_lib.rph_train_ticket_fit(C.byref(desc), int(epochs), stream_handle(stream)), "rph_train_ticket_fit")


def train_lag_finalize(desc: TrainDesc, K: int, stream=None):
    _check(_lib.rph_train_lag_finalize(C.byref(desc), int(K), stream_handle(stream)), "rph_train_lag_finalize")


def train_update(desc: TrainDesc, step: int, epoch: int, stream=None):
    _check(_lib.rph_train_update(C.byref(desc), int(step), int(epoch), stream_handle(stream)), "rph_train_update")


def eval_(desc: EvalDesc, stream=None):
    _check(_lib.rph_eval(C.byref(desc), stream_handle(stream)), "rph_eval")


def lm_shape(nin: int, h: int, nout: int, head: int):
    lib = load(required=True)
    v = [C.c_int() for _ in range(3)]
    if lib.rph_lm_shape(nin, h, nout, head, *[C.byref(x) for x in v]) != 0:
        return None
    return tuple(int(x.value) for x in v)


def lm_pass_wps(nin: int, h: int, nout: int, head: int) -> int:
    return int(load(required=True).rph_lm_pass_wps(nin, h, nout, head))


def lm_eval(desc: TrainDesc, lm: LmDesc, red_new: torch.Tensor, pass_: int, stream=None):
    _check(_lib.rph_lm_eval(C.byref(desc), C.byref(lm), ptr(red_new), int(pass_), stream_handle(stream)),
           "rph_lm_eval")


def lm_solve(desc: TrainDesc, lm: LmDesc, red_new: torch.Tensor, pass_: int, stream=None):
    _check(_lib.rph_lm_solve(C.byref(desc), C.byref(lm), ptr(red_new), int(pass_), stream_handle(stream)),
           "rph_lm_solve")


def lm_fit(desc: TrainDesc, lm: LmDesc, red_new: torch.Tensor, stream=None):
    load(required=True)
    _check(_lib.rph_lm_fit(C.byref(desc), C.byref(lm), ptr(red_new), stream_handle(stream)), "rph_lm_fit")


def lm_select(desc: TrainDesc, lm: LmDesc, sel: torch.Tensor, main_state: torch.Tensor, world: int, rank: int,
              p: int, phase: int, stream=None):
    _check(_lib.rph_lm_select(C.byref(desc), C.byref(lm), ptr(sel), ptr(main_state), int(world), int(rank), int(p),
                              int(phase), stream_handle(stream)), "rph_lm_select")


def lm_dp_exchange(x: LmDpDesc, red: torch.Tensor, ng: int, p: int, stream=None):
    load(required=True)
    _check(_lib.rph_lm_dp_exchange(C.byref(x), ptr(red), int(ng), int(p), stream_handle(stream)),
           "rph_lm_dp_exchange")


def pnl(desc: PnlDesc, stream=None):
    load(required=True)
    _check(_lib.rph_pnl(C.byref(desc), stream_handle(stream)), "rph_pnl")


def oos(desc: OosDesc, stream=None):
    load(required=True)
    _check(_lib.rph_oos(C.byref(desc), stream_handle(stream)), "rph_oos")


def oos_check(desc: OosDesc):
    lib = load(required=True)
    _check(lib.rph_oos_check(C.byref(desc)), "rph_oos")


def oos_max_wgs() -> int:
    lib = load(required=True)
    v = C.c_int()
    _check(lib.rph_oos_max_wgs(C.byref(v)), "rph_oos_max_wgs")
    return int(v.value)


def pnl_finish(desc: PnlFinishDesc, stream=None):
    load(required=True)
    _check(_lib.rph_pnl_finish(C.byref(desc), stream_handle(stream)), "rph_pnl_finish")


def payoff(kind: int, s: torch.Tensor, out: torch.Tensor, strike: float, nfrac=None, wts=None, na: int = 1,
           stream=None, x=None):
    lib = load(required=True)
    n = out.numel()
    _check(lib.rph_payoff(kind, n, na, ptr(s), ptr(nfrac), float(strike), ptr(wts), ptr(x), ptr(out),
                          stream_handle(stream)), "rph_payoff")


def radix_hist(x: torch.Tensor, pmask: int, prefix: int, shift: int, nbins: int, hist: torch.Tensor, stream=None):
    lib = load(required=True)
    _check(lib.rph_radix_hist(ptr(x), x.numel(), pmask & 0xFFFFFFFF, prefix & 0xFFFFFFFF, shift, nbins, ptr(hist),
                              stream_handle(stream)), "rph_radix_hist")
# ... 133 lines not shown
```

Baseline: 215.0 million.

## Ride previous-date evaluation on LM solve workgroups and fuse self-target into first pass

Adds a combined kernel in which the first LM_SPEC workgroups run the LM solve while the remaining workgroups evaluate the previously fitted network over the paths. This overlaps the eval with the latency-bound solve and removes a separate eval launch. It also lets the first LM pass compute the regression target from the next date's network, so no separate target-building kernel is needed. The cost is more kernel variants, extra LDS and registers in the pass kernel, and a narrower set of supported shapes and configurations.

Measured after the change: 222.7 million (median of 6 runs). +3.6%, better.

```diff
diff --git a/csrc/hedge_eval.h b/csrc/hedge_eval.h
--- /dev/null
+++ b/csrc/hedge_eval.h
@@ -0,0 +1,209 @@
+#pragma once
+#include "hedge_core.h"
+
+namespace rph {
+
+template <int NIN, int H, int NO, int HEAD, bool PA, bool EX = false>
+struct EvalBody {
+  using S = NetShape<NIN, H, NO, HEAD>;
+  static constexpr int NHOLD = S::NHOLD;
+  static_assert(!PA || NIN >= NHOLD - 1, "price alias needs a feature per traded asset");
+  static constexpr int WBOFF = (S::P + 3) / 4 * 4;
+  static constexpr int WL_FLOATS = WBOFF + S::P + 4;
+  static constexpr int NS = 64;
+  static constexpr int EPF = 4;
+  struct In {
+    float x[NIN], pt[NHOLD], pt1[NHOLD], tgt, gb;
+    int p;
+    bool valid;
+  };
+  struct Mode {
+    bool has_b, has1, pnl_on, pnl_read;
+    RPH_INLINE explicit Mode(const EvalDesc& d)
+        : has_b(d.wb != nullptr),
+          has1(d.price_t1[0] != nullptr),
+          pnl_on(!EX && d.pnl_acc != nullptr),
+          pnl_read(!EX && d.pnl_acc != nullptr && !d.pnl_first) {}
+  };
+
+  RPH_INLINE static void stage(const EvalDesc& d, const Mode& md, float* wl, const bool snap) {
+    for (int i = threadIdx.x; i < S::P; i += 256) {
+      wl[i] = d.wa->w[0][i];
+      if (md.has_b) wl[WBOFF + i] = d.wb->w[0][i];
+    }
+    __syncthreads();
+    if (snap) {
+      for (int i = threadIdx.x; i < S::P; i += 256) {
+        if (d.snap_a) d.snap_a->w[0][i] = wl[i];
+        if (d.snap_b) d.snap_b->w[0][i] = md.has_b ? wl[WBOFF + i] : wl[i];
+      }
+    }
+  }
+
+  RPH_INLINE static void load_in(const EvalDesc& d, const Mode& md, int p, In& in) {
+    in.p = p;
+    in.valid = p < d.n_local;
+    const int pp = in.valid ? p : 0;
+#pragma unroll
+    for (int f = 0; f < NIN; ++f) in.x[f] = d.feat[f][pp];
+#pragma unroll
+    for (int k = 0; k < NHOLD - 1; ++k) {
+      if constexpr (PA) in.pt[k] = in.x[PA ? k : 0];
+      else in.pt[k] = d.price_t[k][pp];
+      in.pt1[k] = md.has1 ? d.price_t1[k][pp] : 0.f;
+    }
+    in.tgt = (md.has1 && d.target) ? d.target[pp] : 0.f;
+    in.gb = d.g_base ? d.g_base[pp] : 0.f;
+  }
+
+  RPH_INLINE static void reset(float (&st)[NS], float& rmin, float& rmax) {
+#pragma unroll
+    for (int i = 0; i < NS; ++i) st[i] = 0.f;
+    rmin = INFINITY;
+    rmax = -INFINITY;
+  }
+
+  RPH_INLINE static void path(const EvalDesc& d, const Mode& md, const In& cur, const float* __restrict__ WA,
+                              const float* __restrict__ WB, float (&st)[NS], float& rmin, float& rmax) {
+    const int p = cur.p;
+    const bool valid = cur.valid;
+    const float racc = md.pnl_read ? d.pnl_acc[valid ? p : 0] : 0.f;
+    uint32_t zo = 0;
+    asm volatile("" : "+v"(zo));
+    const float* __restrict__ WAi = (const float*)__builtin_assume_aligned(WA + (zo & ~3u), 16);
+    const float* __restrict__ WBi = (const float*)__builtin_assume_aligned(WB + (zo & ~3u), 16);
+    float z1[H], a1[H], z2[H], a2[H], hold[NHOLD], holdv[NHOLD], xn[NIN];
+#pragma unroll
+    for (int f = 0; f < NIN; ++f) xn[f] = (cur.x[f] - d.fmu[f]) * d.fisd[f];
+    net_forward<NIN, H, NO, HEAD>(WAi, xn, d.alpha, z1, a1, z2, a2, hold);
+#pragma unroll
+    for (int k = 0; k < NHOLD; ++k) holdv[k] = hold[k];
+    if (md.has_b) {
+      net_forward<NIN, H, NO, HEAD>(WBi, xn, d.alpha, z1, a1, z2, a2, holdv);
+#pragma unroll
+      for (int k = 0; k < NHOLD; ++k) hold[k] = hold[k] + d.hold_c * (holdv[k] - hold[k]);
+    }
+    float V = 0.f;
+#pragma unroll
+    for (int k = 0; k < NHOLD - 1; ++k) V = fmaf(holdv[k], cur.pt[k], V);
+    V = fmaf(holdv[NHOLD - 1], d.bond_t, V);
+    if (d.g_base) V = cur.gb + d.blend_c * (V - cur.gb);
+    [[maybe_unused]] float cont = V, xval = 0.f;
+    [[maybe_unused]] bool exer = false;
+    if constexpr (EX) {
+      xval = d.ex_kind == EX_PUT ? fmaxf(d.ex_strike - cur.pt[0], 0.f) : fmaxf(cur.pt[0] - d.ex_strike, 0.f);
+      exer = xval > 0.f && xval >= cont;
+      V = exer ? xval : cont;
+    }
+    float res = 0.f, pred1 = 0.f;
+    const float tgt = cur.tgt;
+    if (md.has1) {
+#pragma unroll
+      for (int k = 0; k < NHOLD - 1; ++k) pred1 = fmaf(hold[k], cur.pt1[k], pred1);
+      pred1 = fmaf(hold[NHOLD - 1], d.bond_t1, pred1);
+      if (d.target) res = tgt - pred1;
+    }
+    if (valid) {
+      if (d.v_out) d.v_out[p] = V;
+#pragma unroll
+      for (int k = 0; k < NHOLD; ++k)
+        if (d.hold_out[k]) d.hold_out[k][p] = hold[k];
+      if (d.resid_out) d.resid_out[p] = res;
+      if (d.pred1_out) d.pred1_out[p] = pred1;
+      if constexpr (!EX) {
+        if (md.pnl_on) {
+          float gain = 0.f;
+#pragma unroll
+          for (int k = 0; k < NHOLD - 1; ++k) gain = fmaf(hold[k], cur.pt1[k] - cur.pt[k] * d.pnl_grow, gain);
+          d.pnl_acc[p] = fmaf(d.pnl_carry, gain, racc);
+        }
+      }
+      st[ES_V] += V;
+      st[ES_V2] += V * V;
+      st[ES_RES] += res;
+      st[ES_RES2] += res * res;
+      st[ES_ABSRES] += fabsf(res);
+      st[ES_APE] += d.target ? fabsf(res) * __frcp_rn(fmaxf(fabsf(tgt), 1e-7f)) : 0.f;
+      st[ES_PRED1] += pred1;
+      st[ES_COUNT] += 1.f;
+      if constexpr (EX) {
+        st[ES_EXER] += exer ? 1.f : 0.f;
+        st[ES_EXVAL] += exer ? xval : 0.f;
+        st[ES_CONT] += cont;
+      }
+#pragma unroll
+      for (int k = 0; k < NHOLD; ++k) {
+        st[ES_HOLD + k] += hold[k];
+        st[ES_HOLD2 + k] += hold[k] * hold[k];
+      }
+      rmin = fminf(rmin, res);
+      rmax = fmaxf(rmax, res);
+    }
+  }
+
+  RPH_INLINE static void finish(const EvalDesc& d, float (&st)[NS], float rmin, float rmax,
+                                double (*sst)[EVAL_NSTAT], const int vb) {
+    const int lane = threadIdx.x & 63, wid = threadIdx.x >> 6;
+    wave_reduce_scatter<NS>(st, lane);
+#pragma unroll
+    for (int o = 1; o < 64; o <<= 1) {
+      rmin = fminf(rmin, __shfl_xor(rmin, o, 64));
+      rmax = fmaxf(rmax, __shfl_xor(rmax, o, 64));
+    }
+    if (lane < EVAL_NSTAT) sst[wid][lane] = (double)st[0];
+    if (lane == 0) {
+      sst[wid][ES_RESMIN] = rmin;
+      sst[wid][ES_RESMAX] = rmax;
+    }
+    __syncthreads();
+    if (threadIdx.x < EVAL_NSTAT) {
+      const int i = threadIdx.x;
+      double v;
+      if (i == ES_RESMIN) v = fmin(fmin(sst[0][i], sst[1][i]), fmin(sst[2][i], sst[3][i]));
+      else if (i == ES_RESMAX) v = fmax(fmax(sst[0][i], sst[1][i]), fmax(sst[2][i], sst[3][i]));
+      else v = sst[0][i] + sst[1][i] + sst[2][i] + sst[3][i];
+      d.stats[(size_t)vb * EVAL_NSTAT + i] = v;
+    }
+  }
+
+  RPH_INLINE static void ride(const EvalDesc& d, const int r, const int nr, float* wl, double (*sst)[EVAL_NSTAT]) {
+    const Mode md(d);
+    stage(d, md, wl, r == 0);
+    const float* __restrict__ WA = wl;
+    const float* __restrict__ WB = md.has_b ? wl + WBOFF : wl;
+    const int nvb = d.num_wgs, stride = nvb * 256, n = d.n_local;
+    const int tid = threadIdx.x;
+    int lvb = r, lp0 = r * 256;
+    auto load_next = [&](In& in) {
+      load_in(d, md, lvb < nvb ? lp0 + tid : n, in);
+      lp0 += stride;
+      if (lp0 >= n) {
+        lvb += nr;
+        lp0 = lvb * 256;
+      }
+    };
+    In q[EPF];
+#pragma unroll
+    for (int i = 0; i < EPF; ++i) load_next(q[i]);
+    float st[NS], rmin, rmax;
+    reset(st, rmin, rmax);
+    int cvb = r, cp0 = r * 256;
+    while (cvb < nvb) {
+      const In cur = q[0];
+#pragma unroll
+      for (int i = 0; i + 1 < EPF; ++i) q[i] = q[i + 1];
+      if (lvb < nvb) load_next(q[EPF - 1]);
+      path(d, md, cur, WA, WB, st, rmin, rmax);
+      cp0 += stride;
+      if (cp0 >= n) {
+        finish(d, st, rmin, rmax, sst, cvb);
+        reset(st, rmin, rmax);
+        cvb += nr;
+        cp0 = cvb * 256;
+        __syncthreads();
+      }
+    }
+  }
+};
+
+}
diff --git a/csrc/hedge_lm.hip b/csrc/hedge_lm.hip
--- a/csrc/hedge_lm.hip
+++ b/csrc/hedge_lm.hip
@@ -1,6 +1,8 @@
+#include <type_traits>
 #include <utility>
 
 #include "hedge_core.h"
+#include "hedge_eval.h"
 #include "hedge_narrow.h"
 
 namespace rph {
@@ -52,7 +54,8 @@
 
 template <class B>
 __global__ __launch_bounds__(256, B::WAVES_PER_SIMD) void k_lm_pass(const TrainDesc d, const LmDesc lm, const int pass,
-                                                                   const double* __restrict__ red_new) {
+                                                                   const double* __restrict__ red_new,
+                                                                   const SelfTargetDesc self) {
   constexpr int P = B::P;
   constexpr int R = B::R;
   constexpr int NR = B::NR;
@@ -65,6 +68,7 @@
   __shared__ __attribute__((aligned(16))) float wl[P + 4];
   __shared__ __attribute__((aligned(16))) float jt[B::FINAL ? 4 : LM_TILE * JP];
   __shared__ __attribute__((aligned(16))) unsigned char og_img[B::OGM ? B::OG_LDS : 16];
+  __shared__ __attribute__((aligned(16))) float wt[B::ST_ ? P + 4 : 4];
   const int tid = threadIdx.x, lane = tid & 63, wid = tid >> 6;
   prefetch_kernarg_end(kat);
   const bool stamp_wg = blockIdx.x >= 2 && blockIdx.y == 0;
@@ -87,7 +91,10 @@
   const bool fin = B::FINAL || pass == lm.passes;
   const typename B::Sched sc =
       B::sched(d, lm.num_wgs, (gram_base > 0 || fin) ? 0 : lm.gram_wgs, lm.gram_skip, lm.leaf_blocks);
-  if (path_wg) B::load(d, 0, perm, sc.b0 * 128, lane, pre);
+  if (path_wg) B::load(d, 0, perm, sc.b0 * 128, lane, pre, &self);
+  if constexpr (B::ST_) {
+    for (int i = tid; i < P; i += 256) wt[i] = self.st_wts->w[0][i];
+  }
   for (int i = tid; i < P; i += 256) {
     float w;
     if (pass == 0) {
@@ -146,7 +153,7 @@
     B::make_frags(wl + S::OW2, fr);
     float val[NR];
     B::partial(d, 0, perm, wl, fr, scratch, pre, val, sc, og_img,
-               lm.slab_o + ((size_t)inst * lm.num_wgs + blockIdx.x) * 3 * 1024);
+               lm.slab_o + ((size_t)inst * lm.num_wgs + blockIdx.x) * 3 * 1024, &self, wt);
 #pragma unroll
     for (int j = 0; j < NR; ++j)
       if (tid + 256 * j < R) slab_b[(size_t)blockIdx.x * R + tid + 256 * j] = val[j];
@@ -762,12 +769,11 @@
 }
 
 template <int P, int R, int NU>
-__global__ __launch_bounds__(256) void k_lm_solve(const TrainDesc d, const LmDesc lm, const double* __restrict__ red_new,
-                                                  const int pass) {
+RPH_INLINE void lm_solve_body(const TrainDesc& d, const LmDesc& lm, const double* __restrict__ red_new, const int pass,
+                              double* const lds) {
 #pragma clang fp contract(off)
   using LS = LmShape<P>;
   constexpr int NB = LS::NB, NBLK = LS::NBLK;
-  extern __shared__ __attribute__((aligned(16))) double lds[];
   __shared__ int s_fail;
   __shared__ double s_diag;
   const int tid = threadIdx.x, lane = tid & 63, wid = tid >> 6;
@@ -1128,10 +1134,33 @@
 #undef RPH_STAMPS
 }
 
+template <int P, int R, int NU>
+__global__ __launch_bounds__(256) void k_lm_solve(const TrainDesc d, const LmDesc lm, const double* __restrict__ red_new,
+                                                  const int pass) {
+  extern __shared__ __attribute__((aligned(16))) double lds[];
+  lm_solve_body<P, R, NU>(d, lm, red_new, pass, lds);
+}
+
+template <int P, int R, int NU, class E>
+__global__ __launch_bounds__(256) void k_lm_solve_eval(const TrainDesc d, const LmDesc lm,
+                                                       const double* __restrict__ red_new, const int pass,
+                                                       const EvalDesc ev) {
+  extern __shared__ __attribute__((aligned(16))) double lds[];
+  if (blockIdx.x < LM_SPEC) {
+    lm_solve_body<P, R, NU>(d, lm, red_new, pass, lds);
+    return;
+  }
+  __shared__ double sst[4][EVAL_NSTAT];
+  __shared__ __attribute__((aligned(16))) float wl[E::WL_FLOATS];
+  E::ride(ev, (int)blockIdx.x - LM_SPEC, (int)gridDim.x - LM_SPEC, wl, sst);
+}
+
 template <int NIN, int H, int NO, int HEAD>
 struct LmKernels {
   using Body = NarrowPairBody<NIN, H, NO, HEAD>;
   using BodyOG = NarrowPairBody<NIN, H, NO, HEAD, true>;
+  static constexpr bool HAS_ST = Body::WAVES_PER_SIMD == 2 && HEAD == HEAD_FREE;
+  using BodyST = NarrowPairBody<NIN, H, NO, HEAD, false, HAS_ST>;
   using S = NetShape<NIN, H, NO, HEAD>;
   static constexpr int smem() { return TileGrid<S::P>::LDS_BYTES; }
   static_assert(smem() + 128 <= 160 * 1024, "LM solve exceeds the LDS of one workgroup");
@@ -1187,20 +1216,41 @@
   return 0;
 }
 
+static int lm_validate_st(const TrainDesc* d, const LmDesc* lm, const SelfTargetDesc* st) {
+  if (!st->st_wts || st->st_out != d->target) return rph_report("rph_lm", "st_out: needs st_wts and st_out == target");
+  if (lm->renorm || lm->explore || lm->inst != 1 || lm->weights_only || lm->passes < 1 || d->loss != LOSS_MSE)
+    return rph_report("rph_lm", "st_out: one main MSE fit with passes >= 1, no renorm");
+  for (int f = 0; f < d->nin; ++f)
+    if (!st->st_feat[f] || !(st->st_fisd[f] > 0.f && st->st_fisd[f] < 3.0e38f && st->st_fmu[f] == st->st_fmu[f]))
+      return rph_report("rph_lm", "st_out: null st_feat / bad st_fmu, st_fisd");
+  return 0;
+}
+
 template <int A, int B, int C, int E>
-static int lm_pass_launch(const TrainDesc* d, const LmDesc* lm, int pass, const double* red_new, hipStream_t s) {
+static int lm_pass_launch(const TrainDesc* d, const LmDesc* lm, int pass, const double* red_new, hipStream_t s,
+                          const SelfTargetDesc* stp) {
   using K = LmKernels<A, B, C, E>;
+  const SelfTargetDesc st = stp != nullptr ? *stp : SelfTargetDesc{};
   const bool og = lm->out_gram && pass > lm->passes - LM_OUTG_TAIL;
   const int gend = pass == lm->passes ? 0 : (og && K::BodyOG::OGM ? 0 : lm->gram_base) + lm->gram_wgs;
   const unsigned grid = (unsigned)(gend > lm->num_wgs ? gend : lm->num_wgs);
   if constexpr (K::BodyOG::OGM) {
     if (og) {
       hipLaunchKernelGGL((k_lm_pass<typename K::BodyOG>), dim3(grid, lm->inst), dim3(256), 0, s, *d, *lm, pass,
-                         red_new);
+                         red_new, st);
       return (int)hipGetLastError();
     }
   }
-  hipLaunchKernelGGL((k_lm_pass<typename K::Body>), dim3(grid, lm->inst), dim3(256), 0, s, *d, *lm, pass, red_new);
+  if (st.st_out != nullptr && pass == 0) {
+    if constexpr (K::HAS_ST) {
+      hipLaunchKernelGGL((k_lm_pass<typename K::BodyST>), dim3(grid, lm->inst), dim3(256), 0, s, *d, *lm, pass,
+                         red_new, st);
+      return (int)hipGetLastError();
+    } else {
+      return rph_report("rph_lm", "st_out: no self-target pass body for this network shape");
+    }
+  }
+  hipLaunchKernelGGL((k_lm_pass<typename K::Body>), dim3(grid, lm->inst), dim3(256), 0, s, *d, *lm, pass, red_new, st);
   return (int)hipGetLastError();
 }
 
@@ -1435,16 +1485,20 @@
   return lp;
 }
 
-extern "C" int rph_lm_eval(const TrainDesc* d, const LmDesc* lm, double* red_new, int pass, void* stream) {
+extern "C" int rph_lm_eval_st(const TrainDesc* d, const LmDesc* lm, const SelfTargetDesc* st, double* red_new,
+                              int pass, void* stream) {
   hipStream_t s = (hipStream_t)stream;
+  if (st != nullptr && st->st_out == nullptr) st = nullptr;
   int rc = 0;
   if (match_shape(NarrowShapes{}, d->nin, d->h, d->nout, d->head, &rc, [&](auto t) {
         using T = decltype(t);
         using K = LmKernels<T::NIN, T::H, T::NO, T::HEAD>;
         constexpr int P = K::S::P, R = K::S::R, NU = K::Body::NU, NBLK = LmShape<P>::NBLK;
         if (int rc = lm_validate(d, lm, P, R, NBLK, NU)) return rc;
+        if (st != nullptr)
+          if (int rc = lm_validate_st(d, lm, st)) return rc;
         const LmDesc lp = lm_pass_desc<K>(*lm, pass);
-        if (int rc = lm_pass_launch<T::NIN, T::H, T::NO, T::HEAD>(d, &lp, pass, red_new, s)) return rc;
+        if (int rc = lm_pass_launch<T::NIN, T::H, T::NO, T::HEAD>(d, &lp, pass, red_new, s, st)) return rc;
         const int ngw = lm_gram_red_wgs(NBLK * 1024, lp.gram_wgs);
         const int wg0 = pass == lp.passes ? ngw : 0;
         const int rg = ngw + lm_pk_red_wgs(R, lp.num_wgs, lp.dp_fused) + lm_og_wgs(NU) - wg0;
@@ -1453,6 +1507,10 @@
       }))
     return rc;
   return rph_report("rph_lm_eval", "no LM solver for this network shape (8-unit nets only)");
+}
+
+extern "C" int rph_lm_eval(const TrainDesc* d, const LmDesc* lm, double* red_new, int pass, void* stream) {
+  return rph_lm_eval_st(d, lm, nullptr, red_new, pass, stream);
 }
 
 extern "C" int rph_lm_solve(const TrainDesc* d, const LmDesc* lm, const double* red_new, int pass, void* stream) {
@@ -1479,10 +1537,94 @@
   return rph_report("rph_lm_solve", "no LM solver for this network shape");
 }
 
+extern "C" int rph_lm_solve_eval(const TrainDesc* d, const LmDesc* lm, const double* red_new, int pass,
+                                 const EvalDesc* ev, int riders, void* stream) {
+  hipStream_t s = (hipStream_t)stream;
+  if (!ev || !ev->wa || !ev->stats || ev->n_local < 1 || ev->num_wgs < 1 || riders < 1 || riders > 4096)
+    return rph_report("rph_lm_solve_eval", "bad eval descriptor / rider count");
+  if ((long long)(ev->num_wgs - 1) * 256 >= ev->n_local) return rph_report("rph_lm_solve_eval", "eval grid larger than the paths");
+  if (ev->wb || ev->g_base || ev->ex_kind != EX_NONE) return rph_report("rph_lm_solve_eval", "one network, no exercise date");
+  if (ev->nin != d->nin || ev->h != d->h || ev->nout != d->nout || ev->head != d->head)
+    return rph_report("rph_lm_solve_eval", "eval and fit of different network shapes");
+  if (lm->inst != 1 || lm->explore) return rph_report("rph_lm_solve_eval", "the main fit's solve only");
+  if (!(ev->alpha >= 0.f && ev->alpha <= 1.f)) return rph_report("rph_lm_solve_eval", "LeakyReLU slope must be in [0, 1]");
+  for (int f = 0; f < ev->nin; ++f)
+    if (!ev->feat[f] || !(ev->fisd[f] > 0.f && ev->fisd[f] < 3.0e38f && ev->fmu[f] == ev->fmu[f]))
+      return rph_report("rph_lm_solve_eval", "null feature pointer / bad standardisation");
+  const int nhold = ev->head == HEAD_COMPLEMENT ? 2 : ev->nout;
+  bool alias = ev->nin >= nhold - 1;
+  for (int k = 0; alias && k < nhold - 1; ++k) alias = ev->price_t[k] == ev->feat[k];
+  for (int k = 0; k < nhold - 1; ++k)
+    if (!ev->price_t[k] || (ev->pnl_acc && !ev->price_t1[k]))
+      return rph_report("rph_lm_solve_eval", "null price pointer");
+  if (ev->pnl_acc && (!(fabsf(ev->pnl_grow) <= 3.0e38f) || !(fabsf(ev->pnl_carry) <= 3.0e38f)))
+    return rph_report("rph_lm_solve_eval", "pnl_grow / pnl_carry must be finite");
+  int rc = 0;
+  if (match_shape(NarrowShapes{}, d->nin, d->h, d->nout, d->head, &rc, [&](auto t) {
+        using T = decltype(t);
+        using K = LmKernels<T::NIN, T::H, T::NO, T::HEAD>;
+        if constexpr (!K::HAS_ST) {
+          return rph_report("rph_lm_solve_eval", "no self-target pass body for this network shape");
+        } else {
+        const int bytes = K::smem();
+        auto launch = [&](auto pa) {
+          using E = EvalBody<T::NIN, T::H, T::NO, T::HEAD, decltype(pa)::value, false>;
+          constexpr auto kernel = k_lm_solve_eval<K::S::P, K::S::R, K::Body::NU, E>;
+          static bool attr = false;
+          if (!attr) {
+            hipError_t e = hipFuncSetAttribute((const void*)kernel, hipFuncAttributeMaxDynamicSharedMemorySize, bytes);
+            if (e != hipSuccess) {
+              (void)hipGetLastError();
+              return rph_report("rph_lm_solve_eval", "dynamic LDS request refused");
+            }
+            attr = true;
+          }
+          hipLaunchKernelGGL(kernel, dim3(LM_SPEC + riders, 1), dim3(256), bytes, s, *d, *lm, red_new, pass, *ev);
+          return (int)hipGetLastError();
+        };
+        if constexpr (T::NIN >= T::S::NHOLD - 1) {
+          if (alias) return launch(std::true_type{});
+        }
+        return launch(std::false_type{});
+        }
+      }))
+    return rc;
+  return rph_report("rph_lm_solve_eval", "no LM solver for this network shape");
+}
+
+extern "C" int rph_lm_has_st(int nin, int h, int nout, int head) {
+  int has = 0;
+  match_shape(NarrowShapes{}, nin, h, nout, head, &has, [](auto t) {
+    using T = decltype(t);
+    return LmKernels<T::NIN, T::H, T::NO, T::HEAD>::HAS_ST ? 1 : 0;
+  });
+  return has;
+}
+
+extern "C" int rph_lm_solve_lds(int nin, int h, int nout, int head) {
+  int bytes = 0;
+  match_shape(NarrowShapes{}, nin, h, nout, head, &bytes, [](auto t) {
+    using T = decltype(t);
+    return LmKernels<T::NIN, T::H, T::NO, T::HEAD>::smem();
+  });
+  return bytes;
+}
+
+extern "C" int rph_lm_fit_ride(const TrainDesc* d, const LmDesc* lm, double* red_new, const SelfTargetDesc* st,
+                               const EvalDesc* ev, int riders, void* stream) {
+  if (ev != nullptr && (st == nullptr || st->st_out == nullptr))
+    return rph_report("rph_lm_fit_ride", "a riding eval needs the self-target pass 0 (its v_out has no other writer)");
+  for (int k = 0; k <= lm->passes; ++k) {
+    if (int rc = rph_lm_eval_st(d, lm, st, red_new, k, stream)) return rc;
+    if (k == 0 && ev != nullptr) {
+      if (int rc = rph_lm_solve_eval(d, lm, red_new, k, ev, riders, stream)) return rc;
+    } else if (int rc = rph_lm_solve(d, lm, red_new, k, stream)) {
+      return rc;
+    }
+  }
+  return 0;
+}
+
 extern "C" int rph_lm_fit(const TrainDesc* d, const LmDesc* lm, double* red_new, void* stream) {
-  for (int k = 0; k <= lm->passes; ++k) {
-    if (int rc = rph_lm_eval(d, lm, red_new, k, stream)) return rc;
-    if (int rc = rph_lm_solve(d, lm, red_new, k, stream)) return rc;
-  }
-  return 0;
-}
+  return rph_lm_fit_ride(d, lm, red_new, nullptr, nullptr, 0, stream);
+}
diff --git a/csrc/hedge_mlp.hip b/csrc/hedge_mlp.hip
--- a/csrc/hedge_mlp.hip
+++ b/csrc/hedge_mlp.hip
@@ -1,4 +1,5 @@
 #include "hedge_core.h"
+#include "hedge_eval.h"
 #include "hedge_fit.h"
 #include "hedge_lag.h"
 #include "hedge_narrow.h"
@@ -134,166 +135,32 @@
 
 template <int NIN, int H, int NO, int HEAD, bool PA, bool EX = false>
 __global__ __launch_bounds__(256) void k_hedge_eval(const EvalDesc d) {
-  using S = NetShape<NIN, H, NO, HEAD>;
-  constexpr int NHOLD = S::NHOLD;
-  static_assert(!PA || NIN >= NHOLD - 1, "price alias needs a feature per traded asset");
+  using E = EvalBody<NIN, H, NO, HEAD, PA, EX>;
+  using In = typename E::In;
+  constexpr int EPF = E::EPF;
   prefetch_kernarg<sizeof(EvalDesc)>();
   RPH_DASSERT(d.n_local > 0 && d.num_wgs == (int)gridDim.x && d.wa != nullptr && d.stats != nullptr);
   __shared__ double sst[4][EVAL_NSTAT];
-  constexpr int WBOFF = (S::P + 3) / 4 * 4;
-  __shared__ __attribute__((aligned(16))) float wl[WBOFF + S::P + 4];
-  const bool has_b = d.wb != nullptr;
-  for (int i = threadIdx.x; i < S::P; i += 256) {
-    wl[i] = d.wa->w[0][i];
-    if (has_b) wl[WBOFF + i] = d.wb->w[0][i];
-  }
-  __syncthreads();
-  if (blockIdx.x == 0) {
-    for (int i = threadIdx.x; i < S::P; i += 256) {
-      if (d.snap_a) d.snap_a->w[0][i] = wl[i];
-      if (d.snap_b) d.snap_b->w[0][i] = has_b ? wl[WBOFF + i] : wl[i];
-    }
-  }
+  __shared__ __attribute__((aligned(16))) float wl[E::WL_FLOATS];
+  const typename E::Mode md(d);
+  E::stage(d, md, wl, blockIdx.x == 0);
   const float* __restrict__ WA = wl;
-  const float* __restrict__ WB = has_b ? wl + WBOFF : wl;
-  const int lane = threadIdx.x & 63, wid = threadIdx.x >> 6;
-
-  constexpr int NS = 64;
-  float st[NS];
-#pragma unroll
-  for (int i = 0; i < NS; ++i) st[i] = 0.f;
-  float rmin = INFINITY, rmax = -INFINITY;
-
-  struct In {
-    float x[NIN], pt[NHOLD], pt1[NHOLD], tgt, gb;
-    int p;
-    bool valid;
-  };
-  constexpr int EPF = 4;
+  const float* __restrict__ WB = md.has_b ? wl + E::WBOFF : wl;
+  float st[E::NS], rmin, rmax;
+  E::reset(st, rmin, rmax);
   const int stride = (int)gridDim.x * 256;
-  const bool has1 = d.price_t1[0] != nullptr;
-  const bool pnl_on = !EX && d.pnl_acc != nullptr;
-  const bool pnl_read = pnl_on && !d.pnl_first;
-  auto load_in = [&](int p, In& in) {
-    in.p = p;
-    in.valid = p < d.n_local;
-    const int pp = in.valid ? p : 0;
-#pragma unroll
-    for (int f = 0; f < NIN; ++f) in.x[f] = d.feat[f][pp];
-#pragma unroll
-    for (int k = 0; k < NHOLD - 1; ++k) {
-      if constexpr (PA) in.pt[k] = in.x[PA ? k : 0];
-      else in.pt[k] = d.price_t[k][pp];
-      in.pt1[k] = has1 ? d.price_t1[k][pp] : 0.f;
-    }
-    in.tgt = (has1 && d.target) ? d.target[pp] : 0.f;
-    in.gb = d.g_base ? d.g_base[pp] : 0.f;
-  };
   In q[EPF];
   const int p_first = blockIdx.x * 256 + threadIdx.x;
 #pragma unroll
-  for (int i = 0; i < EPF; ++i) load_in(p_first + i * stride, q[i]);
-
+  for (int i = 0; i < EPF; ++i) E::load_in(d, md, p_first + i * stride, q[i]);
   for (int p0 = blockIdx.x * 256; p0 < d.n_local; p0 += stride) {
     const In cur = q[0];
 #pragma unroll
     for (int i = 0; i + 1 < EPF; ++i) q[i] = q[i + 1];
-    if (p0 + EPF * stride < d.n_local) load_in(cur.p + EPF * stride, q[EPF - 1]);
-    const int p = cur.p;
-    const bool valid = cur.valid;
-    const float racc = pnl_read ? d.pnl_acc[valid ? p : 0] : 0.f;
-    uint32_t zo = 0;
-    asm volatile("" : "+v"(zo));
-    const float* __restrict__ WAi = (const float*)__builtin_assume_aligned(WA + (zo & ~3u), 16);
-    const float* __restrict__ WBi = (const float*)__builtin_assume_aligned(WB + (zo & ~3u), 16);
-    float z1[H], a1[H], z2[H], a2[H], hold[NHOLD], holdv[NHOLD], xn[NIN];
-#pragma unroll
-    for (int f = 0; f < NIN; ++f) xn[f] = (cur.x[f] - d.fmu[f]) * d.fisd[f];
-    net_forward<NIN, H, NO, HEAD>(WAi, xn, d.alpha, z1, a1, z2, a2, hold);
-#pragma unroll
-    for (int k = 0; k < NHOLD; ++k) holdv[k] = hold[k];
-    if (has_b) {
-      net_forward<NIN, H, NO, HEAD>(WBi, xn, d.alpha, z1, a1, z2, a2, holdv);
-#pragma unroll
-      for (int k = 0; k < NHOLD; ++k) hold[k] = hold[k] + d.hold_c * (holdv[k] - hold[k]);
-    }
-    float V = 0.f;
-#pragma unroll
-    for (int k = 0; k < NHOLD - 1; ++k) V = fmaf(holdv[k], cur.pt[k], V);
-    V = fmaf(holdv[NHOLD - 1], d.bond_t, V);
-    if (d.g_base) V = cur.gb + d.blend_c * (V - cur.gb);
-    [[maybe_unused]] float cont = V, xval = 0.f;
-    [[maybe_unused]] bool exer = false;
-    if constexpr (EX) {
-      xval = d.ex_kind == EX_PUT ? fmaxf(d.ex_strike - cur.pt[0], 0.f) : fmaxf(cur.pt[0] - d.ex_strike, 0.f);
-      exer = xval > 0.f && xval >= cont;
-      V = exer ? xval : cont;
-    }
-    float res = 0.f, pred1 = 0.f;
-    const float tgt = cur.tgt;
-    if (has1) {
-#pragma unroll
-      for (int k = 0; k < NHOLD - 1; ++k) pred1 = fmaf(hold[k], cur.pt1[k], pred1);
-      pred1 = fmaf(hold[NHOLD - 1], d.bond_t1, pred1);
-      if (d.target) res = tgt - pred1;
-    }
-    if (valid) {
-      if (d.v_out) d.v_out[p] = V;
-#pragma unroll
-      for (int k = 0; k < NHOLD; ++k)
-        if (d.hold_out[k]) d.hold_out[k][p] = hold[k];
-      if (d.resid_out) d.resid_out[p] = res;
-      if (d.pred1_out) d.pred1_out[p] = pred1;
-      if constexpr (!EX) {
-        if (pnl_on) {
-          float gain = 0.f;
-#pragma unroll
-          for (int k = 0; k < NHOLD - 1; ++k) gain = fmaf(hold[k], cur.pt1[k] - cur.pt[k] * d.pnl_grow, gain);
-          d.pnl_acc[p] = fmaf(d.pnl_carry, gain, racc);
-        }
-      }
-      st[ES_V] += V;
-      st[ES_V2] += V * V;
-      st[ES_RES] += res;
-      st[ES_RES2] += res * res;
-      st[ES_ABSRES] += fabsf(res);
-      st[ES_APE] += d.target ? fabsf(res) * __frcp_rn(fmaxf(fabsf(tgt), 1e-7f)) : 0.f;
-      st[ES_PRED1] += pred1;
-      st[ES_COUNT] += 1.f;
-      if constexpr (EX) {
-        st[ES_EXER] += exer ? 1.f : 0.f;
-        st[ES_EXVAL] += exer ? xval : 0.f;
-        st[ES_CONT] += cont;
-      }
-#pragma unroll
-      for (int k = 0; k < NHOLD; ++k) {
-        st[ES_HOLD + k] += hold[k];
-        st[ES_HOLD2 + k] += hold[k] * hold[k];
-      }
-      rmin = fminf(rmin, res);
-      rmax = fmaxf(rmax, res);
-    }
-  }
-  wave_reduce_scatter<NS>(st, lane);
-#pragma unroll
-  for (int o = 1; o < 64; o <<= 1) {
-    rmin = fminf(rmin, __shfl_xor(rmin, o, 64));
-    rmax = fmaxf(rmax, __shfl_xor(rmax, o, 64));
-  }
-  if (lane < EVAL_NSTAT) sst[wid][lane] = (double)st[0];
-  if (lane == 0) {
-    sst[wid][ES_RESMIN] = rmin;
-    sst[wid][ES_RESMAX] = rmax;
-  }
-  __syncthreads();
-  if (threadIdx.x < EVAL_NSTAT) {
-    const int i = threadIdx.x;
-    double v;
-    if (i == ES_RESMIN) v = fmin(fmin(sst[0][i], sst[1][i]), fmin(sst[2][i], sst[3][i]));
-    else if (i == ES_RESMAX) v = fmax(fmax(sst[0][i], sst[1][i]), fmax(sst[2][i], sst[3][i]));
-    else v = sst[0][i] + sst[1][i] + sst[2][i] + sst[3][i];
-    d.stats[(size_t)blockIdx.x * EVAL_NSTAT + i] = v;
-  }
+    if (p0 + EPF * stride < d.n_local) E::load_in(d, md, cur.p + EPF * stride, q[EPF - 1]);
+    E::path(d, md, cur, WA, WB, st, rmin, rmax);
+  }
+  E::finish(d, st, rmin, rmax, sst, blockIdx.x);
 }
 
 
diff --git a/csrc/hedge_narrow.h b/csrc/hedge_narrow.h
--- a/csrc/hedge_narrow.h
+++ b/csrc/hedge_narrow.h
@@ -1,4 +1,6 @@
 #pragma once
+#include <type_traits>
+
 #include "hedge_core.h"
 
 namespace rph {
@@ -172,8 +174,10 @@
   return __builtin_bit_cast(nb_bf16x8, __builtin_shufflevector(r0, r1, 0, 1, 2, 3, 4, 5, 6, 7));
 }
 
-template <int NIN, int H, int NO, int HEAD, bool OG = false>
+template <int NIN, int H, int NO, int HEAD, bool OG = false, bool ST = false>
 struct NarrowPairBody {
+  static_assert(!ST || (!OG && HEAD == HEAD_FREE), "self-target: the plain free-head body only");
+  static constexpr bool ST_ = ST;
   static constexpr int WAVES_PER_SIMD = (!OG && NIN <= 2 && HEAD == HEAD_FREE && NO <= 2) ? 2 : 1;
   static constexpr int NIN_ = NIN, H_ = H, NO_ = NO, HEAD_ = HEAD;
   using S = NetShape<NIN, H, NO, HEAD>;
@@ -196,8 +200,14 @@
   static_assert(P - NU == S::OW3, "the output block is [OW3, P)");
   static_assert(4 * NBO * 1024 * 4 <= OG_LDS, "the waves' output-Gram tiles reuse the image LDS");
   struct Frags {};
-  struct Pre {
-    nb_f2 x[NIN], pr[NHOLD], y;
+  struct PreTarget {
+    nb_f2 y;
+  };
+  struct PreSelf {
+    nb_f2 xt[NIN];
+  };
+  struct Pre : std::conditional_t<ST, PreSelf, PreTarget> {
+    nb_f2 x[NIN], pr[NHOLD];
     nb_f2 m;
   };
 
@@ -222,16 +232,21 @@
     return {GW * gb + (w - GW), TW - GW, nblk};
   }
 
-  RPH_INLINE static void load(const TrainDesc& d, int, const Perm&, long long j0, int lane, Pre& p) {
+  RPH_INLINE static void load(const TrainDesc& d, int, const Perm&, long long j0, int lane, Pre& p,
+                              const SelfTargetDesc* lm = nullptr) {
     const long long ja = j0 + lane, jb = ja + 64;
     const bool va = ja < d.batch, vb = jb < d.batch;
     const long long qa = va ? ja : 0, qb = vb ? jb : 0;
+    if constexpr (ST) {
+#pragma unroll
+      for (int f = 0; f < NIN; ++f) p.xt[f] = nb_f2{lm->st_feat[f][qa], lm->st_feat[f][qb]};
+    }
 #pragma unroll
     for (int f = 0; f < NIN; ++f) p.x[f] = nb_f2{d.feat[f][qa], d.feat[f][qb]};
 #pragma unroll
     for (int k = 0; k < NHOLD - 1; ++k) p.pr[k] = nb_f2{d.price[k][qa], d.price[k][qb]};
     p.pr[NHOLD - 1] = nb_s(d.bond);
-    p.y = nb_f2{d.target[qa], d.target[qb]};
+    if constexpr (!ST) p.y = nb_f2{d.target[qa], d.target[qb]};
     p.m = nb_f2{va ? 1.f : 0.f, vb ? 1.f : 0.f};
   }
 
@@ -303,7 +318,8 @@
 
   RPH_INLINE static void partial(const TrainDesc& d, int step, const Perm& perm, const float* __restrict__ W,
                                  const Frags&, float* lds, Pre& pre, float (&val)[NR], const Sched& sc,
-                                 unsigned char* og_lds = nullptr, float* __restrict__ og_out = nullptr) {
+                                 unsigned char* og_lds = nullptr, float* __restrict__ og_out = nullptr,
+                                 const SelfTargetDesc* lm = nullptr, const float* __restrict__ Wt = nullptr) {
     const int lane = threadIdx.x & 63, wid = threadIdx.x >> 6;
     const long long stride = sc.bstep * 128;
     const long long jend = sc.bend * 128 < d.batch ? sc.bend * 128 : d.batch;
@@ -338,8 +354,49 @@
       for (int f = 0; f < NIN; ++f) x[f] = (cur.x[f] - d.fmu[f]) * d.fisd[f];
 #pragma unroll
       for (int k = 0; k < NHOLD; ++k) pr[k] = cur.pr[k];
-      const nb_f2 y = cur.y, m = cur.m;
-      if (j0 + stride < jend) load(d, step, perm, j0 + stride, lane, cur);
+      const nb_f2 m = cur.m;
+      nb_f2 y;
+      [[maybe_unused]] nb_f2 xt[ST ? NIN : 1];
+      if constexpr (ST) {
+#pragma unroll
+        for (int f = 0; f < NIN; ++f) xt[f] = (cur.xt[f] - lm->st_fmu[f]) * lm->st_fisd[f];
+      } else {
+        y = cur.y;
+      }
+      if (j0 + stride < jend) load(d, step, perm, j0 + stride, lane, cur, lm);
+      if constexpr (ST) {
+        uint32_t zt = 0;
+        asm volatile("" : "+v"(zt));
+        const float* __restrict__ Wq = (const float*)__builtin_assume_aligned(Wt + (zt & ~3u), 16);
+        nb_f2 t1[H], t2[H];
+#pragma unroll
+        for (int j = 0; j < H; ++j) {
+          nb_f2 acc = nb_s(Wq[S::OB1 + j]);
+#pragma unroll
+          for (int f = 0; f < NIN; ++f) acc = nb_fma(xt[f], nb_s(Wq[S::OW1 + f * H + j]), acc);
+          t1[j] = nb_lrelu(acc, alpha);
+        }
+#pragma unroll
+        for (int j = 0; j < H; ++j) t2[j] = nb_s(Wq[S::OB2 + j]);
+#pragma unroll
+        for (int i = 0; i < H; ++i)
+#pragma unroll
+          for (int j = 0; j < H; ++j) t2[j] = nb_fma(t1[i], nb_s(Wq[S::OW2 + i * H + j]), t2[j]);
+#pragma unroll
+        for (int j = 0; j < H; ++j) t2[j] = nb_lrelu(t2[j], alpha);
+        nb_f2 Vt = nb_s(0.f);
+#pragma unroll
+        for (int k = 0; k < NO; ++k) {
+          nb_f2 acc = nb_s(Wq[S::OB3 + k]);
+#pragma unroll
+          for (int j = 0; j < H; ++j) acc = nb_fma(t2[j], nb_s(Wq[S::OW3 + j * NO + k]), acc);
+          Vt = nb_fma(acc, pr[k], Vt);
+        }
+        y = Vt;
+        if (m.x != 0.f) lm->st_out[j0 + lane] = y.x;
+        if (m.y != 0.f) lm->st_out[j0 + 64 + lane] = y.y;
+        __builtin_amdgcn_sched_barrier(0);
+      }
 
       nb_f2 a1[H], a2[H], o[NO];
 #pragma unroll
diff --git a/csrc/rph_layout.h b/csrc/rph_layout.h
--- a/csrc/rph_layout.h
+++ b/csrc/rph_layout.h
@@ -48,9 +48,12 @@
   X(T, hold_c) X(T, wealth0) X(T, strike) X(T, has_b) X(T, payoff_kind) X(T, n_dates) X(T, num_wgs) X(T, nin)       \
   X(T, h) X(T, nout) X(T, head)
 
+#define RPH_FIELDS_SelfTargetDesc(X, T) X(T, st_feat) X(T, st_wts) X(T, st_out) X(T, st_fmu) X(T, st_fisd)
+
 #define RPH_DESCRIPTORS(X) \
   X(TrainDesc) X(EvalDesc) X(PnlFinishDesc) X(PnlDesc) X(LmDpDesc) X(LmDesc) X(SimDesc)
 #define RPH_DESCRIPTORS_EXT(X) X(OosDesc)
+#define RPH_DESCRIPTORS_RIDE(X) X(SelfTargetDesc)
 
 struct FieldRow {
   const char* strct;
@@ -62,6 +65,7 @@
 #define RPH_STRUCT_ROWS(T) RPH_FIELDS_##T(RPH_FIELD_ROW, T)
 constexpr FieldRow kFieldRows[] = {RPH_DESCRIPTORS(RPH_STRUCT_ROWS)};
 constexpr FieldRow kFieldRowsExt[] = {RPH_DESCRIPTORS_EXT(RPH_STRUCT_ROWS)};
+constexpr FieldRow kFieldRowsRide[] = {RPH_DESCRIPTORS_RIDE(RPH_STRUCT_ROWS)};
 
 constexpr bool layout_same(const char* a, const char* b) {
   for (; *a && *a == *b; ++a, ++b) {}
@@ -83,8 +87,10 @@
                                                     "the struct has implicit padding");
 #define RPH_STRUCT_COVERED(T) RPH_STRUCT_COVERED_IN(kFieldRows, T)
 #define RPH_STRUCT_COVERED_EXT(T) RPH_STRUCT_COVERED_IN(kFieldRowsExt, T)
+#define RPH_STRUCT_COVERED_RIDE(T) RPH_STRUCT_COVERED_IN(kFieldRowsRide, T)
 RPH_DESCRIPTORS(RPH_STRUCT_COVERED)
 RPH_DESCRIPTORS_EXT(RPH_STRUCT_COVERED_EXT)
+RPH_DESCRIPTORS_RIDE(RPH_STRUCT_COVERED_RIDE)
 
 struct ConstRow {
   const char* name;
diff --git a/csrc/rph_types.h b/csrc/rph_types.h
--- a/csrc/rph_types.h
+++ b/csrc/rph_types.h
@@ -266,6 +266,14 @@
   int pad4;
 };
 
+struct SelfTargetDesc {
+  const float* st_feat[MAXIN];
+  const NetWeights* st_wts;
+  float* st_out;
+  float st_fmu[MAXIN];
+  float st_fisd[MAXIN];
+};
+
 constexpr int LM_SEL_W = LM_NPMAX + 2;
 constexpr int LM_SEL_MAX = 64;
 
diff --git a/csrc/runtime.cpp b/csrc/runtime.cpp
--- a/csrc/runtime.cpp
+++ b/csrc/runtime.cpp
@@ -46,6 +46,11 @@
 extern "C" int rph_layout_fields_ext(const FieldRow** rows) {
   *rows = kFieldRowsExt;
   return (int)(sizeof(kFieldRowsExt) / sizeof(kFieldRowsExt[0]));
+}
+
+extern "C" int rph_layout_fields_ride(const FieldRow** rows) {
+  *rows = kFieldRowsRide;
+  return (int)(sizeof(kFieldRowsRide) / sizeof(kFieldRowsRide[0]));
 }
 
 extern "C" int rph_layout_consts(const ConstRow** rows) {
diff --git a/rphedge/api.py b/rphedge/api.py
--- a/rphedge/api.py
+++ b/rphedge/api.py
@@ -348,7 +348,7 @@
                            lm_lam_down=float(tr.lm_lam_down), lm_out_fix=bool(tr.lm_out_fix),
                            lm_out_mu=float(tr.lm_out_mu), lm_out_tr=float(getattr(tr, "lm_out_tr", 0.0)),
                            lm_ridge=float(getattr(tr, "lm_ridge", 1e-10)),
-                           lm_diag_floor=float(tr.lm_diag_floor))
+                           lm_diag_floor=float(tr.lm_diag_floor), eval_ride=bool(getattr(tr, "eval_ride", True)))
         if int(tr.variant) >= 0:
             tcfg.variant = int(tr.variant)
         kw = {}
diff --git a/rphedge/config.py b/rphedge/config.py
--- a/rphedge/config.py
+++ b/rphedge/config.py
@@ -100,6 +100,7 @@
     lm_lam_down: float = 1.0 / 3.0
     lm_lam0_first: float = 0.0
     lm_diag_floor: float = 0.0
+    eval_ride: bool = True
     mean_refit: bool = True
     feature_norm: str = "date"
     feature_norm_floor: float = 0.0
diff --git a/rphedge/driver.py b/rphedge/driver.py
--- a/rphedge/driver.py
+++ b/rphedge/driver.py
@@ -315,6 +315,10 @@
         self.ran = list(range(start, -1, -1))
         self.pnl_done = start == nc - 2
         fold = self.pnl_fold and self.pnl_done
+        ride_run = (hasattr(be, "eval_ride_ok") and c.optimizer == "lm" and not c.q99 and c.exercise is None
+                    and c.warm_start and be.eval_ride_ok(self._fcfg(False, L.LOSS_MSE, 0)))
+        self.eval_rides = 0
+        pending = None
         for t in self.ran:
             first = t == nc - 2
             pnl_kw = dict(pnl_acc=self.pnl_acc, pnl_grow=float(self.pnl_grow[t]), pnl_carry=float(self.pnl_carry[t]),
@@ -347,8 +351,14 @@
                                        seed=fit_seed(c.seed, t, 1), poll_every=0)
                     join = torch.cuda.Event()
                     join.record(self._side)
-            be.fit(self.w_mse, self.opt_mse, f_m, data, self._fcfg(first, L.LOSS_MSE, t),
-                   seed=fit_seed(c.seed, t, 0), poll_every=c.poll_every)
+            if pending is not None:
+                be.fit(self.w_mse, self.opt_mse, f_m, data, self._fcfg(first, L.LOSS_MSE, t),
+                       seed=fit_seed(c.seed, t, 0), poll_every=c.poll_every, ride=pending)
+                pending = None
+                self.eval_rides += 1
+            else:
+                be.fit(self.w_mse, self.opt_mse, f_m, data, self._fcfg(first, L.LOSS_MSE, t),
+                       seed=fit_seed(c.seed, t, 0), poll_every=c.poll_every)
             if c.mean_refit and c.optimizer != "lm":
                 be.bias_refit(self.w_mse, self.opt_mse, f_m, data, self._fcfg(first, L.LOSS_MSE))
             hold_out = [self.holdings[t, k] for k in range(self.spec.nhold)] if self.holdings is not None else None
@@ -367,6 +377,9 @@
                         snap_a=self.snap[t, 0], snap_b=self.snap[t, 1], **pnl_kw)
                 if self.gvalues is not None:
                     self.eval_gram_values(t)
+            elif ride_run and t > 0:
+                pending = be.eval_desc(self.w_mse, data, s_q, hold_out=hold_out, resid_out=resid_out,
+                                       snap_a=self.snap[t, 0], **pnl_kw)
             else:
                 be.eval(self.w_mse, data, s_q, v_out=self.values[t], hold_out=hold_out, resid_out=resid_out,
                         snap_a=self.snap[t, 0], exercise=self.exercise_at(t), **pnl_kw)
diff --git a/rphedge/engine/config.py b/rphedge/engine/config.py
--- a/rphedge/engine/config.py
+++ b/rphedge/engine/config.py
@@ -80,6 +80,7 @@
     lm_out_mu: float = 1e-5
     lm_out_tr: float = 0.0
     lm_split: bool = False
+    eval_ride: bool = True
     expose_packet: bool = False
     step_mode: str = "auto"
     variant: int = -1
diff --git a/rphedge/engine/hip.py b/rphedge/engine/hip.py
--- a/rphedge/engine/hip.py
+++ b/rphedge/engine/hip.py
@@ -69,6 +69,7 @@
         self._cache = _Cache()
         self.lm_last_fused = False
         self._lm_same_gram = True
+        self._lm_st = self._lm_shape is not None and native.lm_has_st(*self.shape)
 
     def _template(self, fcfg: FitConfig):
         return self._cache.get(("fit", fcfg.key()), lambda: fit_template(fcfg, self.device))
@@ -115,10 +116,12 @@
         d.loss = int(loss)
         return d
 
-    def fit(self, wts, opt, fit, data: DateData, fcfg: FitConfig, seed: int, poll_every: int = 0):
+    def fit(self, wts, opt, fit, data: DateData, fcfg: FitConfig, seed: int, poll_every: int = 0, ride=None):
         assert len(data.feats) == self.spec.nin and len(data.prices_next) == self.spec.nhold - 1
         if fcfg.optimizer == "lm":
-            return self._lm_fit(wts, opt, fit, data, fcfg)
+            return self._lm_fit(wts, opt, fit, data, fcfg, ride)
+        if ride is not None:
+            raise ValueError("an eval rides in Levenberg-Marquardt fits only")
         d = self._train_desc(wts, opt, fit, data, fcfg, seed, self._lr(fcfg))
         n, S = self.native, self.steps_per_epoch
         mode = self.step_mode(poll_every)
@@ -266,7 +269,32 @@
         if fused:
             lm.dp = self._cache.get(("lm_dp",), self.lm_mailbox.lm_desc)
 
-    def _lm_prepare(self, wts, opt, fit, data: DateData, fcfg: FitConfig):
+    def eval_riders(self) -> int:
+        cus = 256
+        if self.device.type == "cuda":
+            cus = int(torch.cuda.get_device_properties(self.device).multi_processor_count)
+        per_cu = 2 if 2 * (self.native.lm_solve_lds(*self.shape) + 4096) <= 160 * 1024 else 1
+        return max(1, _env("EVAL_RIDERS", per_cu * cus - L.LM_SPEC))
+
+    def eval_ride_ok(self, fcfg: FitConfig) -> bool:
+        return bool(self.tcfg.eval_ride and _env("EVAL_RIDE", 1) and self._lm_st and self.world == 1
+                    and not self.tcfg.lm_split and fcfg.optimizer == "lm" and int(fcfg.loss) == L.LOSS_MSE
+                    and int(fcfg.epochs) >= 1 and fcfg.lm_renorm is None
+                    and not (int(fcfg.lm_starts) >= 1 and int(fcfg.lm_explore_passes) > 0))
+
+    def _lm_self_target(self, d, ride):
+        st = self.native.SelfTargetDesc()
+        nh = self.spec.nhold
+        if any(ride.price_t[k] != d.price[k] for k in range(nh - 1)) or float(ride.bond_t) != float(d.bond):
+            raise ValueError("ride: the eval's prices / bond at its date are not this fit's prices_next / bond_next")
+        if ride.v_out not in (None, d.target) or ride.wb or ride.g_base or ride.ex_kind:
+            raise ValueError("ride: one network, no exercise date, v_out the fit's target (or none)")
+        for f in range(self.spec.nin):
+            st.st_feat[f], st.st_fmu[f], st.st_fisd[f] = ride.feat[f], ride.fmu[f], ride.fisd[f]
+        st.st_wts, st.st_out = ride.wa, d.target
+        return st
+
+    def _lm_prepare(self, wts, opt, fit, data: DateData, fcfg: FitConfig, ride=None):
         pin = int(fcfg.loss) == L.LOSS_PINBALL
         if int(fcfg.loss) not in (L.LOSS_MSE, L.LOSS_PINBALL):
             raise ValueError(f"no Levenberg-Marquardt fit for loss {fcfg.loss}")
@@ -280,20 +308,29 @@
         if explore:
             lm.lam_carry = 1.0
         self.lm_last_fused = fused
-        return self._full_batch_desc(wts, opt, fit, data, fcfg, fcfg.loss), lm
-
-    def _lm_fit(self, wts, opt, fit, data: DateData, fcfg: FitConfig):
-        d, lm = self._lm_prepare(wts, opt, fit, data, fcfg)
+        d = self._full_batch_desc(wts, opt, fit, data, fcfg, fcfg.loss)
+        if ride is not None and not self.eval_ride_ok(fcfg):
+            raise ValueError("this fit cannot carry an eval (eval_ride_ok)")
+        if ride is not None:
+            return d, lm, self._lm_self_target(d, ride)
+        return d, lm
+
+    def _lm_fit(self, wts, opt, fit, data: DateData, fcfg: FitConfig, ride=None):
+        d, lm, *st = self._lm_prepare(wts, opt, fit, data, fcfg, ride)
         if int(fcfg.lm_starts) >= 1 and int(fcfg.lm_explore_passes) > 0:
             self._lm_explore(d, fcfg)
         self._lm_launch(d, lm, self._lm_buffers(fcfg.loss)["red"],
-                        (self.world <= 1 or lm.dp_fused) and not self.tcfg.lm_split, not self._lm_same_gram)
-
-    def _lm_launch(self, d, lm, red, one_launch: bool, gram: bool):
+                        (self.world <= 1 or lm.dp_fused) and not self.tcfg.lm_split, not self._lm_same_gram, ride, st[0] if st else None)
+
+    def _lm_launch(self, d, lm, red, one_launch: bool, gram: bool, ride=None, st=None):
         n = self.native
         if one_launch:
-            n.lm_fit(d, lm, red, self.stream)
+            if ride is not None:
+                n.lm_fit_ride(d, lm, red, st, ride, self.eval_riders(), self.stream)
+            else:
+                n.lm_fit(d, lm, red, self.stream)
             return
+        assert ride is None
         for k in range(lm.passes + 1):
             n.lm_eval(d, lm, red, k, self.stream)
             og = bool(lm.out_gram) and k > lm.passes - L.LM_OUTG_TAIL
@@ -560,6 +597,16 @@
              v_out=None, hold_out=None, resid_out=None, pred1_out=None, snap_a=None, snap_b=None,
              n_local: int | None = None, exercise: Exercise | None = None, pnl_acc=None, pnl_grow: float = 1.0,
              pnl_carry: float = 1.0, pnl_first: bool = False):
+        self.native.eval_(self.eval_desc(wts, data, stats, wts_b=wts_b, g_base=g_base, blend_c=blend_c, hold_c=hold_c,
+                                         v_out=v_out, hold_out=hold_out, resid_out=resid_out, pred1_out=pred1_out,
+                                         snap_a=snap_a, snap_b=snap_b, n_local=n_local, exercise=exercise,
+                                         pnl_acc=pnl_acc, pnl_grow=pnl_grow, pnl_carry=pnl_carry,
+                                         pnl_first=pnl_first), self.stream)
+
+    def eval_desc(self, wts, data: DateData, stats, wts_b=None, g_base=None, blend_c=0.0, hold_c=0.0,
+                  v_out=None, hold_out=None, resid_out=None, pred1_out=None, snap_a=None, snap_b=None,
+                  n_local: int | None = None, exercise: Exercise | None = None, pnl_acc=None, pnl_grow: float = 1.0,
+                  pnl_carry: float = 1.0, pnl_first: bool = False):
         _check_eval_data(self.spec, data)
         n = self.native
         d = n.EvalDesc()
@@ -589,4 +636,4 @@
                 raise ValueError(f"eval: pnl_acc must be float32 [{d.n_local}]")
             d.pnl_acc = pnl_acc.data_ptr()
             d.pnl_grow, d.pnl_carry, d.pnl_first = float(pnl_grow), float(pnl_carry), 1 if pnl_first else 0
-        n.eval_(d, self.stream)
+        return d
diff --git a/rphedge/ops/native.py b/rphedge/ops/native.py
--- a/rphedge/ops/native.py
+++ b/rphedge/ops/native.py
@@ -110,6 +110,14 @@
         self.inst = 1
 
 
+class SelfTargetDesc(C.Structure):
+
+    _fields_ = [
+        ("st_feat", VP * MAXIN), ("st_wts", VP), ("st_out", VP), ("st_fmu", C.c_float * MAXIN),
+        ("st_fisd", C.c_float * MAXIN),
+    ]
+
+
 class SimDesc(C.Structure):
     _fields_ = [
         ("model", C.c_int), ("n_local", C.c_int), ("path_offset", C.c_longlong),
@@ -141,6 +149,7 @@
 
 DESCRIPTORS = (TrainDesc, EvalDesc, PnlFinishDesc, PnlDesc, LmDpDesc, LmDesc, SimDesc)
 DESCRIPTORS_EXT = (OosDesc,)
+DESCRIPTORS_RIDE = (SelfTargetDesc,)
 
 PYTHON_ONLY: tuple[str, ...] = ()
 
@@ -163,6 +172,12 @@
 def native_layout_ext(lib) -> list[tuple[str, str, int, int]]:
     fr = C.POINTER(_FieldRow)()
     nf = lib.rph_layout_fields_ext(C.byref(fr))
+    return [(r.strct.decode(), r.field.decode(), r.offset, r.size) for r in fr[:nf]]
+
+
+def native_layout_ride(lib) -> list[tuple[str, str, int, int]]:
+    fr = C.POINTER(_FieldRow)()
+    nf = lib.rph_layout_fields_ride(C.byref(fr))
     return [(r.strct.decode(), r.field.decode(), r.offset, r.size) for r in fr[:nf]]
 
 
@@ -192,6 +207,7 @@
         "rph_layout_fields": (C.c_int, [C.POINTER(C.POINTER(_FieldRow))]),
         "rph_layout_consts": (C.c_int, [C.POINTER(C.POINTER(_ConstRow))]),
         "rph_layout_fields_ext": (C.c_int, [C.POINTER(C.POINTER(_FieldRow))]),
+        "rph_layout_fields_ride": (C.c_int, [C.POINTER(C.POINTER(_FieldRow))]),
         "rph_oos": (C.c_int, [C.POINTER(OosDesc), VP]),
         "rph_oos_check": (C.c_int, [C.POINTER(OosDesc)]),
         "rph_oos_max_wgs": (C.c_int, [C.POINTER(C.c_int)]),
@@ -225,6 +241,14 @@
         "rph_lm_eval": (C.c_int, [C.POINTER(TrainDesc), C.POINTER(LmDesc), VP, C.c_int, VP]),
         "rph_lm_solve": (C.c_int, [C.POINTER(TrainDesc), C.POINTER(LmDesc), VP, C.c_int, VP]),
         "rph_lm_fit": (C.c_int, [C.POINTER(TrainDesc), C.POINTER(LmDesc), VP, VP]),
+        "rph_lm_fit_ride": (C.c_int, [C.POINTER(TrainDesc), C.POINTER(LmDesc), VP, C.POINTER(SelfTargetDesc),
+                                      C.POINTER(EvalDesc), C.c_int, VP]),
+        "rph_lm_eval_st": (C.c_int, [C.POINTER(TrainDesc), C.POINTER(LmDesc), C.POINTER(SelfTargetDesc), VP, C.c_int,
+                                     VP]),
+        "rph_lm_solve_eval": (C.c_int, [C.POINTER(TrainDesc), C.POINTER(LmDesc), VP, C.c_int, C.POINTER(EvalDesc),
+                                        C.c_int, VP]),
+        "rph_lm_has_st": (C.c_int, [C.c_int] * 4),
+        "rph_lm_solve_lds": (C.c_int, [C.c_int] * 4),
         "rph_lm_dp_exchange": (C.c_int, [C.POINTER(LmDpDesc), VP, C.c_int, C.c_int, VP]),
         "rph_lm_select": (C.c_int, [C.POINTER(TrainDesc), C.POINTER(LmDesc), VP, VP, C.c_int, C.c_int, C.c_int,
                                     C.c_int, VP]),
@@ -265,7 +289,8 @@
         lib = C.CDLL(str(_LIB_PATH), mode=C.RTLD_GLOBAL)
         _bind(lib)
         fields, consts = native_layout(lib)
-        bad = layout_mismatches(fields + native_layout_ext(lib), consts, classes=DESCRIPTORS + DESCRIPTORS_EXT)
+        bad = layout_mismatches(fields + native_layout_ext(lib) + native_layout_ride(lib), consts,
+                                classes=DESCRIPTORS + DESCRIPTORS_EXT + DESCRIPTORS_RIDE)
         if bad:
             raise RuntimeError("native/Python layout mismatch:\n  " + "\n  ".join(bad))
         _lib = lib
@@ -391,7 +416,11 @@
     return int(load(required=True).rph_lm_pass_wps(nin, h, nout, head))
 
 
-def lm_eval(desc: TrainDesc, lm: LmDesc, red_new: torch.Tensor, pass_: int, stream=None):
+def lm_eval(desc: TrainDesc, lm: LmDesc, red_new: torch.Tensor, pass_: int, stream=None, st=None):
+    if st is not None:
+        _check(_lib.rph_lm_eval_st(C.byref(desc), C.byref(lm), C.byref(st), ptr(red_new), int(pass_),
+                                   stream_handle(stream)), "rph_lm_eval_st")
+        return
     _check(_lib.rph_lm_eval(C.byref(desc), C.byref(lm), ptr(red_new), int(pass_), stream_handle(stream)),
            "rph_lm_eval")
 
@@ -404,6 +433,27 @@
 def lm_fit(desc: TrainDesc, lm: LmDesc, red_new: torch.Tensor, stream=None):
     load(required=True)
     _check(_lib.rph_lm_fit(C.byref(desc), C.byref(lm), ptr(red_new), stream_handle(stream)), "rph_lm_fit")
+
+
+def lm_has_st(nin: int, h: int, nout: int, head: int) -> bool:
+    return bool(load(required=True).rph_lm_has_st(nin, h, nout, head))
+
+
+def lm_solve_lds(nin: int, h: int, nout: int, head: int) -> int:
+    return int(load(required=True).rph_lm_solve_lds(nin, h, nout, head))
+
+
+def lm_solve_eval(desc: TrainDesc, lm: LmDesc, red_new: torch.Tensor, pass_: int, ev: EvalDesc, riders: int,
+                  stream=None):
+    _check(_lib.rph_lm_solve_eval(C.byref(desc), C.byref(lm), ptr(red_new), int(pass_), C.byref(ev), int(riders),
+                                  stream_handle(stream)), "rph_lm_solve_eval")
+
+
+def lm_fit_ride(desc: TrainDesc, lm: LmDesc, red_new: torch.Tensor, st: SelfTargetDesc, ev: EvalDesc, riders: int,
+                stream=None):
+    load(required=True)
+    _check(_lib.rph_lm_fit_ride(C.byref(desc), C.byref(lm), ptr(red_new), C.byref(st), C.byref(ev), int(riders),
+                                stream_handle(stream)), "rph_lm_fit_ride")
 
 
 def lm_select(desc: TrainDesc, lm: LmDesc, sel: torch.Tensor, main_state: torch.Tensor, world: int, rank: int,
```
